# stardist/stardist

Hardware: AMD Instinct MI355X
Metric: predict_instances() Mpix/s (2D) + Mvox/s (3D) end-to-end at 1/2/4/8 GPU (higher is better)
Workload: dtype f32

## Files before the change

include/stardist_hip.h:

```cpp
#ifndef STARDIST_HIP_H
#define STARDIST_HIP_H

#include <stdbool.h>
#include <stdint.h>

#ifdef __cplusplus
extern "C" {
#endif

const char* sd_last_error(void);
int sd_version(void);
int sd_device_count(void);
int sd_release_workspace(void);
int sd_set_option(const char* name, int value);
int sd_get_option(const char* name);

int sd_nms2d_host(const float* dist, const float* points, int n_polys, int n_rays,
                  int use_kdtree, int use_bbox, int verbose, float threshold,
                  uint8_t* keep, int64_t* stats);
int sd_nms2d_device(const float* d_dist, const float* d_points, int n_polys, int n_rays,
                    int use_kdtree, int use_bbox, int verbose, float threshold,
                    uint8_t* d_keep, int64_t* stats, void* stream);

int sd_nms2d_build_device(const float* d_dist, const float* d_points, int n_polys, int n_rays, int32_t* d_vx, int32_t* d_vy,
                          int32_t* d_bbox, float* d_radius, float* d_area, int32_t* d_gstats, void* stream);

int sd_nms2d_old_host(const int32_t* polys, int n_polys, int n_rays, const int32_t* mapping, int height, int width,
                      float threshold, int max_bbox_search, int grid_y, int grid_x, int verbose, uint8_t* keep);
int sd_nms2d_old_device(const int32_t* d_polys, int n_polys, int n_rays, const int32_t* d_mapping, int height, int width,
                        float threshold, int max_bbox_search, int grid_y, int grid_x, int verbose, uint8_t* d_keep, void* stream);

int sd_exclusive_sum_i32_i64_device(const int32_t* d_in, int n, int64_t* d_out, void* stream);

int sd_prepare_polys_device(const int32_t* d_x, const int32_t* d_y, int n_polys, int n_verts, void* d_out,
                            int64_t out_bytes, void* stream);

int sd_clip_pairs_device(const int32_t* d_xa, const int32_t* d_ya, const int32_t* d_xb,
                         const int32_t* d_yb, int n_pairs, int n_verts,
                         int64_t* d_out_twice_area, int32_t* d_out_flags, void* stream);

int sd_area_bounds_pairs_device(const int32_t* d_xa, const int32_t* d_ya, const int32_t* d_xb, const int32_t* d_yb, int n_pairs,
                                int n_verts, float* d_out_area, float* d_out_band, int32_t* d_out_info, void* stream);
int sd_area_bounds_pairs_grid(void);

int sd_poly_pass_device(const int32_t* d_x, const int32_t* d_y, int n_polys, int n_verts, void* d_props, void* d_prep, void* stream);

int sd_star_dist2d_host(const uint16_t* src, int H, int W, int n_rays, int grid_y, int grid_x,
                        float* dst);
int sd_star_dist2d_device(const uint16_t* d_src, int H, int W, int n_rays, int grid_y,
                          int grid_x, float* d_dst, void* stream);
int sd_star_dist3d_host(const uint16_t* src, int Z, int Y, int X, const float* dz,
                        const float* dy, const float* dx, int n_rays, int grid_z, int grid_y,
                        int grid_x, float* dst);
int sd_star_dist3d_device(const uint16_t* d_src, int Z, int Y, int X, const float* d_dz,
                          const float* d_dy, const float* d_dx, int n_rays, int grid_z,
                          int grid_y, int grid_x, float* d_dst, void* stream);

int sd_edt_prob_device(const int32_t* d_lbl, int Z, int Y, int X, double sz, double sy, double sx, int max_label,
                       float* d_prob, void* stream);

int sd_polygons_to_label_host(const float* coord, const int32_t* labels, int n_polys, int n_rays,
                              int H, int W, int32_t* result);
int sd_polygons_to_label_device(const float* d_coord, const int32_t* d_labels, int n_polys,
                                int n_rays, int H, int W, int32_t* d_result, void* stream);
int sd_polygons_to_label_window_device(const float* d_coord, const int32_t* d_labels, int n_polys, int n_rays, int HI, int WI,
                                       int y0, int x0, int H, int W, int32_t* d_result, void* stream);

int sd_dist_to_coord_device(const float* d_dist, const double* d_points, const double* d_sincos, long long n_polys, int n_rays,
                            double scale_y, double scale_x, float* d_coord, void* stream);

int sd_survivor_positions_device(const unsigned char* d_keep, long long n, long long* d_positions, int32_t* d_count, void* stream);
int sd_survivors2d_device(const long long* d_positions, int m, const float* d_prob, const long long* d_points, const float* d_dist,
                          int n_rays, const double* d_sincos, float* d_out_prob, long long* d_out_points, float* d_out_coord,
                          float* d_out_coord_paint, int32_t* d_out_labels_paint, void* stream);

void _LIB_non_maximum_suppression_sparse(const float* scores, const float* dist,
                                         const float* points, const int n_polys,
                                         const int n_rays, const int n_faces, const float* verts,
                                         const int* faces, const float threshold,
                                         const int use_bbox, const int use_kdtree,
                                         const int verbose, bool* result);
int sd_nms3d_device(const float* d_scores, const float* d_dist, const float* d_points,
                    int n_polys, int n_rays, int n_faces, const float* d_verts,
                    const int* d_faces, float threshold, int use_bbox, int use_kdtree,
                    int verbose, uint8_t* d_keep, int64_t* stats, void* stream);

int sd_hiv_pairs_device(const float* d_dist, const float* d_points, int n_polys, int n_rays, int n_faces,
                        const float* d_verts, const int* d_faces, const int32_t* d_pairs, int n_pairs,
                        double* d_vol_kernel, double* d_vol_hull, void* stream);

void _LIB_polyhedron_to_label(const float* dist, const float* points, const float* verts,
                              const int* faces, const int n_polys, const int n_rays,
                              const int n_faces, const int* labels, const int nz, const int ny,
                              const int nx, const int render_mode, const int verbose,
                              const int use_overlap_label, const int overlap_label, int* result);
int sd_polyhedron_to_label_device(const float* d_dist, const float* d_points,
                                  const float* d_verts, const int* d_faces, int n_polys,
                                  int n_rays, int n_faces, const int* d_labels, int nz, int ny,
                                  int nx, int render_mode, int verbose, int use_overlap_label,
                                  int overlap_label, int* d_result, void* stream);
int sd_polyhedron_to_label_window_device(const float* d_dist, const float* d_points, const float* d_verts, const int* d_faces,
                                         int n_polys, int n_rays, int n_faces, const int* d_labels, int NZ, int NY, int NX,
                                         int z0, int y0, int x0, int nz, int ny, int nx, int render_mode, int verbose,
                                         int use_overlap_label, int overlap_label, int* d_result, void* stream);

int sd_select_candidates_device(const float* d_prob, const float* d_dist, int ndim,
                                const int* shape, const int* b, int n_rays, float thresh,
                                int cap, float* d_out_prob, float* d_out_dist,
                                int32_t* d_out_points, int32_t* d_count, void* stream);

int sd_sort_scores_desc_device(const float* d_scores, int n, float* d_sorted, int64_t* d_order, void* stream);

int sd_sorted_rows_device(const int32_t* d_points, const int64_t* d_order, int n, int ndim, const int* full_shape, const int* origin,
                          const int* grid, int64_t* d_rows, float* d_points_f32, int64_t* d_points_i64, void* stream);

void _LIB_non_maximum_suppression_2d(const float* dist, const float* points, const int n_polys,
                                     const int n_rays, const float threshold, const int use_bbox,
                                     const int use_kdtree, const int verbose, bool* result);
void _LIB_polygon_to_label(const float* coord, const int* labels, const int n_polys,
                           const int n_rays, const int ny, const int nx, int* result);
void _LIB_star_dist(const unsigned short* src, const int ny, const int nx, const int n_rays,
                    const int grid_y, const int grid_x, float* dst);
void _LIB_star_dist3d(const unsigned short* src, const int nz, const int ny, const int nx,
                      const float* pdz, const float* pdy, const float* pdx, const int n_rays,
                      const int grid_z, const int grid_y, const int grid_x, float* dst);

int sd_bias_act_device(float* d_x, const float* d_bias, long long n_outer, int n_channels,
                       long long inner, int act, void* stream);
int sd_add_bias_act_device(float* d_x, const float* d_addend, const float* d_bias, long long n_outer,
                           int n_channels, long long inner, int act, void* stream);

int sd_maxpool_ndhwc_device(const float* d_in, int n_channels, int D, int H, int W, int pz, int py, int px, float* d_out, void* stream);

int sd_inside_polyhedron_device(const float* d_dist, const float* d_centre, int n_rays, int n_faces,
                                const float* d_verts, const int* d_faces, const float* d_points,
                                long long n, int use_cone_map, uint8_t* d_out, void* stream);

int sd_bias_act_dot_device(const float* d_in, float* d_out, const float* d_bias, long long n_pix, int n_channels,
                           int act, const float* d_w, const float* d_wbias, int sigmoid, float* d_dot, void* stream);
int sd_head_rows_device(const float* d_feat, int n_channels, const long long* d_rows, long long n_rows,
                        const float* d_w, const float* d_bias, int n_out, float clamp_min, float* d_out,
                        void* stream);

long long sd_conv3_packed_floats(int c_in, int c_out, int kz);
int sd_conv3_pack_weights_host(const float* w , int c_in, int c_out, int kz, float* packed);
int sd_conv3_ndhwc_device(const float* d_src0, int c0, int stride0, int up0, const float* d_src1, int c1, int stride1, int up1,
                          int D, int H, int W, int kz, const float* d_wpacked, const float* d_bias, int c_out, int act,
                          float* d_out, void* stream);
int sd_conv3_res_ndhwc_device(const float* d_src0, int c0, int stride0, int up0, const float* d_src1, int c1, int stride1, int up1,
                              int D, int H, int W, int kz, const float* d_wpacked, const float* d_bias, const float* d_res,
                              int res_stride, int c_out, int act, float* d_out, void* stream);

long long sd_conv3_bf16x6_packed_floats(int c_in, int c_out, int kz);
int sd_conv3_bf16x6_pack_weights_host(const float* w , int c_in, int c_out, int kz, float* packed);
int sd_conv3_bf16x6_ndhwc_device(const float* d_src0, int c0, int stride0, int up0, const float* d_src1, int c1, int stride1,
                                 int up1, int D, int H, int W, int kz, const float* d_wpacked, const float* d_bias, int c_out,
                                 int act, float* d_out, void* stream);
int sd_conv3_bf16x6_res_ndhwc_device(const float* d_src0, int c0, int stride0, int up0, const float* d_src1, int c1, int stride1,
                                     int up1, int D, int H, int W, int kz, const float* d_wpacked, const float* d_bias,
                                     const float* d_res, int res_stride, int c_out, int act, float* d_out, void* stream);

long long sd_conv3_f16x3_packed_floats(int c_in, int c_out, int kz);
int sd_conv3_f16x3_pack_weights_host(const float* w , int c_in, int c_out, int kz, float* packed);
int sd_conv3_f16x3_ndhwc_device(const float* d_src0, int c0, int stride0, int up0, const float* d_src1, int c1, int stride1,
                                int up1, int D, int H, int W, int kz, const float* d_wpacked, const float* d_bias, int c_out,
                                int act, float* d_out, int* d_range_flag, void* stream);
int sd_conv3_f16x3_res_ndhwc_device(const float* d_src0, int c0, int stride0, int up0, const float* d_src1, int c1, int stride1,
                                    int up1, int D, int H, int W, int kz, const float* d_wpacked, const float* d_bias,
                                    const float* d_res, int res_stride, int c_out, int act, float* d_out, int* d_range_flag,
                                    void* stream);

int sd_conv3_f16x3_dot_ndhwc_device(const float* d_src0, int c0, int stride0, int up0, const float* d_src1, int c1, int stride1,
                                    int up1, int D, int H, int W, int kz, const float* d_wpacked, const float* d_bias, int c_out,
                                    int act, float* d_out, int* d_range_flag, const float* d_dot_w, float* d_dot_partial, void* stream);
int sd_dot_combine_device(const float* d_partial, int groups, long long n_pix, const float* d_wbias, int sigmoid, float* d_out, void* stream);

int sd_conv3_f16x3_fmt_ndhwc_device(const float* d_src0, int c0, int up0, const float* d_src1, int c1, int up1, int D, int H, int W, int kz,
                                    const float* d_wpacked, const float* d_bias, int c_out, int act, float* d_out, int in_split16,
                                    int out_split16, int* d_range_flag, const float* d_dot_w, float* d_dot_partial, void* stream);
int sd_conv3_f16x3_rows_device(const float* d_src, int c_in, int in_split16, int D, int H, int W, int kz, const float* d_wpacked,
                               const float* d_bias, int c_out, int act, const long long* d_rows, long long n_rows, float* d_out, void* stream);
int sd_conv3_c1x32_split16_device(const float* d_src, int D, int H, int W, int kz, const float* d_wpacked, const float* d_bias, int act,
                                  float* d_out, int* d_range_flag, void* stream);
int sd_maxpool_split16_ndhwc_device(const float* d_in, int n_channels, int D, int H, int W, int pz, int py, int px, float* d_out, void* stream);
int sd_split16_pack_device(const float* d_in, long long n_pix, int n_channels, float* d_out, int* d_range_flag, void* stream);
int sd_split16_unpack_device(const float* d_in, long long n_pix, int n_channels, float* d_out, void* stream);

int sd_upcat_ndhwc_device(const float* d_a, int ca, int up, const float* d_b, int cb, int D, int H, int W, float* d_out, void* stream);

long long sd_convg_packed_floats(int c_in, int c_out, int kz, int ky, int kx);
int sd_convg_pack_weights_host(const float* w , int c_in, int c_out, int kz, int ky, int kx, float* packed);
int sd_convg_ndhwc_device(const float* d_src, int c_in, int src_stride, int D, int H, int W, int kz, int ky, int kx, int sz, int sy,
                          int sx, int pz, int py, int px, int Do, int Ho, int Wo, const float* d_wpacked, const float* d_bias,
                          const float* d_res, int res_stride, int c_out, int act, float* d_out, int out_stride, void* stream);

int sd_label_overlap_device(const int32_t* d_true, const int32_t* d_pred, long long n, long long cap, int64_t* d_keys, int64_t* d_counts,
                            long long* h_count, int32_t* h_minmax, void* stream);

int sd_label_overlap_stack_device(const int32_t* d_ys, int K, long long n, long long cap, int64_t* d_keys, int64_t* d_counts,
                                  long long* h_offsets, long long* h_count, int32_t* h_minmax, void* stream);

int sd_relabel_stack_device(const int32_t* d_ys, int K, long long n, const int32_t* d_ids, const int32_t* d_new,
                            const long long* h_offsets, const int32_t* h_max, int32_t* d_out, void* stream);

int sd_conv_wgrad_ndhwc_device(const float* d_g, int c_out, const float* d_src0, int c0, int up0, const float* d_src1, int c1, int up1,
                               int B, int H, int W, int k, float* d_dw, float* d_db, void* stream);
int sd_relu_mask_device(const float* d_dy, const float* d_y, long long n, float* d_out, void* stream);
int sd_maxpool_adjoint_ndhwc_device(const float* d_in, const float* d_gout, int n_channels, int B, int H, int W, int py, int px,
                                    float* d_gin, void* stream);
int sd_upcat_adjoint_ndhwc_device(const float* d_gcat, int c0, int up0, int c1, int B, int H, int W, float* d_g0, float* d_g1, void* stream);
int sd_stardist_loss2d_device(const float* d_prob, const float* d_dist, const float* d_prob_true, const float* d_dist_true_mask,
                              long long n_pix, int n_rays, int dist_loss, double w_prob, double w_dist, double background_reg,
                              double* d_losses, float* d_grad_logit, float* d_grad_dist, void* stream);
int sd_stardist_loss2d_metrics_device(const float* d_prob, const float* d_dist, const float* d_prob_true, const float* d_dist_true_mask,
                                      long long n_pix, int n_rays, int dist_loss, double w_prob, double w_dist, double background_reg,
                                      double* d_losses, float* d_grad_logit, float* d_grad_dist, double* d_metrics, void* stream);

int sd_conv3_wgrad_ndhwc_device(const float* d_g, int c_out, const float* d_src0, int c0, int up0, const float* d_src1, int c1, int up1,
                                int B, int D, int H, int W, float* d_dw, float* d_db, void* stream);
int sd_convg_wgrad_ndhwc_device(const float* d_g, int c_out, const float* d_src, int c_in, int B, int D, int H, int W, int kz, int ky,
                                int kx, int sz, int sy, int sx, int pz, int py, int px, int Do, int Ho, int Wo, float* d_dw, float* d_db,
                                void* stream);
int sd_convg_dgrad_ndhwc_device(const float* d_g, int c_out, const float* d_wt, int c_in, int B, int D, int H, int W, int kz, int ky,
                                int kx, int sz, int sy, int sx, int pz, int py, int px, int Do, int Ho, int Wo, float* d_gin, void* stream);
int sd_maxpool3d_adjoint_ndhwc_device(const float* d_in, const float* d_gout, int n_channels, int B, int D, int H, int W, int pz, int py,
                                      int px, float* d_gin, void* stream);
int sd_upcat3d_adjoint_ndhwc_device(const float* d_gcat, int c0, int up0, int c1, int B, int D, int H, int W, float* d_g0, float* d_g1,
// ... 84 lines not shown
```

stardist_amd/csrc/common.h:

```cpp
#pragma once
#include <hip/hip_runtime.h>
#include <stdint.h>
#include <stdio.h>
#include <string.h>

namespace sd {

char* err_buf();
void set_error(const char* fmt, ...);

#define SD_CHECK(expr)                                                                   \
  do {                                                                                   \
    hipError_t _e = (expr);                                                              \
    if (_e != hipSuccess) {                                                              \
      sd::set_error("%s:%d: %s -> %s", __FILE__, __LINE__, #expr, hipGetErrorString(_e)); \
      return -1;                                                                         \
    }                                                                                    \
  } while (0)

#define SD_LAUNCH_CHECK() SD_CHECK(hipGetLastError())

class Arena {
 public:
  int begin(hipStream_t stream);
  void* take(size_t bytes);
  template <typename T> T* take_n(size_t n) { return (T*)take((n ? n : 1) * sizeof(T)); }
  void release();
  size_t capacity() const;
 private:
  enum { kMaxChunks = 64 };
  void* base_[kMaxChunks] = {};
  size_t cap_[kMaxChunks] = {};
  int n_ = 0, cur_ = 0;
  size_t off_ = 0;
};
Arena& arena();

hipStream_t side_stream();

enum { kMaxDevices = 64 };
int resident_grid(const void* kernel, int threads, int* cache);

int cu_count();
int allow_dynamic_lds(const void* const* kernels, int n, int bytes, bool* done);

static inline int div_up(long long a, long long b) { return (int)((a + b - 1) / b); }

enum Option { OPT_NMS3D_VOLUME_BOUNDS, OPT_NMS3D_CONE_MAP, OPT_NMS3D_REFINE_MESH, OPT_PROBE_TIER, OPT_PROBE_NO_GENERAL, OPT_TRACE, OPT_NMS3D_TAIL_BATCH, OPT_NMS3D_SPLIT_EXACT, OPT_CONV_F16_WGS, OPT_NMS2D_PAIR_LANES, OPT_NMS2D_AREA_BOUNDS, OPT_NMS2D_DEFER_UNDECIDED, OPT_NMS2D_STRICT, OPT_NMS2D_NBR_SINGLE, OPT_NMS3D_NBR_SINGLE, OPT_NMS2D_DEFER_MAX, OPT_NMS3D_BOUNDS_REUSE, OPT_NMS3D_DEFER_EXACT, OPT_NMS3D_BOUNDS_LEAN, OPT_COUNT };
int option(Option o);

#ifdef SD_DEBUG_SWITCHES
int tuning_env(const char* name, int dflt);
#else
static inline int tuning_env(const char*, int dflt) { return dflt; }
#endif

}
```

stardist_amd/csrc/lib.hip:

```cpp
#include "common.h"
#include "../../include/stardist_hip.h"
#include <stdarg.h>
#include <stdlib.h>
#include <mutex>

namespace sd {

static thread_local char g_err[1024] = "";
char* err_buf() { return g_err; }
void set_error(const char* fmt, ...) {
  va_list ap;
  va_start(ap, fmt);
  vsnprintf(g_err, sizeof(g_err), fmt, ap);
  va_end(ap);
}

static int g_opt[OPT_COUNT] = {1, 1, 2, 1, 0, 0, 1, 3, 2, 64, 1, 2, 0, 1, 1, 16384, 1, 3, 1};
static const char* const g_opt_name[OPT_COUNT] = {"nms3d_volume_bounds", "nms3d_cone_map", "nms3d_refine_mesh", "probe_tier", "probe_no_general", "trace", "nms3d_tail_batch", "nms3d_split_exact", "conv_f16_workgroups_per_cu", "nms2d_pair_lanes", "nms2d_area_bounds", "nms2d_defer_undecided", "nms2d_strict", "nms2d_neighbours_single_pass", "nms3d_neighbours_single_pass", "nms2d_defer_max", "nms3d_bounds_reuse", "nms3d_defer_exact", "nms3d_bounds_lean"};
int option(Option o) { return g_opt[o]; }
#ifdef SD_DEBUG_SWITCHES
int tuning_env(const char* name, int dflt) { const char* e = getenv(name); return e ? atoi(e) : dflt; }
#endif

static Arena g_arena[kMaxDevices];
Arena& arena() {
  int d = 0;
  if (hipGetDevice(&d) != hipSuccess || d < 0 || d >= kMaxDevices) d = 0;
  return g_arena[d];
}

hipStream_t side_stream() {
  static std::mutex mu;
  static hipStream_t st[kMaxDevices] = {};
  int d = 0;
  if (hipGetDevice(&d) != hipSuccess || d < 0 || d >= kMaxDevices) { set_error("side_stream: no current device"); return nullptr; }
  std::lock_guard<std::mutex> lock(mu);
  if (!st[d] && hipStreamCreateWithFlags(&st[d], hipStreamNonBlocking) != hipSuccess) { st[d] = nullptr; set_error("side_stream: cannot create a stream"); }
  return st[d];
}

int resident_grid(const void* kernel, int threads, int* cache) {
  static std::mutex mu;
  int d = 0;
  if (hipGetDevice(&d) != hipSuccess || d < 0 || d >= kMaxDevices) { set_error("resident_grid: no current device"); return 0; }
  std::lock_guard<std::mutex> lock(mu);
  if (!cache[d]) {
    int per_cu = 0, cus = 0;
    if (hipOccupancyMaxActiveBlocksPerMultiprocessor(&per_cu, kernel, threads, 0) != hipSuccess ||
        hipDeviceGetAttribute(&cus, hipDeviceAttributeMultiprocessorCount, d) != hipSuccess || per_cu <= 0 || cus <= 0) {
      set_error("resident_grid: occupancy query failed");
      return 0;
    }
    cache[d] = per_cu * cus;
  }
  return cache[d];
}

int cu_count() {
  static std::mutex mu;
  static int n_cu[kMaxDevices] = {};
  int d = 0;
  SD_CHECK(hipGetDevice(&d));
  const bool kept = d >= 0 && d < kMaxDevices;
  std::lock_guard<std::mutex> lock(mu);
  if (kept && n_cu[d] > 0) return n_cu[d];
  int cus = 0;
  SD_CHECK(hipDeviceGetAttribute(&cus, hipDeviceAttributeMultiprocessorCount, d));
  if (cus <= 0) cus = 256;
  if (kept) n_cu[d] = cus;
  return cus;
}

int allow_dynamic_lds(const void* const* kernels, int n, int bytes, bool* done) {
  static std::mutex mu;
  int d = 0;
  SD_CHECK(hipGetDevice(&d));
  const bool kept = d >= 0 && d < kMaxDevices;
  std::lock_guard<std::mutex> lock(mu);
  if (kept && done[d]) return 0;
  for (int k = 0; k < n; ++k) SD_CHECK(hipFuncSetAttribute(kernels[k], hipFuncAttributeMaxDynamicSharedMemorySize, bytes));
  if (kept) done[d] = true;
  return 0;
}

size_t Arena::capacity() const { size_t t = 0; for (int i = 0; i < n_; ++i) t += cap_[i]; return t; }
int Arena::begin(hipStream_t stream) {
  if (n_ > 1) {
    size_t total = capacity();
    SD_CHECK(hipStreamSynchronize(stream));
    for (int i = 0; i < n_; ++i) { (void)hipFree(base_[i]); base_[i] = nullptr; cap_[i] = 0; }
    n_ = 0;
    size_t want = total + (total >> 3);
    SD_CHECK(hipMalloc(&base_[0], want));
    cap_[0] = want; n_ = 1;
  }
  cur_ = 0; off_ = 0;
  return 0;
}
void* Arena::take(size_t bytes) {
  for (;;) {
    if (cur_ < n_) {
      size_t a = (off_ + 255) & ~size_t(255);
      if (a + bytes <= cap_[cur_]) { off_ = a + bytes; return (char*)base_[cur_] + a; }
      ++cur_; off_ = 0;
      continue;
    }
    if (n_ >= kMaxChunks) { set_error("workspace arena: too many chunks"); return nullptr; }
    size_t want = bytes + (bytes >> 2) + (size_t(4) << 20);
    void* p = nullptr;
    hipError_t e = hipMalloc(&p, want);
    if (e != hipSuccess) { set_error("workspace arena: hipMalloc(%zu) failed: %s", want, hipGetErrorString(e)); return nullptr; }
    base_[n_] = p; cap_[n_] = want; cur_ = n_; ++n_; off_ = 0;
  }
}
void Arena::release() {
  for (int i = 0; i < n_; ++i) { (void)hipFree(base_[i]); base_[i] = nullptr; cap_[i] = 0; }
  n_ = 0; cur_ = 0; off_ = 0;
}

}

extern "C" {
int sd_set_option(const char* name, int value) {
  for (int k = 0; name && k < sd::OPT_COUNT; ++k)
    if (!strcmp(name, sd::g_opt_name[k])) { sd::g_opt[k] = value; return 0; }
  sd::set_error("sd_set_option: unknown option '%s'", name ? name : "(null)");
  return -1;
}
int sd_get_option(const char* name) {
  for (int k = 0; name && k < sd::OPT_COUNT; ++k)
    if (!strcmp(name, sd::g_opt_name[k])) return sd::g_opt[k];
  return -1;
}
const char* sd_last_error(void) { return sd::err_buf(); }
int sd_version(void) { return 1; }
int sd_device_count(void) {
  int n = 0;
  if (hipGetDeviceCount(&n) != hipSuccess) return 0;
  return n;
}
int sd_release_workspace(void) { sd::arena().release(); return 0; }
}
```

stardist_amd/csrc/nms2d.hip:

```cpp
#include <type_traits>

#include "common.h"
#include "clip_sweep.h"
#include "clip_beam.h"
#include "area_bounds.h"
#include "poly_pass.h"
#include "nms_rounds.h"
#include "../../include/stardist_hip.h"
#include <hipcub/hipcub.hpp>
#include <math.h>
#include <stdlib.h>
#include <vector>

namespace {

using sdclip::i64;

__device__ __forceinline__ float wave_min(float v) { for (int o = 32; o; o >>= 1) v = fminf(v, __shfl_xor(v, o)); return v; }
__device__ __forceinline__ float wave_max(float v) { for (int o = 32; o; o >>= 1) v = fmaxf(v, __shfl_xor(v, o)); return v; }
__device__ __forceinline__ i64 wave_sum(i64 v) { for (int o = 32; o; o >>= 1) v += __shfl_xor(v, o); return v; }

__global__ void __launch_bounds__(256) k_build(const float* __restrict__ dist, const float* __restrict__ pts,
                                               const float2* __restrict__ sincos, int N, int R,
                                               int* __restrict__ vx, int* __restrict__ vy, int4* __restrict__ bbox,
// ... 522 lines not shown
    pairs[t] = ij;
    if (kind[t] == 0) { exact[atomicAdd(nExact, 1u)] = t; decided[t] = 3; }
    else if (state[ij.y] == ST_SUPPRESSED) { decided[t] = 4; atomicAdd(nSkipped, 1u); }
    else decided[t] = 0;
  }
  if (blockIdx.x == 0 && threadIdx.x == 0) { *nPairs = n; *firstNew = n; }
}
__global__ void k_round_lists_init(int N, int* __restrict__ U, unsigned char* __restrict__ state, unsigned char* __restrict__ pend,
                                   int* __restrict__ head, unsigned int* __restrict__ dcount) {
  const int i = blockIdx.x * blockDim.x + threadIdx.x;
  if (i == 0) *dcount = 0;
  if (i >= N) return;
  U[i] = i; state[i] = ST_UNDECIDED; pend[i] = 0; head[i] = -1;
}
__global__ void k_copy_u32(unsigned int* dst, const unsigned int* src) { *dst = *src; }
__device__ __forceinline__ bool deferred_suppresses(int j, const int* __restrict__ defHead, const int* __restrict__ defNext,
                                                    const unsigned char* __restrict__ supp) {
  for (int k = defHead[j]; k >= 0; k = defNext[k]) if (supp[k]) return true;
  return false;
}

__global__ void __launch_bounds__(256) k_tail_step(const int* __restrict__ U, int nU, unsigned char* state, const int2* __restrict__ pairs,
                                                   const unsigned char* __restrict__ supp, const unsigned int* __restrict__ segStart,
                                                   const int* __restrict__ segCnt, unsigned long long pairCap,
                                                   const int* __restrict__ defHead, const int* __restrict__ defNext) {
  const int t = blockIdx.x * blockDim.x + threadIdx.x;
  if (t >= nU) return;
  const int j = U[t];
  if (state[j] != ST_UNDECIDED) return;
  bool wait = false, sup = deferred_suppresses(j, defHead, defNext, supp);
  const unsigned int e0 = segStart[t];
  const int c = segCnt[t];
  for (int e = 0; e < c && !sup; ++e) {
    if ((unsigned long long)e0 + e >= pairCap) { wait = true; break; }
    const unsigned char si = state[pairs[e0 + e].x];
    if (si == ST_UNDECIDED) wait = true;
    else if (si == ST_KEPT && supp[e0 + e]) sup = true;
  }
  if (sup) state[j] = ST_SUPPRESSED;
  else if (!wait) state[j] = ST_KEPT;
}
__global__ void __launch_bounds__(1024) k_tail_resolve(const int* __restrict__ U, int nU, volatile unsigned char* state,
                                                       const int2* __restrict__ pairs, const unsigned char* __restrict__ supp,
                                                       const unsigned int* __restrict__ segStart, const int* __restrict__ segCnt,
                                                       unsigned long long pairCap, int* left, const int* __restrict__ defHead,
                                                       const int* __restrict__ defNext) {
  __shared__ int changed, undecided;
  for (int iter = 0; iter <= nU; ++iter) {
    if (threadIdx.x == 0) { changed = 0; undecided = 0; }
    __syncthreads();
    for (int t = threadIdx.x; t < nU; t += blockDim.x) {
      const int j = U[t];
      if (state[j] != ST_UNDECIDED) continue;
      bool wait = false, sup = deferred_suppresses(j, defHead, defNext, supp);
      const unsigned int e0 = segStart[t];
      const int c = segCnt[t];
      for (int e = 0; e < c && !sup; ++e) {
        if ((unsigned long long)e0 + e >= pairCap) { wait = true; break; }
        const unsigned char si = state[pairs[e0 + e].x];
        if (si == ST_UNDECIDED) wait = true;
        else if (si == ST_KEPT && supp[e0 + e]) sup = true;
      }
      if (sup) { state[j] = ST_SUPPRESSED; changed = 1; }
      else if (!wait) { state[j] = ST_KEPT; changed = 1; }
      else undecided = 1;
    }
    __threadfence_block();
    __syncthreads();
    const int ch = changed, un = undecided;
    __syncthreads();
    if (!un || !ch) { if (threadIdx.x == 0) *left = un; break; }
  }
}

__device__ __forceinline__ bool pair_j_suppressed(const unsigned char* __restrict__ state, int2 ij) { return state && state[ij.y] == ST_SUPPRESSED; }
constexpr int PAIR_BUCKETS = 4096;
struct PairKey { const char* prep; size_t prepStride; float inv; int nl, ny, nx; };
__device__ __forceinline__ int pair_bucket(const float* __restrict__ pts, int2 ij, const PairKey& k) {
  const float dy = pts[2 * ij.y] - pts[2 * ij.x], dx = pts[2 * ij.y + 1] - pts[2 * ij.x + 1];
  int by = (int)((dy * k.inv + 0.5f) * (float)k.ny), bx = (int)((dx * k.inv + 0.5f) * (float)k.nx);
  by = by < 0 ? 0 : (by >= k.ny ? k.ny - 1 : by); bx = bx < 0 ? 0 : (bx >= k.nx ? k.nx - 1 : bx);
  int lm = 0;
  if (k.nl > 1) {
    int a = *(const int*)(k.prep + (size_t)ij.x * k.prepStride + 4), b = *(const int*)(k.prep + (size_t)ij.y * k.prepStride + 4);
    a = a < 1 ? 0 : (a > 4 ? 3 : a - 1); b = b < 1 ? 0 : (b > 4 ? 3 : b - 1);
    lm = (a * 4 + b) % k.nl;
  }
  return (lm * k.ny + by) * k.nx + bx;
}
__global__ void __launch_bounds__(256) k_pair_bucket_count(const int2* __restrict__ pairs, const unsigned long long* __restrict__ nPtr,
                                                           const unsigned int* __restrict__ firstPtr, const float* __restrict__ pts, PairKey key,
                                                           unsigned int* __restrict__ hist, const unsigned char* __restrict__ decided,
                                                           const unsigned char* __restrict__ state, unsigned int* __restrict__ nSkipped) {
  __shared__ unsigned int h[PAIR_BUCKETS];
  __shared__ unsigned int skipped;
  for (int b = threadIdx.x; b < PAIR_BUCKETS; b += 256) h[b] = 0;
  if (threadIdx.x == 0) skipped = 0;
  __syncthreads();
  const unsigned long long n = *nPtr, first = firstPtr ? *firstPtr : 0u;
  for (unsigned long long t = first + (unsigned long long)blockIdx.x * 256 + threadIdx.x; t < n; t += (unsigned long long)gridDim.x * 256) {
    if (decided && decided[t]) continue;
    const int2 ij = pairs[t];
    if (pair_j_suppressed(state, ij)) { atomicAdd(&skipped, 1u); continue; }
    atomicAdd(&h[pair_bucket(pts, ij, key)], 1u);
  }
  __syncthreads();
  for (int b = threadIdx.x; b < PAIR_BUCKETS; b += 256) if (h[b]) atomicAdd(&hist[b], h[b]);
  if (threadIdx.x == 0 && skipped) atomicAdd(nSkipped, skipped);
}
__global__ void __launch_bounds__(1024) k_pair_bucket_scan(const unsigned int* __restrict__ hist, unsigned int* __restrict__ cursor,
                                                           unsigned long long* __restrict__ nOrdered) {
  __shared__ unsigned int sh[1024];
  const int t = threadIdx.x;
  unsigned int v[PAIR_BUCKETS / 1024], tot = 0;
#pragma unroll
  for (int k = 0; k < PAIR_BUCKETS / 1024; ++k) { v[k] = hist[t * (PAIR_BUCKETS / 1024) + k]; tot += v[k]; }
  sh[t] = tot;
  __syncthreads();
  for (int o = 1; o < 1024; o <<= 1) {
    const unsigned int add = t >= o ? sh[t - o] : 0u;
    __syncthreads();
    sh[t] += add;
    __syncthreads();
  }
  unsigned int run = sh[t] - tot;
#pragma unroll
  for (int k = 0; k < PAIR_BUCKETS / 1024; ++k) { cursor[t * (PAIR_BUCKETS / 1024) + k] = run; run += v[k]; }
  if (t == 1023) *nOrdered = sh[t];
}
__global__ void __launch_bounds__(256) k_pair_bucket_scatter(const int2* __restrict__ pairs, const unsigned long long* __restrict__ nPtr,
                                                             const unsigned int* __restrict__ firstPtr, const float* __restrict__ pts, PairKey key,
                                                             unsigned int* __restrict__ cursor, unsigned int* __restrict__ order, unsigned int cap,
                                                             const unsigned char* __restrict__ decided, const unsigned char* __restrict__ state) {
  const unsigned long long n = *nPtr, first = firstPtr ? *firstPtr : 0u;
  for (unsigned long long t = first + (unsigned long long)blockIdx.x * 256 + threadIdx.x; t < n; t += (unsigned long long)gridDim.x * 256) {
    if (decided && decided[t]) continue;
    const int2 ij = pairs[t];
    if (pair_j_suppressed(state, ij)) continue;
    const unsigned int k = atomicAdd(&cursor[pair_bucket(pts, ij, key)], 1u);
    if (k < cap) order[k] = (unsigned int)t;
  }
}

__global__ void k_count_after(unsigned int* out, const unsigned int* total, const unsigned int* first) { *out = *total > *first ? *total - *first : 0u; }

}

namespace sd {
int clip_full_pairs(const int2* d_pairs, const unsigned int* d_idx, const unsigned int* d_n, unsigned int cap, int R, const int* d_vx, const int* d_vy,
                    const float* d_area, float thr, unsigned char* d_state, unsigned char* d_supp, unsigned int* d_errCount, hipStream_t stream);
}

namespace {
struct Counters { int nU, nK, nS, left; unsigned long long nPairs; unsigned int nSpill, nExact, nErr, nDecided, nSkipped; };

template <int MAXV, int SPREP>
struct BeamPath {
  typedef sdclip::PolyPrep<MAXV> Prep;
  static constexpr size_t prep_stride = sizeof(Prep);
  static constexpr bool two_tiers = MAXV == 32;
  static int prepare(const int* vx, const int* vy, int N, int R, sdarea::PolyProps* props, void* prep, hipStream_t s) {
    if constexpr (MAXV == 32) {
      if (sdpass::launch_poly_pass(vx, vy, N, R, props, prep, s)) { sd::set_error("sd_nms2d: launch of the per-polygon pass failed"); return -1; }
      return 0;
    } else {
      const size_t lds = sdclip::PrepWork<sdclip::LdsStorage<SPREP>, MAXV>::lds_bytes() + 64;
      hipLaunchKernelGGL((k_prepare<MAXV, SPREP>), dim3(sd::div_up(N, SPREP)), dim3(SPREP), lds, s, vx, vy, N, R, (Prep*)prep);
      SD_LAUNCH_CHECK();
      return 0;
    }
  }
  static int tier1(const int2* pairs, const unsigned int* idx, const unsigned long long* nPairs, const unsigned int* first, const void* prep, const float* area,
                   float thr, unsigned char* state, unsigned char* supp, PairQueues q, hipStream_t s) {
    const int lanes = sd::option(sd::OPT_NMS2D_PAIR_LANES);
    if (lanes == 32) {
      static const size_t lds32 = beam_lds_bytes<MAXV, 8, 6, 4, 32>();
      hipLaunchKernelGGL((k_pairs_beam<MAXV, 8, 6, 4, 32, unsigned long long>), dim3(256 * 8), dim3(32), lds32, s, pairs, idx, nPairs, first, (const Prep*)prep, area, thr, state, supp, q);
    } else if (lanes == 6464) {
      static const size_t lds = beam_lds_bytes<MAXV, 8, 6, 4, 64>();
      hipLaunchKernelGGL((k_pairs_beam<MAXV, 8, 6, 4, 64, unsigned long long>), dim3(256 * 4), dim3(64), lds, s, pairs, idx, nPairs, first, (const Prep*)prep, area, thr, state, supp, q);
    } else {
      static const size_t lds16 = beam_lds_bytes<MAXV, 8, 6, 4, 64, true>();
      static const int per_cu = (int)((160 * 1024) / lds16);
      hipLaunchKernelGGL((k_pairs_beam<MAXV, 8, 6, 4, 64, unsigned long long, true>), dim3(256 * per_cu), dim3(64), lds16, s, pairs, idx, nPairs, first, (const Prep*)prep, area, thr, state, supp, q);
    }
    SD_LAUNCH_CHECK();
    return 0;
  }
  template <typename CNT>
  static int tier2(const int2* pairs, const unsigned int* idx, const CNT* nPairs, const unsigned int* first, const void* prep, const float* area, float thr,
                   unsigned char* state, unsigned char* supp, PairQueues q, hipStream_t s) {
    static const size_t lds = beam_lds_bytes<MAXV, 15, 16, 8, 32>();
    hipLaunchKernelGGL((k_pairs_beam<MAXV, 15, 16, 8, 32, CNT>), dim3(256 * 3), dim3(32), lds, s, pairs, idx, nPairs, first, (const Prep*)prep, area, thr, state, supp, q);
    SD_LAUNCH_CHECK();
    return 0;
  }
};
template <class F>
int with_beam_path(int R, F&& f) {
  if (R <= 32) return f(BeamPath<32, 64>{});
  if (R <= 64) return f(BeamPath<64, 64>{});
  if (R <= 128) return f(BeamPath<128, 32>{});
  return f(BeamPath<256, 16>{});
}
size_t prep_stride(int R) { return (size_t)with_beam_path(R, [](auto bp) { return (int)decltype(bp)::prep_stride; }); }
int prepare_polys(const int* vx, const int* vy, int N, int R, sdarea::PolyProps* props, void* prep, hipStream_t s) {
  return with_beam_path(R, [&](auto bp) { return decltype(bp)::prepare(vx, vy, N, R, props, prep, s); });
}

struct Sweep {
  hipStream_t s; int R; const int *vx, *vy; const void* prep; const float* area; float thr;
  const int2* pairs; unsigned int *spillPairs, *exactPairs, qCap; Counters* d_cnt; unsigned char *state, *supp;
};
int general_path(const Sweep& w) {
  return sd::clip_full_pairs(w.pairs, w.exactPairs, &w.d_cnt->nExact, w.qCap, w.R, w.vx, w.vy, w.area, w.thr, w.state, w.supp, &w.d_cnt->nErr, w.s);
}
template <class General>
int sweep_tiers(const Sweep& w, const unsigned int* idx, const unsigned long long* n, const unsigned int* first, Timer& pairTimer, General general) {
  const PairQueues q1{w.spillPairs, &w.d_cnt->nSpill, w.exactPairs, &w.d_cnt->nExact, w.qCap};
  const PairQueues q2{w.exactPairs, &w.d_cnt->nExact, w.exactPairs, &w.d_cnt->nExact, w.qCap};
  const int rc = with_beam_path(w.R, [&](auto bp) -> int {
    typedef decltype(bp) BP;
    if constexpr (BP::two_tiers) {
      if (BP::tier1(w.pairs, idx, n, first, w.prep, w.area, w.thr, w.state, w.supp, q1, w.s) || pairTimer.stop(w.s)) return -1;
      return BP::tier2(w.pairs, w.spillPairs, &w.d_cnt->nSpill, (const unsigned int*)nullptr, w.prep, w.area, w.thr, w.state, w.supp, q2, w.s);
    } else {
      if (BP::tier2(w.pairs, idx, n, first, w.prep, w.area, w.thr, w.state, w.supp, q2, w.s)) return -1;
      return pairTimer.stop(w.s);
    }
  });
  return rc ? -1 : general();
}
int check_sweep(const char* who, const Counters& h, unsigned int qCap, bool listOverflow, const char* alsoCounted) {
  if (listOverflow || h.nSpill > qCap || h.nExact > qCap) { sd::set_error("%s: pair queue overflow (internal error)", who); return -1; }
  if (h.nErr) { sd::set_error("%s: %u pairs exceeded the general path's fixed capacities%s", who, h.nErr, alsoCounted); return -1; }
  return 0;
}

int launch_build(sd::Arena& A, hipStream_t s, const float* d_dist, const float* d_points, int N, int R, int* vx, int* vy, int4* bbox,
                 float* radius, float* area, int** gstatsOut, hipEvent_t evStart) {
  const int gs_init[8] = {0, INT32_MAX, INT32_MIN, INT32_MAX, INT32_MIN, 0, 0, 0};
  std::vector<float> hdr(8 + 2 * (size_t)R);
  memcpy(hdr.data(), gs_init, sizeof(gs_init));
  const float ANGLE_PI = 2 * M_PI / R;
  for (int k = 0; k < R; ++k) { hdr[8 + 2 * k] = sinf(ANGLE_PI * k); hdr[8 + 2 * k + 1] = cosf(ANGLE_PI * k); }
  int* gstats = A.take_n<int>(8 + 2 * (size_t)R);
  if (!gstats) return -1;
  const float2* d_sc = (const float2*)(gstats + 8);
  SD_CHECK(hipMemcpyAsync(gstats, hdr.data(), hdr.size() * sizeof(float), hipMemcpyHostToDevice, s));
  if (evStart) SD_CHECK(hipEventRecord(evStart, s));
  if (R <= 32) {
    const int vec4 = ((((uintptr_t)d_dist | (uintptr_t)vx | (uintptr_t)vy) & 15) == 0) ? 1 : 0;
    hipLaunchKernelGGL(k_build32, dim3(sd::div_up(N, 64)), dim3(64), 2 * 64 * (size_t)R * sizeof(int), s, d_dist, d_points, d_sc, N, R, vec4,
                       vx, vy, bbox, radius, area, gstats);
  } else
    hipLaunchKernelGGL(k_build, dim3(sd::div_up(N, 4)), dim3(256), 4 * 2 * R * sizeof(int), s, d_dist, d_points, d_sc, N, R,
                       vx, vy, bbox, radius, area, gstats);
  SD_LAUNCH_CHECK();
  *gstatsOut = gstats;
  return 0;
}
}

extern "C" int sd_nms2d_build_device(const float* d_dist, const float* d_points, int n_polys, int n_rays, int32_t* d_vx, int32_t* d_vy,
                                     int32_t* d_bbox, float* d_radius, float* d_area, int32_t* d_gstats, void* stream_) {
  hipStream_t s = (hipStream_t)stream_;
  if (n_polys <= 0) return 0;
  if (n_rays < 1 || n_rays > 256) { sd::set_error("sd_nms2d_build: n_rays=%d unsupported (1..256)", n_rays); return -1; }
  sd::Arena& A = sd::arena();
  if (A.begin(s)) return -1;
  int* gstats = nullptr;
  if (launch_build(A, s, d_dist, d_points, n_polys, n_rays, d_vx, d_vy, (int4*)d_bbox, d_radius, d_area, &gstats, nullptr)) return -1;
  SD_CHECK(hipMemcpyAsync(d_gstats, gstats, 5 * sizeof(int), hipMemcpyDeviceToDevice, s));
  SD_CHECK(hipStreamSynchronize(s));
  return 0;
}

namespace {
struct SideEvents {
  hipEvent_t props = nullptr, prep = nullptr;
  ~SideEvents() { if (props) (void)hipEventDestroy(props); if (prep) (void)hipEventDestroy(prep); }
  int init() { SD_CHECK(hipEventCreateWithFlags(&props, hipEventDisableTiming)); SD_CHECK(hipEventCreateWithFlags(&prep, hipEventDisableTiming)); return 0; }
};

struct Nms2d {
  hipStream_t s; const float *dist, *pts; int N, R, use_kdtree, use_bbox; float thr; bool wantStats; sd::Arena& A;
  bool areaBounds = false, singlePass = false, ordered = false, decide = false, deferOn = false, trace = false;
  int tailT = -1, deferFrom = 0, keyMode = 2; unsigned int deferMax = 0;
  hipStream_t side = nullptr; sd::SideJoin sideJoin; SideEvents sideEv;
  Timer broadTimer, pairTimer, fullTimer, replayTimer;
  double ns_pairs = 0, ns_full = 0, ns_pre = 0; long long n_pair_launches = 0;
  int *vx = nullptr, *vy = nullptr, *candCell = nullptr, *gstats = nullptr; int4* bbox = nullptr; float *radius = nullptr, *area = nullptr;
  unsigned char* state = nullptr; void* prep = nullptr; size_t prepStride = 0; sdarea::PolyProps* props = nullptr;
  GridP g; NmsFlags f; float max_dist = 0, reach = 0;
  int by_bbox = 0, *cellStart = nullptr, *nbrCount = nullptr, *nbrLow = nullptr, *Ucur = nullptr; i64* nbrStart = nullptr; CellRec* cellRec = nullptr;
  void* scanTmp = nullptr; size_t scanBytes = 0; Deferred dfr{nullptr, nullptr, nullptr, nullptr, nullptr, 0};
  NbrLists L{}; i64 totalNbr = 0;
  unsigned long long pairCap = 0, *nOrdered = nullptr; int2* pairs = nullptr; unsigned char *decided = nullptr, *defKind = nullptr;
  unsigned int qCap = 0, *spillPairs = nullptr, *exactPairs = nullptr, *pairOrder = nullptr, *bucketHist = nullptr, *firstNew = nullptr, *nNewExact = nullptr, *nJoinDef = nullptr;
  int *Unext = nullptr, *K = nullptr, *Sl = nullptr, decideGrid = 0; Counters *d_cnt = nullptr, h;
  int nU = 0, rounds = 0; bool forceTail = false;
  i64 nDeferred = 0, nUndecDeferredUpper = 0, totalPairs = 0, totalExact = 0, totalSpill = 0, totalUndecDeferred = 0, totalDecided = 0, totalSkipped = 0;
  unsigned char* supp = nullptr; unsigned int* segStart = nullptr; int* segCnt = nullptr;

  Nms2d(hipStream_t s_, const float* dist_, const float* pts_, int N_, int R_, int use_kdtree_, int use_bbox_, float thr_, bool wantStats_)
      : s(s_), dist(dist_), pts(pts_), N(N_), R(R_), use_kdtree(use_kdtree_), use_bbox(use_bbox_), thr(thr_), wantStats(wantStats_), A(sd::arena()) {}

// ... 132 lines not shown
    firstNew = A.take_n<unsigned int>(1);
    nNewExact = A.take_n<unsigned int>(1);
    if (!Unext || !K || !pairs || !spillPairs || !exactPairs || !Sl || !d_cnt || !bucketHist || !nOrdered || !firstNew || !nNewExact || (ordered && !pairOrder) ||
        (decide && !decided)) return -1;
    static int decideGridOf[sd::kMaxDevices] = {};
    decideGrid = decide ? sd::resident_grid((const void*)k_pairs_decide, 256, decideGridOf) : 0;
    if (decide && decideGrid <= 0) return -1;
    dfr.cap = qCap;
    if (deferOn) {
      dfr.pairs = A.take_n<int2>(qCap);
      dfr.next = A.take_n<int>(qCap);
      if (!dfr.pairs || !dfr.next) return -1;
    }
    if (deferFrom > 0) {
      defKind = A.take_n<unsigned char>(qCap); nJoinDef = A.take_n<unsigned int>(1);
      if (!defKind || !nJoinDef) return -1;
      SD_CHECK(hipMemsetAsync(defKind, 0, qCap, s));
    }
    nU = N;
    return 0;
  }

  int order_pairs(unsigned char* suppOut, const unsigned int* first) {
    static const int modes[6][3] = {{1, 32, 32}, {1, 64, 16}, {1, 64, 64}, {16, 16, 16}, {16, 32, 8}, {4, 32, 32}};
    const int* md = modes[keyMode >= 0 && keyMode < 6 ? keyMode : 2];
    const PairKey key{(const char*)prep, prepStride, 1.f / (4.f * (max_dist + 1.f)), md[0], md[1], md[2]};
    SD_CHECK(hipMemsetAsync(bucketHist, 0, PAIR_BUCKETS * sizeof(unsigned int), s));
    if (decided)
      hipLaunchKernelGGL(k_pairs_decide, dim3(decideGrid), dim3(256), 0, s, pairs, &d_cnt->nPairs, first, vx, vy, R, props, area, thr, state, suppOut,
                         decided, &d_cnt->nDecided);
    if (!suppOut && deferFrom > 0 && rounds >= deferFrom)
      hipLaunchKernelGGL(k_defer_undecided, dim3(256), dim3(256), 0, s, pairs, &d_cnt->nPairs, &d_cnt->nDecided, deferMax, decided, state, dfr, defKind, &d_cnt->nErr);
    const unsigned int* bfirst = (suppOut && deferFrom > 0) ? nullptr : first;
    SD_CHECK(hipStreamWaitEvent(s, sideEv.prep, 0));
    const unsigned char* liveState = suppOut ? nullptr : state;
    hipLaunchKernelGGL(k_pair_bucket_count, dim3(512), dim3(256), 0, s, pairs, &d_cnt->nPairs, bfirst, pts, key, bucketHist, decided, liveState,
                       &d_cnt->nSkipped);
    hipLaunchKernelGGL(k_pair_bucket_scan, dim3(1), dim3(1024), 0, s, bucketHist, bucketHist + PAIR_BUCKETS, nOrdered);
    hipLaunchKernelGGL(k_pair_bucket_scatter, dim3(512), dim3(256), 0, s, pairs, &d_cnt->nPairs, bfirst, pts, key, bucketHist + PAIR_BUCKETS,
                       pairOrder, qCap, decided, liveState);
    SD_LAUNCH_CHECK();
    return 0;
  }

  int sweep_pairs(unsigned char* suppOut) {
    const unsigned int* first = suppOut ? firstNew : nullptr;
    if (pairTimer.start(s)) return -1;
    if (!ordered) SD_CHECK(hipStreamWaitEvent(s, sideEv.prep, 0));
    else if (order_pairs(suppOut, first)) return -1;
    const Sweep w{s, R, vx, vy, prep, area, thr, pairs, spillPairs, exactPairs, qCap, d_cnt, state, suppOut};
    auto general = [&]() -> int {
      if (fullTimer.start(s)) return -1;
      if (!suppOut && deferOn) {
        hipLaunchKernelGGL(k_defer, dim3(64), dim3(256), 0, s, pairs, exactPairs, &d_cnt->nExact, qCap, dfr, &d_cnt->nErr);
        SD_LAUNCH_CHECK();
      } else if (suppOut && sideJoin.pending) {
        hipLaunchKernelGGL(k_count_after, dim3(1), dim3(1), 0, s, nNewExact, &d_cnt->nExact, deferFrom > 0 ? nJoinDef : firstNew);
        SD_LAUNCH_CHECK();
        if (sd::clip_full_pairs(pairs, exactPairs + nDeferred, nNewExact, qCap - (unsigned int)nDeferred, R, vx, vy, area, thr, state, suppOut, &d_cnt->nErr, s)) return -1;
        if (sideJoin.join(s)) return -1;
      } else if (general_path(w)) return -1;
      return fullTimer.stop(s);
    };
    if (ordered) return sweep_tiers(w, pairOrder, nOrdered, nullptr, pairTimer, general);
    return sweep_tiers(w, nullptr, &d_cnt->nPairs, first, pairTimer, general);
  }

  int account(const char* what) {
    if (check_sweep("sd_nms2d", h, qCap, h.nPairs > pairCap,
                    " or the deferred-pair list (with more than 64 rays: at least that many; the launch stops at the first)")) return -1;
    totalPairs += (i64)h.nPairs; totalExact += h.nExact; totalSpill += h.nSpill; totalDecided += h.nDecided; totalSkipped += h.nSkipped;
    if (wantStats) {
      float ms = 0, ms2 = 0;
      if (pairTimer.ms(&ms) || fullTimer.ms(&ms2)) return -1;
      if (h.nPairs) { ns_pairs += ms * 1e6; ++n_pair_launches; }
      ns_full += ms2 * 1e6;
      if (trace) printf("%s %d: nU=%d nK=%d pairs=%llu decided by the area enclosure=%u j already suppressed=%u spill=%u exact=%u pair_kernel=%.3f ms general_path=%.3f ms\n", what, rounds, h.nU, h.nK, h.nPairs, h.nDecided, h.nSkipped, h.nSpill, h.nExact, ms, ms2);
    }
    return 0;
  }

  int run_round() {
    ++rounds;
    if (tailT >= 0 && ((nU <= tailT && rounds > 1) || forceTail)) return tail_batch();
    SD_CHECK(hipMemsetAsync(d_cnt, 0, sizeof(Counters), s));
    hipLaunchKernelGGL(k_round_triage, dim3(sd::div_up(nU, 1024)), dim3(1024), 0, s, Ucur, nU, state, L.waitOn, Unext, K, Sl, (int*)d_cnt, dfr.pend);
    const int wgrid = sd::div_up(nU, 4) < 2048 ? sd::div_up(nU, 4) : 2048;
    hipLaunchKernelGGL(k_round_scan, dim3(wgrid), dim3(256), 0, s, Sl, state, nbrStart, nbrLow, L.nbr, L.waitOn, Unext, K, (int*)d_cnt, dfr.pend);
    hipLaunchKernelGGL(k_round_emit, dim3(wgrid), dim3(256), 0, s, K, &d_cnt->nK, state, g, cellRec, cellStart, by_bbox, reach, f, pts, bbox,
                       radius, area, pairs, &d_cnt->nPairs, pairCap);
    SD_LAUNCH_CHECK();
    if (sweep_pairs(nullptr)) return -1;
    SD_CHECK(hipMemcpyAsync(&h, d_cnt, sizeof(Counters), hipMemcpyDeviceToHost, s));
    SD_CHECK(hipStreamSynchronize(s));
    if (h.nK == 0 && h.nU > 0) {
      if (deferOn && (nDeferred > 0 || nUndecDeferredUpper > 0) && !forceTail) forceTail = true;
      else { sd::set_error("sd_nms2d: greedy scan made no progress (internal error)"); return -1; }
    }
    if (deferOn) nDeferred += h.nExact;
    if (deferFrom > 0 && rounds >= deferFrom && h.nPairs > h.nDecided && h.nPairs - h.nDecided <= deferMax) nUndecDeferredUpper += (i64)(h.nPairs - h.nDecided);
    if (account("round")) return -1;
    nU = h.nU;
    int* t = Ucur; Ucur = Unext; Unext = t;
    return 0;
  }

  int tail_batch() {
    if (!supp) { supp = A.take_n<unsigned char>(pairCap); segStart = A.take_n<unsigned int>(N); segCnt = A.take_n<int>(N); }
    if (!supp || !segStart || !segCnt) return -1;
    SD_CHECK(hipMemsetAsync(d_cnt, 0, sizeof(Counters), s));
    SD_CHECK(hipMemsetAsync(supp, 0, pairCap, s));
    if (deferFrom > 0) {
      hipLaunchKernelGGL(k_tail_init2, dim3(64), dim3(256), 0, s, dfr, defKind, pairs, exactPairs, &d_cnt->nPairs, &d_cnt->nExact, firstNew, decided, state,
                         &d_cnt->nSkipped);
      hipLaunchKernelGGL(k_copy_u32, dim3(1), dim3(1), 0, s, nJoinDef, &d_cnt->nExact);
    } else
      hipLaunchKernelGGL(k_tail_init, dim3(64), dim3(256), 0, s, dfr, pairs, exactPairs, &d_cnt->nPairs, &d_cnt->nExact, firstNew);
    if (deferOn && nDeferred > 0 && nDeferred < (i64)qCap) {
      if (sideJoin.begin(s, side)) return -1;
      if (sd::clip_full_pairs(pairs, exactPairs, deferFrom > 0 ? nJoinDef : firstNew, qCap, R, vx, vy, area, thr, state, supp, &d_cnt->nErr, side)) return -1;
      if (sideJoin.end(side)) return -1;
    }
    const int wg = sd::div_up(nU, 4) < 2048 ? sd::div_up(nU, 4) : 2048;
    hipLaunchKernelGGL(k_tail_emit, dim3(wg), dim3(256), 0, s, Ucur, nU, state, nbrStart, nbrLow, L.nbr, f, pts, bbox, radius, area, pairs,
                       &d_cnt->nPairs, pairCap, segStart, segCnt);
    SD_LAUNCH_CHECK();
    if (sweep_pairs(supp)) return -1;
    if (trace && (replayTimer.init() || replayTimer.start(s))) return -1;
    for (int it = 0; it < 10; ++it)
      hipLaunchKernelGGL(k_tail_step, dim3(sd::div_up(nU, 256)), dim3(256), 0, s, Ucur, nU, state, pairs, supp, segStart, segCnt, pairCap, dfr.head, dfr.next);
    hipLaunchKernelGGL(k_tail_resolve, dim3(1), dim3(1024), 0, s, Ucur, nU, state, pairs, supp, segStart, segCnt, pairCap, &d_cnt->left, dfr.head, dfr.next);
    SD_LAUNCH_CHECK();
    if (trace) {
      float ms = 0;
      if (replayTimer.stop(s) || replayTimer.wait() || replayTimer.ms(&ms)) return -1;
      printf("tail replay (10 steps + resolve loop): %.3f ms\n", ms);
    }
    unsigned int hDefTotal = (unsigned int)nDeferred;
    SD_CHECK(hipMemcpyAsync(&h, d_cnt, sizeof(Counters), hipMemcpyDeviceToHost, s));
    if (deferFrom > 0) SD_CHECK(hipMemcpyAsync(&hDefTotal, dfr.count, sizeof(unsigned int), hipMemcpyDeviceToHost, s));
    SD_CHECK(hipStreamSynchronize(s));
    h.nU = nU; h.nK = 0;
    if (deferFrom > 0) totalUndecDeferred = (i64)hDefTotal - nDeferred;
    const unsigned long long counted = deferFrom > 0 ? (unsigned long long)hDefTotal : (unsigned long long)nDeferred;
    if (counted <= h.nPairs) h.nPairs -= counted;
    if ((i64)h.nExact >= nDeferred) h.nExact -= (unsigned int)nDeferred;
    if (account("tail batch after round")) return -1;
    if (h.left) { sd::set_error("sd_nms2d: tail batch left candidates undecided (internal error)"); return -1; }
    nU = 0;
    return 0;
  }

  int report(uint8_t* d_keep, int64_t* stats, int verbose) {
    hipLaunchKernelGGL(k_keep, dim3(sd::div_up(N, 256)), dim3(256), 0, s, state, d_keep, N);
    SD_LAUNCH_CHECK();
    SD_CHECK(hipStreamSynchronize(s));
    if (stats) { stats[0] = totalPairs; stats[1] = totalExact; stats[2] = rounds; stats[3] = totalNbr;
                 stats[4] = (int64_t)ns_pairs; stats[5] = n_pair_launches; stats[6] = (int64_t)ns_full; stats[7] = (int64_t)ns_pre;
                 stats[8] = totalSpill; stats[9] = totalDecided; stats[10] = totalUndecDeferred; stats[11] = totalSkipped;
                 stats[12] = L.slotTotal; stats[13] = L.slots ? 1 : 0; }
    if (verbose) {
      printf("NMS: %lld pair intersections (%lld on the exact-join path), %d greedy rounds, %lld neighbour entries\n",
             (long long)totalPairs, (long long)totalExact, rounds, (long long)totalNbr);
      fflush(stdout);
    }
    return 0;
  }
};
}

extern "C" int sd_nms2d_device(const float* d_dist, const float* d_points, int n_polys, int n_rays, int use_kdtree,
                               int use_bbox, int verbose, float threshold, uint8_t* d_keep, int64_t* stats,
                               void* stream_) {
  hipStream_t s = (hipStream_t)stream_;
  if (stats) memset(stats, 0, 16 * sizeof(int64_t));
  if (n_polys <= 0) return 0;
  Nms2d c(s, d_dist, d_points, n_polys, n_rays, use_kdtree, use_bbox, threshold, stats != nullptr);
  if (c.plan()) return -1;
  if (verbose) {
    printf("Non Maximum Suppression (2D) ++++ \n");
    printf("NMS: n_polys    = %d \nNMS: n_rays     = %d  \nNMS: thresh     = %.3f \nNMS: use_bbox   = %d\nNMS: use_kdtree = %d\n",
           n_polys, n_rays, threshold, use_bbox, use_kdtree);
    printf("NMS: using HIP (gfx950), uniform-grid broad phase + scan-beam pair kernel\n");
  }
  if (!use_kdtree && !use_bbox && threshold < 0) {
    SD_CHECK(hipMemsetAsync(d_keep, 0, n_polys, s));
    SD_CHECK(hipMemsetAsync(d_keep, 1, 1, s));
    SD_CHECK(hipStreamSynchronize(s));
    return 0;
  }
  if (c.build() || c.build_grid() || c.build_lists() || c.begin_rounds()) return -1;
  while (c.nU > 0)
    if (c.run_round()) return -1;
  return c.report(d_keep, stats, verbose);
}

namespace {
__global__ void __launch_bounds__(256) k_old_build(const int* __restrict__ polys, int N, int R, int* __restrict__ vx, int* __restrict__ vy,
                                                   int4* __restrict__ bbox, float* __restrict__ area, int* __restrict__ gmax) {
  const int i = blockIdx.x * blockDim.x + threadIdx.x;
  if (i >= N) return;
  const int* py = polys + (size_t)i * 2 * R;
  const int* px = py + R;
  int x1 = 0, x2 = 0, y1 = 0, y2 = 0;
  float a = 0.f;
  for (int k = 0; k < R; ++k) {
    const int y = py[k], x = px[k];
    if (k == 0) { x1 = x2 = x; y1 = y2 = y; }
    else { x1 = x < x1 ? x : x1; x2 = x > x2 ? x : x2; y1 = y < y1 ? y : y1; y2 = y > y2 ? y : y2; }
    vx[(size_t)i * R + k] = x; vy[(size_t)i * R + k] = y;
    const int kn = (k + 1 == R) ? 0 : k + 1;
    a += (float)((i64)x * py[kn] - (i64)y * px[kn]);
  }
  area[i] = (float)(0.5 * (double)fabsf(a));
  bbox[i] = make_int4(x1, x2, y1, y2);
  atomicMax(&gmax[0], x2 - x1); atomicMax(&gmax[1], y2 - y1);
}
struct OldSearch { int max_bbox_search, grid_y, grid_x, height, width; };
template <int MODE>
__global__ void __launch_bounds__(256) k_old_pairs(int N, OldSearch o, const int* __restrict__ mapping, const int4* __restrict__ bbox,
                                                   const int* __restrict__ gmax, int* __restrict__ cnt, const i64* __restrict__ start,
                                                   int2* __restrict__ pairs) {
  const int lane = threadIdx.x & 63;
  const int i = blockIdx.x * (blockDim.x >> 6) + (threadIdx.x >> 6);
  if (i >= N) return;
  const int4 bi = bbox[i];
  const i64 base = MODE ? start[i] : 0;
  int n = 0;
  auto visit = [&](bool in, int j) {
    const bool hit = in && j > i && j < N && bbox_intersect(bi, bbox[j]);
    const unsigned long long m = __ballot(hit);
    if (MODE && hit) pairs[base + n + __popcll(m & ((1ull << lane) - 1))] = make_int2(i, j);
    n += __popcll(m);
  };
  if (o.max_bbox_search) {
    const int mx = gmax[0], my = gmax[1];
    const int xs = max((bi.x - mx) / o.grid_x, 0), xe = min((bi.y + mx) / o.grid_x, o.width);
    const int ys = max((bi.z - my) / o.grid_y, 0), ye = min((bi.w + my) / o.grid_y, o.height);
    const int w = xe - xs, h = ye - ys;
    if (w > 0 && h > 0) {
      const i64 tot = (i64)w * h;
      for (i64 t = 0; t < tot; t += 64) {
        const i64 q = t + lane;
        const bool in = q < tot;
        int j = -1;
        if (in) { const int jj = ys + (int)(q / w), ii = xs + (int)(q % w); j = mapping[(size_t)jj * o.width + ii]; }
        visit(in, j);
      }
    }
  } else {
    for (int t = i + 1; t < N; t += 64) visit(t + lane < N, t + lane);
  }
  if (!MODE && lane == 0) cnt[i] = n;
}
__global__ void __launch_bounds__(1024) k_old_replay(int N, const i64* __restrict__ start, const int2* __restrict__ pairs,
                                                     const unsigned char* __restrict__ supp, volatile unsigned char* state) {
  for (int i = 0; i < N; ++i) {
    const i64 beg = start[i], end = start[i + 1];
    if (beg == end) continue;
    if (state[i] != ST_SUPPRESSED)
      for (i64 t = beg + threadIdx.x; t < end; t += blockDim.x) if (supp[t]) state[pairs[t].y] = ST_SUPPRESSED;
    __threadfence_block();
    __syncthreads();
  }
}
}

extern "C" int sd_nms2d_old_device(const int32_t* d_polys, int n_polys, int n_rays, const int32_t* d_mapping, int height, int width,
                                   float threshold, int max_bbox_search, int grid_y, int grid_x, int verbose, uint8_t* d_keep,
                                   void* stream_) {
  hipStream_t s = (hipStream_t)stream_;
  const int N = n_polys, R = n_rays;
  if (N <= 0) return 0;
  if (R < 1 || R > 256) { sd::set_error("sd_nms2d_old: n_rays=%d unsupported (1..256)", R); return -1; }
  if (max_bbox_search && (!d_mapping || height <= 0 || width <= 0 || grid_y <= 0 || grid_x <= 0)) {
    sd::set_error("sd_nms2d_old: max_bbox_search needs a (height, width) mapping and positive grid steps"); return -1;
  }
  if (verbose) {
    printf("Non Maximum Suppression (2D) ++++ \n");
    printf("NMS: n_polys  = %d \nNMS: n_rays   = %d  \nNMS: thresh   = %.3f \nNMS: max_bbox_search = %d \n", N, R, threshold, max_bbox_search);
    printf("NMS: using HIP (gfx950), every candidate pair by the scan-beam pair kernel, greedy order replayed on the device\n");
  }
  sd::Arena& A = sd::arena();
  if (A.begin(s)) return -1;
  int* vx = A.take_n<int>((size_t)N * R);
  int* vy = A.take_n<int>((size_t)N * R);
  int4* bbox = A.take_n<int4>(N);
  float* area = A.take_n<float>(N);
  int* gmax = A.take_n<int>(2);
  unsigned char* state = A.take_n<unsigned char>(N);
  int* cnt = A.take_n<int>(N + 1);
  i64* start = A.take_n<i64>(N + 1);
  Counters* d_cnt = (Counters*)A.take(sizeof(Counters));
  if (!vx || !vy || !bbox || !area || !gmax || !state || !cnt || !start || !d_cnt) return -1;
  SD_CHECK(hipMemsetAsync(gmax, 0, 2 * sizeof(int), s));
  SD_CHECK(hipMemsetAsync(state, 0, N, s));
  SD_CHECK(hipMemsetAsync(cnt, 0, (N + 1) * sizeof(int), s));
  SD_CHECK(hipMemsetAsync(d_cnt, 0, sizeof(Counters), s));
  hipLaunchKernelGGL(k_old_build, dim3(sd::div_up(N, 256)), dim3(256), 0, s, d_polys, N, R, vx, vy, bbox, area, gmax);
  SD_LAUNCH_CHECK();
  const OldSearch o{max_bbox_search, grid_y, grid_x, height, width};
  hipLaunchKernelGGL((k_old_pairs<0>), dim3(sd::div_up(N, 4)), dim3(256), 0, s, N, o, d_mapping, bbox, gmax, cnt, (const i64*)nullptr, (int2*)nullptr);
  SD_LAUNCH_CHECK();
  size_t tmpBytes = 0;
  (void)exclusive_sum_i64(nullptr, tmpBytes, cnt, start, N + 1, s);
  void* scanTmp = A.take(tmpBytes + 256);
  if (!scanTmp) return -1;
  SD_CHECK(exclusive_sum_i64(scanTmp, tmpBytes, cnt, start, N + 1, s));
  i64 total = 0;
  SD_CHECK(hipMemcpyAsync(&total, start + N, sizeof(i64), hipMemcpyDeviceToHost, s));
  SD_CHECK(hipStreamSynchronize(s));
  if (total < 0 || total >= (i64)(1ll << 30)) {
    sd::set_error("sd_nms2d_old: %lld candidate pairs exceed the capacity of one call (2^30)", (long long)total); return -1;
  }
  if (total > 0) {
    const unsigned int qCap = (unsigned int)total + 64u;
    int2* pairs = A.take_n<int2>((size_t)total + 64);
    unsigned char* supp = A.take_n<unsigned char>((size_t)total + 64);
    unsigned int* spillPairs = A.take_n<unsigned int>(qCap);
    unsigned int* exactPairs = A.take_n<unsigned int>(qCap);
    void* prep = A.take((size_t)N * prep_stride(R));
    if (!pairs || !supp || !spillPairs || !exactPairs || !prep) return -1;
    SD_CHECK(hipMemsetAsync(supp, 0, (size_t)total + 64, s));
    hipLaunchKernelGGL((k_old_pairs<1>), dim3(sd::div_up(N, 4)), dim3(256), 0, s, N, o, d_mapping, bbox, gmax, cnt, (const i64*)start, pairs);
    SD_LAUNCH_CHECK();
    const unsigned long long nP = (unsigned long long)total;
    SD_CHECK(hipMemcpyAsync(&d_cnt->nPairs, &nP, sizeof(nP), hipMemcpyHostToDevice, s));
    const Sweep w{s, R, vx, vy, prep, area, threshold, pairs, spillPairs, exactPairs, qCap, d_cnt, state, supp};
    Timer untimed;
    if (prepare_polys(vx, vy, N, R, nullptr, prep, s)) return -1;
    if (sweep_tiers(w, nullptr, &d_cnt->nPairs, nullptr, untimed, [&]() { return general_path(w); })) return -1;
    hipLaunchKernelGGL(k_old_replay, dim3(1), dim3(1024), 0, s, N, (const i64*)start, (const int2*)pairs, (const unsigned char*)supp, state);
    SD_LAUNCH_CHECK();
    Counters h;
    SD_CHECK(hipMemcpyAsync(&h, d_cnt, sizeof(Counters), hipMemcpyDeviceToHost, s));
    SD_CHECK(hipStreamSynchronize(s));
    if (check_sweep("sd_nms2d_old", h, qCap, false, "")) return -1;
  }
  hipLaunchKernelGGL(k_keep, dim3(sd::div_up(N, 256)), dim3(256), 0, s, state, d_keep, N);
  SD_LAUNCH_CHECK();
  SD_CHECK(hipStreamSynchronize(s));
  if (verbose) { printf("NMS: %lld candidate pairs evaluated\n", (long long)total); fflush(stdout); }
  return 0;
}

extern "C" int sd_exclusive_sum_i32_i64_device(const int32_t* d_in, int n, int64_t* d_out, void* stream_) {
  hipStream_t s = (hipStream_t)stream_;
  if (n <= 0) return 0;
  sd::Arena& A = sd::arena();
  if (A.begin(s)) return -1;
  size_t tmpBytes = 0;
  (void)exclusive_sum_i64(nullptr, tmpBytes, (const int*)d_in, (long long*)d_out, n, s);
  void* tmp = A.take(tmpBytes + 256);
  if (!tmp) return -1;
  SD_CHECK(exclusive_sum_i64(tmp, tmpBytes, (const int*)d_in, (long long*)d_out, n, s));
  SD_CHECK(hipStreamSynchronize(s));
  return 0;
}

extern "C" int sd_nms2d_old_host(const int32_t* polys, int n_polys, int n_rays, const int32_t* mapping, int height, int width,
                                 float threshold, int max_bbox_search, int grid_y, int grid_x, int verbose, uint8_t* keep) {
  if (n_polys <= 0) return 0;
  int32_t *d_polys = nullptr, *d_map = nullptr;
  uint8_t* d_keep = nullptr;
  const size_t pb = (size_t)n_polys * 2 * n_rays * sizeof(int32_t), mb = max_bbox_search ? (size_t)height * width * sizeof(int32_t) : 0;
  SD_CHECK(hipMalloc(&d_polys, pb));
  if (mb) SD_CHECK(hipMalloc(&d_map, mb));
  SD_CHECK(hipMalloc(&d_keep, n_polys));
  int rc = -1;
  do {
    if (hipMemcpy(d_polys, polys, pb, hipMemcpyHostToDevice) != hipSuccess) { sd::set_error("H2D failed"); break; }
    if (mb && hipMemcpy(d_map, mapping, mb, hipMemcpyHostToDevice) != hipSuccess) { sd::set_error("H2D failed"); break; }
    if (sd_nms2d_old_device(d_polys, n_polys, n_rays, d_map, height, width, threshold, max_bbox_search, grid_y, grid_x, verbose, d_keep, nullptr)) break;
    if (hipMemcpy(keep, d_keep, n_polys, hipMemcpyDeviceToHost) != hipSuccess) { sd::set_error("D2H failed"); break; }
    rc = 0;
  } while (0);
  (void)hipFree(d_polys); if (d_map) (void)hipFree(d_map); (void)hipFree(d_keep);
  return rc;
}

extern "C" int sd_nms2d_host(const float* dist, const float* points, int n_polys, int n_rays, int use_kdtree, int use_bbox,
                             int verbose, float threshold, uint8_t* keep, int64_t* stats) {
  if (n_polys <= 0) return 0;
  float *d_dist = nullptr, *d_pts = nullptr;
  uint8_t* d_keep = nullptr;
  SD_CHECK(hipMalloc(&d_dist, (size_t)n_polys * n_rays * sizeof(float)));
  SD_CHECK(hipMalloc(&d_pts, (size_t)n_polys * 2 * sizeof(float)));
  SD_CHECK(hipMalloc(&d_keep, n_polys));
  int rc = -1;
  do {
    if (hipMemcpy(d_dist, dist, (size_t)n_polys * n_rays * sizeof(float), hipMemcpyHostToDevice) != hipSuccess) { sd::set_error("H2D failed"); break; }
    if (hipMemcpy(d_pts, points, (size_t)n_polys * 2 * sizeof(float), hipMemcpyHostToDevice) != hipSuccess) { sd::set_error("H2D failed"); break; }
    if (sd_nms2d_device(d_dist, d_pts, n_polys, n_rays, use_kdtree, use_bbox, verbose, threshold, d_keep, stats, nullptr)) break;
    if (hipMemcpy(keep, d_keep, n_polys, hipMemcpyDeviceToHost) != hipSuccess) { sd::set_error("D2H failed"); break; }
    rc = 0;
  } while (0);
  (void)hipFree(d_dist); (void)hipFree(d_pts); (void)hipFree(d_keep);
  return rc;
}
```

stardist_amd/csrc/nms3d.hip:

```cpp
#include <algorithm>

#include "common.h"
#include "geom3d.h"
#include "nms_rounds.h"
#include "nms3d_shared.h"
#include "nms3d_lds.h"
#include "nms3d_hiv.h"
#include "nms3d_mesh.h"
#include "nms3d_hull.h"
#include "../../include/stardist_hip.h"
#include <hipcub/hipcub.hpp>
#include <math.h>
#include <vector>

namespace {

typedef long long i64;

__device__ __forceinline__ const float* stage_rows(const float* __restrict__ dist, int N, int R, float* lds, int staged) {
  if (!staged) return dist + (size_t)min((int)(blockIdx.x * blockDim.x + threadIdx.x), N - 1) * R;
  const int i0 = blockIdx.x * blockDim.x;
  const int rows = min((int)blockDim.x, N - i0);
  const float* src = dist + (size_t)i0 * R;
  const int pitch = sdl::RowsLds{R}.pitch();
// ... 1126 lines not shown
  template <class Exact>
  int finish_volume_stage(bool sp, bool tail, unsigned int nPairs, unsigned int* d_nX, unsigned int Counters::*nX, Exact launchExact, double* ns, float* ms) {
    const bool defer = sp && !tail && deferFrom > 0 && rounds >= deferFrom && hDef + nPairs <= dfrCap;
    if (defer)
      hipLaunchKernelGGL(k_defer3, dim3(nPairs < 16384u ? sd::div_up(nPairs, 256) : 64), dim3(256), 0, s, pairsX, d_nX, dfr, dfrCount, dfrCap, pend, &d_st->overflow);
    else if (sp) launchExact();
    SD_LAUNCH_CHECK();
    if (stageTimer.stop(s)) return -1;
    SD_CHECK(hipMemcpyAsync(&h, d_cnt, sizeof(Counters), hipMemcpyDeviceToHost, s));
    SD_CHECK(hipStreamSynchronize(s));
    if (defer) hDef += h.*nX;
    if (stageTimer.ms(ms)) return -1;
    *ns += *ms * 1e6;
    return 0;
  }

  int run_stage3(bool tail, const SuppSink& sink) {
    const unsigned int nP3 = h.nP3, b3grid = nP3 < 16384u ? nP3 : 16384u;
    if (stageTimer.start(s)) return -1;
    const bool sp3 = split3 && nP3 <= split3Max;
    const sdl::PairLds small = sdl::stage3_lds(R, F, sdl::WS_SMALL, b.R, 1);
    const bool small3 = sp3 && splitOpt >= 2 && small.ws < lds.s3.ws;
    const sdl::PairLds l3 = !small3 ? lds.s3 : leanOpt ? sdl::stage3_lds(R, F, sdl::WS_LEAN, b.R, 1) : small;
    hipLaunchKernelGGL(k_stage3, dim3(b3grid), dim3(64), l3.bytes(), s, pairs3, nP3, dist, pts, rays.verts, rays.faces, faceAdj, R, volume,
                       thr, sink, pairs4, &d_cnt->nP4, d_st, l3, flags3, b.verts, b.faces, b.R, b.F, (double*)nullptr, sp3 ? pairsX : (int2*)nullptr, &d_cnt->nX3);
    float ms;
    if (finish_volume_stage(sp3, tail, nP3, &d_cnt->nX3, &Counters::nX3, [&]() {
          hipLaunchKernelGGL(k_stage3x<4>, dim3(nP3 < 256u ? nP3 : 256u), dim3(256), lds.s3x.bytes(), s, pairsX, &d_cnt->nX3, 0u, dist, pts, rays.verts, rays.faces, faceAdj,
                             R, volume, thr, sink, pairs4, &d_cnt->nP4, d_st, lds.s3x, (double*)nullptr, b3.verts, b3.faces, b3.R, b3.F);
        }, &ns3, &ms)) return -1;
    if (wantStats && trace) printf("round %d: nU=%d nK=%d stage3 pairs=%u %.3f ms -> stage4 pairs=%u\n", rounds, h.nU, h.nK, h.nP3, ms, h.nP4);
    return 0;
  }

  int run_stage4(bool tail) {
    const unsigned int nP4 = h.nP4, b4grid = nP4 < 16384u ? nP4 : 16384u;
    if (stageTimer.start(s)) return -1;
    if (!hullPlanes) {
      hullPlanes = A.take_n<double>((size_t)N * hullCap * 4);
      hullAdj = A.take_n<unsigned short>((size_t)N * hullCap * 3);
      if (!hullPlanes || !hullAdj) return -1;
    }
    SD_CHECK(hipMemsetAsync(&d_cnt->nHull, 0, sizeof(unsigned int), s));
    hipLaunchKernelGGL(k_hull_mark, dim3(sd::div_up(nP4, 256)), dim3(256), 0, s, pairs4, nP4, hullState, hullList, &d_cnt->nHull);
    {
      const unsigned long long ub = 2ull * nP4;
      const unsigned int bh = ub < 32768ull ? (unsigned int)ub : 32768u;
      hipLaunchKernelGGL(k_hull, dim3(bh), dim3(64), lds.hull.bytes(), s, hullList, 0u, dist, pts, rays.verts, R, hullCap, hullPlanes, hullAdj, hullCount,
                         (const unsigned int*)&d_cnt->nHull);
      SD_LAUNCH_CHECK();
    }
    const bool sp4 = split4 && nP4 <= split4Max;
    const sdl::PairLds small = sdl::stage4_lds(hullCap, sdl::WS_SMALL, b.R, 1);
    const bool small4 = sp4 && splitOpt >= 2 && small.ws < lds.s4.ws;
    const sdl::PairLds l4 = !small4 ? lds.s4 : leanOpt ? sdl::stage4_lds(hullCap, sdl::WS_LEAN, b.R, 1) : small;
    hipLaunchKernelGGL(k_stage4, dim3(b4grid), dim3(64), l4.bytes(), s, pairs4, nP4, dist, pts, rays.verts, rays.faces, R, F, hullPlanes, hullAdj, hullCount,
                       volume, thr, pairs5, &d_cnt->nP5, d_st, l4, flags4, b.verts, b.faces, b.R, b.F, (double*)nullptr, sp4 ? pairsX : (int2*)nullptr, &d_cnt->nX4);
    float ms;
    if (finish_volume_stage(sp4, tail, nP4, &d_cnt->nX4, &Counters::nX4, [&]() {
          hipLaunchKernelGGL(k_stage4x<4>, dim3(nP4 < 256u ? nP4 : 256u), dim3(256), lds.s4x.bytes(), s, pairsX, &d_cnt->nX4, 0u, dist, pts, R, hullPlanes, hullAdj,
                             hullCount, volume, thr, pairs5, &d_cnt->nP5, d_st, lds.s4x, (double*)nullptr, b3.verts, b3.faces, b3.R, b3.F);
        }, &ns4, &ms)) return -1;
    if (wantStats && trace) printf("         stage4 pairs=%u hulls=%u %.3f ms -> stage5 pairs=%u\n", h.nP4, h.nHull, ms, h.nP5);
    return 0;
  }

  int run_stage5(const SuppSink& sink) {
    const unsigned int b5grid = h.nP5 < 16384u ? h.nP5 : 16384u;
    if (stageTimer.start(s)) return -1;
    hipLaunchKernelGGL(k_stage5, dim3(b5grid), dim3(256), lds.render.bytes(), s, pairs5, h.nP5, dist, pts, rays.verts, rays.faces, R, F, bbox, volume,
                       thr, sink, d_st, cmap, mesh_ok ? 0 : 1);
    SD_LAUNCH_CHECK();
    float ms;
    if (stageTimer.stop(s) || stageTimer.wait() || stageTimer.ms(&ms)) return -1;
    ns5 += ms * 1e6;
    return 0;
  }

  int tail_replay() {
    unsigned int nEdges = 0;
    SD_CHECK(hipMemcpyAsync(&nEdges, supCount, sizeof(unsigned int), hipMemcpyDeviceToHost, s));
    SD_CHECK(hipStreamSynchronize(s));
    if (nEdges > pairCap) { sd::set_error("sd_nms3d: tail edge list overflow (internal error)"); return -1; }
    if (trace) printf("tail batch after round %d: %d undecided candidates, %u suppressing edges, %u pairs carried over from the rounds%s\n", rounds - 1, nU, nEdges, hDef,
                      forceTail ? " (started early: every remaining candidate waits for one of them)" : "");
    int left = 1, sweeps = 0;
    while (left) {
      for (int it = 0; it < 8; ++it) {
        SD_CHECK(hipMemsetAsync(d_left, 0, sizeof(int), s));
        if (nEdges) hipLaunchKernelGGL(k_tail3_mark, dim3(sd::div_up(nEdges, 256)), dim3(256), 0, s, supEdges, nEdges, state, blocked);
        hipLaunchKernelGGL(k_tail3_promote, dim3(sd::div_up(nU, 256)), dim3(256), 0, s, Ucur, nU, state, blocked, d_left);
      }
      SD_LAUNCH_CHECK();
      SD_CHECK(hipMemcpyAsync(&left, d_left, sizeof(int), hipMemcpyDeviceToHost, s));
      SD_CHECK(hipStreamSynchronize(s));
      if (++sweeps > N / 8 + 4) { sd::set_error("sd_nms3d: tail replay does not converge (internal error)"); return -1; }
    }
    return 0;
  }

  int run_round() {
    ++rounds;
    const bool tail = rounds > 1 && (nU <= tailT || forceTail);
    SD_CHECK(hipMemsetAsync(d_cnt, 0, sizeof(Counters), s));
    if (tail) {
      if (!supEdges) {
        supEdges = A.take_n<int2>(pairCap); supCount = A.take_n<unsigned int>(1); blocked = A.take_n<unsigned char>(N); d_left = A.take_n<int>(1);
        if (!supEdges || !supCount || !blocked || !d_left) return -1;
      }
      SD_CHECK(hipMemsetAsync(supCount, 0, sizeof(unsigned int), s));
      SD_CHECK(hipMemsetAsync(blocked, 0, N, s));
      if (hDef) hipLaunchKernelGGL(k_seed3, dim3(sd::div_up(hDef, 256)), dim3(256), 0, s, dfr, dfrCount, dfrCap, pairs3, &d_cnt->nP3);
      h.nK = nU; h.nU = 0;
    } else {
      hipLaunchKernelGGL(k_round_triage, dim3(sd::div_up(nU, 256)), dim3(256), 0, s, Ucur, nU, state, L.waitOn, Unext, Kl, Sl, (int*)d_cnt, (const unsigned char*)pend);
      const int wgrid = sd::div_up(nU, 4) < 2048 ? sd::div_up(nU, 4) : 2048;
      hipLaunchKernelGGL(k_round_scan, dim3(wgrid), dim3(256), 0, s, Sl, state, nbrStart, nbrLow, L.nbr, L.waitOn, Unext, Kl, (int*)d_cnt, (const unsigned char*)pend);
      SD_LAUNCH_CHECK();
    }
    const SuppSink sink = tail ? SuppSink{state, supEdges, supCount, pairCap} : SuppSink{state, nullptr, nullptr, 0u};
    {
      const int egrid = sd::div_up(nU, 4) < 2048 ? sd::div_up(nU, 4) : 2048;
      hipLaunchKernelGGL(k_round_emit3, dim3(egrid), dim3(256), 0, s, tail ? Ucur : Kl, tail ? nU : 0, tail ? (const int*)nullptr : (const int*)&d_cnt->nK, sink, tail ? 1 : 0,
                         nbrStart, nbrCount, (const int*)L.nbr, f, an, pts, bbox, volume, r_outer, r_outer_iso, r_inner_iso, pairs3, &d_cnt->nP3, pairCap, d_st);
      SD_LAUNCH_CHECK();
      SD_CHECK(hipMemcpyAsync(&h, d_cnt, sizeof(Counters), hipMemcpyDeviceToHost, s));
      SD_CHECK(hipStreamSynchronize(s));
    }
    if (!tail && h.nK == 0 && h.nU > 0) {
      if (!hDef) { sd::set_error("sd_nms3d: greedy scan made no progress (internal error)"); return -1; }
      forceTail = true;
      nU = h.nU;
      std::swap(Ucur, Unext);
      return 0;
    }
    const int nUndecided = tail ? 0 : h.nU;
    if (h.nP3 > pairCap) { sd::set_error("sd_nms3d: pair queue overflow (internal error)"); return -1; }
    if (h.nP3 > 0) {
      if (run_stage3(tail, sink)) return -1;
      if (h.nP4 > 0 && run_stage4(tail)) return -1;
      if (h.nP4 > 0 && h.nP5 > 0 && run_stage5(sink)) return -1;
    }
    if (tail) {
      if (tail_replay()) return -1;
      nU = 0;
      return 0;
    }
    nU = nUndecided;
    std::swap(Ucur, Unext);
    return 0;
  }

  int report(uint8_t* d_keep, int64_t* stats) {
    hipLaunchKernelGGL(k_keep, dim3(sd::div_up(N, 256)), dim3(256), 0, s, state, d_keep, N);
    SD_LAUNCH_CHECK();
    Stats hs_;
    SD_CHECK(hipMemcpyAsync(&hs_, d_st, sizeof(Stats), hipMemcpyDeviceToHost, s));
    SD_CHECK(hipStreamSynchronize(s));
    if (hs_.overflow) { sd::set_error("sd_nms3d: half-space intersection capacity exceeded (%llu pairs)", hs_.overflow); return -1; }
    if (stats) {
      stats[0] = (int64_t)hs_.upper; stats[1] = (int64_t)hs_.lower; stats[2] = (int64_t)hs_.kernel; stats[3] = (int64_t)hs_.render;
      stats[4] = rounds; stats[5] = L.total; stats[6] = (int64_t)hs_.sup_kernel; stats[7] = (int64_t)hs_.sup_render;
      stats[8] = (int64_t)ns3; stats[9] = (int64_t)ns4; stats[10] = (int64_t)ns5; stats[11] = (int64_t)hs_.convex; stats[12] = (int64_t)hs_.kept_convex;
      stats[13] = (int64_t)hs_.near_thr; stats[14] = (int64_t)hs_.hiv_fallback;
      { float msb = 0; if (broadTimer.ms(&msb)) return -1; stats[15] = (int64_t)(msb * 1e6); }
      if (trace) printf("hiv: faces %llu list entries %llu clips %llu list overflows %llu fallbacks %llu\n", hs_.hiv_faces, hs_.hiv_list, hs_.hiv_clips, hs_.hiv_rest, hs_.hiv_fallback);
      if (trace && hs_.cyc[5]) printf("stage 3 wave cycles per pair (clock64): load+half-spaces %.0f, cull %.0f, bounds %.0f, decide/exact %.0f, total %.0f (%llu pairs)\n",
                                      (double)hs_.cyc[0] / hs_.cyc[5], (double)hs_.cyc[1] / hs_.cyc[5], (double)hs_.cyc[2] / hs_.cyc[5], (double)hs_.cyc[3] / hs_.cyc[5],
                                      (double)hs_.cyc[4] / hs_.cyc[5], hs_.cyc[5]);
      if (trace) printf("hiv: pairs decided by the lower bound %llu, by the upper bound %llu, of %llu\n", hs_.lb_decided, hs_.ub_decided, hs_.kernel + hs_.convex);
    }
    if (verbose) {
      printf("NMS: Function calls:\nNMS: ~ bbox+out: %8llu\nNMS: ~ inner:    %8llu\nNMS: ~ kernel:   %8llu\nNMS: ~ convex:   %8llu\nNMS: ~ render:   %8llu\n",
             hs_.upper, hs_.lower, hs_.kernel, hs_.convex, hs_.render);
      printf("NMS: Excluded intersection:\nNMS: + pretest:  %8llu\nNMS: + convex:   %8llu\n", hs_.kept_pre, hs_.kept_convex);
      printf("NMS: Suppressed polyhedra:\nNMS: # inner:    %8llu / %d\nNMS: # kernel:   %8llu / %d\nNMS: # render:   %8llu / %d\n", hs_.sup_pre, N,
             hs_.sup_kernel, N, hs_.sup_render, N);
      printf("NMS: greedy rounds: %d, neighbour entries: %lld\n", rounds, (long long)L.total);
      fflush(stdout);
    }
    if (trace) fflush(stdout);
    return 0;
  }
};

}

extern "C" int sd_nms3d_device(const float* d_scores, const float* d_dist, const float* d_points, int n_polys, int n_rays, int n_faces,
                               const float* d_verts, const int* d_faces, float threshold, int use_bbox, int use_kdtree, int verbose,
                               uint8_t* d_keep, int64_t* stats, void* stream_) {
  (void)d_scores;
  hipStream_t s = (hipStream_t)stream_;
  if (stats) memset(stats, 0, 16 * sizeof(int64_t));
  if (verbose) {
    printf("Non Maximum Suppression (3D) ++++ \n");
    printf("NMS: n_polys  = %d \nNMS: n_rays   = %d  \nNMS: n_faces  = %d \nNMS: thresh   = %.3f \nNMS: use_bbox = %d \nNMS: use_kdtree = %d \n",
           n_polys, n_rays, n_faces, threshold, use_bbox, use_kdtree);
    printf("NMS: using HIP (gfx950)\n");
    fflush(stdout);
  }
  if (n_polys <= 0) return 0;
  Nms3d c(s, d_dist, d_points, n_polys, n_rays, n_faces, d_verts, d_faces, threshold, use_bbox, use_kdtree, verbose, stats != nullptr);
  if (c.plan()) return -1;
  if (!use_kdtree && !use_bbox && threshold < 0) {
    SD_CHECK(hipMemsetAsync(d_keep, 0, n_polys, s));
    SD_CHECK(hipMemsetAsync(d_keep, 1, 1, s));
    SD_CHECK(hipStreamSynchronize(s));
    return 0;
  }
  if (c.precompute() || c.build_grid() || c.prepare_mesh() || c.build_lists() || c.begin_rounds()) return -1;
  while (c.nU > 0)
    if (c.run_round()) return -1;
  return c.report(d_keep, stats);
}

extern "C" void _LIB_non_maximum_suppression_sparse(const float* scores, const float* dist, const float* points, const int n_polys,
                                                    const int n_rays, const int n_faces, const float* verts, const int* faces,
                                                    const float threshold, const int use_bbox, const int use_kdtree, const int verbose,
                                                    bool* result) {
  if (n_polys <= 0) return;
  float *d_dist = nullptr, *d_pts = nullptr, *d_verts = nullptr, *d_scores = nullptr;
  int* d_faces = nullptr;
  uint8_t* d_keep = nullptr;
  bool ok = hipMalloc(&d_dist, (size_t)n_polys * n_rays * 4) == hipSuccess && hipMalloc(&d_pts, (size_t)n_polys * 12) == hipSuccess &&
            hipMalloc(&d_verts, (size_t)n_rays * 12) == hipSuccess && hipMalloc(&d_faces, (size_t)n_faces * 12) == hipSuccess &&
            hipMalloc(&d_scores, (size_t)n_polys * 4) == hipSuccess && hipMalloc(&d_keep, n_polys) == hipSuccess;
  if (ok) {
    ok = hipMemcpy(d_dist, dist, (size_t)n_polys * n_rays * 4, hipMemcpyHostToDevice) == hipSuccess &&
         hipMemcpy(d_pts, points, (size_t)n_polys * 12, hipMemcpyHostToDevice) == hipSuccess &&
         hipMemcpy(d_verts, verts, (size_t)n_rays * 12, hipMemcpyHostToDevice) == hipSuccess &&
         hipMemcpy(d_faces, faces, (size_t)n_faces * 12, hipMemcpyHostToDevice) == hipSuccess &&
         (scores == nullptr || hipMemcpy(d_scores, scores, (size_t)n_polys * 4, hipMemcpyHostToDevice) == hipSuccess);
    if (!ok) sd::set_error("_LIB_non_maximum_suppression_sparse: H2D failed");
  } else sd::set_error("_LIB_non_maximum_suppression_sparse: hipMalloc failed");
  std::vector<uint8_t> keep(n_polys);
  if (ok) ok = sd_nms3d_device(d_scores, d_dist, d_pts, n_polys, n_rays, n_faces, d_verts, d_faces, threshold, use_bbox, use_kdtree, verbose,
                               d_keep, nullptr, nullptr) == 0;
  if (ok) ok = hipMemcpy(keep.data(), d_keep, n_polys, hipMemcpyDeviceToHost) == hipSuccess;
  (void)hipFree(d_dist); (void)hipFree(d_pts); (void)hipFree(d_verts); (void)hipFree(d_faces); (void)hipFree(d_scores); (void)hipFree(d_keep);
  if (!ok) {
    fprintf(stderr, "_LIB_non_maximum_suppression_sparse failed: %s\n", sd::err_buf());
    abort();
  }
  for (int i = 0; i < n_polys; ++i) result[i] = keep[i] != 0;
}
```

stardist_amd/csrc/nms_rounds.h:

```cpp
#pragma once
#include "common.h"
#include <hipcub/hipcub.hpp>

namespace sd {
struct SideJoin {
  hipEvent_t fork = nullptr, done = nullptr;
  bool pending = false;
  ~SideJoin() { if (pending) (void)hipEventSynchronize(done); if (fork) (void)hipEventDestroy(fork); if (done) (void)hipEventDestroy(done); }
  int begin(hipStream_t s, hipStream_t side) {
    if (!fork) { SD_CHECK(hipEventCreateWithFlags(&fork, hipEventDisableTiming)); SD_CHECK(hipEventCreateWithFlags(&done, hipEventDisableTiming)); }
    SD_CHECK(hipEventRecord(fork, s));
    SD_CHECK(hipStreamWaitEvent(side, fork, 0));
    return 0;
  }
  int end(hipStream_t side) { SD_CHECK(hipEventRecord(done, side)); pending = true; return 0; }
  int join(hipStream_t s) { if (pending) { SD_CHECK(hipStreamWaitEvent(s, done, 0)); pending = false; } return 0; }
};
}

namespace {

struct Timer {
  hipEvent_t a = nullptr, b = nullptr;
  ~Timer() { if (a) (void)hipEventDestroy(a); if (b) (void)hipEventDestroy(b); }
  int init() { SD_CHECK(hipEventCreate(&a)); SD_CHECK(hipEventCreate(&b)); return 0; }
  int start(hipStream_t s) { if (a) SD_CHECK(hipEventRecord(a, s)); return 0; }
  int stop(hipStream_t s) { if (a) SD_CHECK(hipEventRecord(b, s)); return 0; }
  int wait() { if (a) SD_CHECK(hipEventSynchronize(b)); return 0; }
  int ms(float* out) { *out = 0; if (a) SD_CHECK(hipEventElapsedTime(out, a, b)); return 0; }
};

enum { ST_UNDECIDED = 0, ST_KEPT = 1, ST_SUPPRESSED = 2 };

#define WAIT_NONE (-2)
#define WAIT_SCAN (-1)

struct NmsFlags { int use_kdtree, use_bbox, thr_nonneg; float thr, max_dist; };

__global__ void k_iota(int* a, int n) { int i = blockIdx.x * blockDim.x + threadIdx.x; if (i < n) a[i] = i; }
__global__ void k_keep(const unsigned char* __restrict__ state, unsigned char* __restrict__ keep, int n) {
  int i = blockIdx.x * blockDim.x + threadIdx.x;
  if (i < n) keep[i] = (state[i] != ST_SUPPRESSED);
}

__global__ void __launch_bounds__(256) k_sum_halves(const int* __restrict__ nLow, const int* __restrict__ nHigh, int N, unsigned long long* total) {
  __shared__ unsigned long long ws[4];
  unsigned long long v = 0;
  for (int i = blockIdx.x * 256 + threadIdx.x; i < N; i += gridDim.x * 256) v += (unsigned long long)(nLow[i] + (nHigh ? nHigh[i] : 0));
  for (int o = 32; o; o >>= 1) v += __shfl_xor(v, o);
  if ((threadIdx.x & 63) == 0) ws[threadIdx.x >> 6] = v;
  __syncthreads();
  if (threadIdx.x == 0) atomicAdd(total, ws[0] + ws[1] + ws[2] + ws[3]);
}

__global__ void __launch_bounds__(1024) k_round_triage(const int* __restrict__ U, int nU, const unsigned char* __restrict__ state,
                                                       const int* __restrict__ waitOn, int* __restrict__ Unext, int* __restrict__ K,
                                                       int* __restrict__ S, int* counters ,
                                                       const unsigned char* __restrict__ pend) {
  const int t = blockIdx.x * blockDim.x + threadIdx.x;
  const int lane = threadIdx.x & 63, wave = threadIdx.x >> 6, nw = blockDim.x >> 6;
  int kind = 0, i = -1;
  if (t < nU) {
    i = U[t];
    if (state[i] != ST_SUPPRESSED) {
      const int wo = waitOn[i];
      if (pend && pend[i]) kind = 1;
      else if (wo == WAIT_NONE) kind = 2;
      else if (wo >= 0 && state[wo] == ST_UNDECIDED) kind = 1;
      else kind = 3;
    }
  }
  __shared__ int wcnt[3][16];
  __shared__ int bbase[3];
#pragma unroll
  for (int q = 1; q <= 3; ++q) {
    const unsigned long long m = __ballot(kind == q);
    if (lane == 0) wcnt[q - 1][wave] = __popcll(m);
  }
  __syncthreads();
  if (threadIdx.x < 3) {
    int sum = 0;
    for (int w = 0; w < nw; ++w) { const int c = wcnt[threadIdx.x][w]; wcnt[threadIdx.x][w] = sum; sum += c; }
    bbase[threadIdx.x] = sum ? atomicAdd(&counters[threadIdx.x], sum) : 0;
  }
  __syncthreads();
#pragma unroll
  for (int q = 1; q <= 3; ++q) {
    const unsigned long long m = __ballot(kind == q);
    if (kind == q) (q == 1 ? Unext : (q == 2 ? K : S))[bbase[q - 1] + wcnt[q - 1][wave] + __popcll(m & ((1ull << lane) - 1))] = i;
  }
}

__global__ void __launch_bounds__(256) k_round_scan(const int* __restrict__ S, const unsigned char* __restrict__ state,
                                                    const long long* __restrict__ nbrStart, const int* __restrict__ nbrLow, const int* __restrict__ nbr,
                                                    int* __restrict__ waitOn, int* __restrict__ Unext, int* __restrict__ K,
                                                    int* counters , const unsigned char* __restrict__ pend) {
  const int lane = threadIdx.x & 63;
  const int nS = counters[2];
  const int nWaves = gridDim.x * (blockDim.x >> 6);
  int myI = -1, myKind = 0, nbuf = 0;
  auto flush = [&]() {
#pragma unroll
    for (int q = 1; q <= 2; ++q) {
      const unsigned long long m = __ballot(lane < nbuf && myKind == q);
      if (!m) continue;
      int base = 0;
      if (lane == 0) base = atomicAdd(&counters[q - 1], __popcll(m));
      base = __shfl(base, 0);
      if (lane < nbuf && myKind == q) (q == 1 ? Unext : K)[base + __popcll(m & ((1ull << lane) - 1))] = myI;
    }
    nbuf = 0;
  };
  const int sub = lane >> 4, sl = lane & 15;
  for (int w0 = (blockIdx.x * (blockDim.x >> 6) + (threadIdx.x >> 6)) * 4; w0 < nS; w0 += nWaves * 4) {
    const int w = w0 + sub;
    const bool valid = w < nS;
    const int i = valid ? S[w] : -1;
    long long t = 0, end = 0;
    if (valid) { t = nbrStart[i]; end = t + nbrLow[i]; }
    int found = -1;
    while (__any(found < 0 && t < end)) {
      const long long idx = t + sl;
      int j = -1;
      if (found < 0 && idx < end) { j = nbr[idx]; if (!(j < i && state[j] == ST_UNDECIDED)) j = -1; }
      const unsigned long long m = __ballot(j >= 0);
      const unsigned int m16 = (unsigned int)(m >> (sub << 4)) & 0xffffu;
      const int src = (sub << 4) + (m16 ? __ffs((int)m16) - 1 : 0);
      const int jf = __shfl(j, src);
      if (found < 0 && m16) found = jf;
      t += 16;
    }
    if (valid && sl == 0) waitOn[i] = found >= 0 ? found : WAIT_NONE;
    const int kind = (found >= 0 || (valid && pend && pend[i])) ? 1 : 2;
#pragma unroll
    for (int q = 0; q < 4; ++q) {
      const int vi = __shfl(i, q << 4), vk = __shfl(kind, q << 4);
      if (vi >= 0) { if (lane == nbuf) { myI = vi; myKind = vk; } ++nbuf; }
    }
    if (nbuf > 60) flush();
  }
  flush();
}

struct NbrLists {
  int* count; int* low; long long* start;
  int* nbr; int* waitOn;
  long long total, slotTotal;
  bool slots;
  bool lowOnly;
  bool wantSlotTotal;
};

struct WidenCount { __host__ __device__ __forceinline__ long long operator()(const int& v) const { return (long long)v; } };
inline hipError_t exclusive_sum_i64(void* tmp, size_t& tmpBytes, const int* count, long long* start, int n, hipStream_t s) {
  hipcub::TransformInputIterator<long long, WidenCount, const int*> in(count, WidenCount());
  return hipcub::DeviceScan::ExclusiveScan(tmp, tmpBytes, in, start, hipcub::Sum(), (long long)0, n, s);
}

template <class LaunchNeighbours, class BeforeLists>
int build_neighbour_lists(sd::Arena& A, hipStream_t s, int N, bool singlePass, void* scanTmp, size_t scanBytes,
                          LaunchNeighbours launch, BeforeLists beforeLists, NbrLists& L) {
  L.nbr = nullptr; L.waitOn = nullptr; L.total = 0; L.slotTotal = 0; L.slots = false;
  if (singlePass || L.wantSlotTotal) {
    SD_CHECK(exclusive_sum_i64(scanTmp, scanBytes, L.count, L.start, N + 1, s));
    SD_CHECK(hipMemcpyAsync(&L.slotTotal, L.start + N, sizeof(long long), hipMemcpyDeviceToHost, s));
    SD_CHECK(hipStreamSynchronize(s));
    L.slots = singlePass && L.slotTotal >= 0 && L.slotTotal < 0x7fffffffll;
  }
  if (L.slots) {
    L.nbr = A.take_n<int>((size_t)L.slotTotal);
    if (!L.nbr) L.slots = false;
  }
  if (L.slots && beforeLists()) return -1;
  if (!L.slots) {
    SD_CHECK(hipMemsetAsync(L.count, 0, (N + 1) * sizeof(int), s));
    launch(0, L);
    SD_LAUNCH_CHECK();
    SD_CHECK(exclusive_sum_i64(scanTmp, scanBytes, L.count, L.start, N + 1, s));
    SD_CHECK(hipMemcpyAsync(&L.total, L.start + N, sizeof(long long), hipMemcpyDeviceToHost, s));
    SD_CHECK(hipStreamSynchronize(s));
    if (beforeLists()) return -1;
  }
  if (L.total < 0 || L.total >= 0x7fffffffll) return 1;
  if (!L.slots) L.nbr = A.take_n<int>((size_t)L.total);
  L.waitOn = A.take_n<int>(N);
  if (!L.nbr || !L.waitOn) return -1;
  if (L.slots) {
    unsigned long long* d_total = A.take_n<unsigned long long>(1);
    if (!d_total) return -1;
    SD_CHECK(hipMemsetAsync(d_total, 0, sizeof(unsigned long long), s));
    launch(2, L);
    hipLaunchKernelGGL(k_sum_halves, dim3(sd::div_up(N, 256) < 1024 ? sd::div_up(N, 256) : 1024), dim3(256), 0, s, L.low, L.lowOnly ? (const int*)nullptr : L.count, N, d_total);
    SD_LAUNCH_CHECK();
    unsigned long long tot = 0;
    SD_CHECK(hipMemcpyAsync(&tot, d_total, sizeof(tot), hipMemcpyDeviceToHost, s));
    SD_CHECK(hipStreamSynchronize(s));
// ... 10 lines not shown
```

stardist_amd/csrc/raster2d.hip:

```cpp
#include "common.h"
#include "../../include/stardist_hip.h"
#include <math.h>

namespace {

__device__ __forceinline__ int point_in_polygon(const double* xp, const double* yp, int n, double x, double y) {
  unsigned int l_cross = 0, r_cross = 0;
  const double eps = (double)1e-12f;
  double x1 = xp[n - 1] - x, y1 = yp[n - 1] - y;
  for (int i = 0; i < n; ++i) {
    const double x0 = xp[i] - x, y0 = yp[i] - y;
    if ((-eps < x0 && x0 < eps) && (-eps < y0 && y0 < eps)) return 2;
    if ((y0 > 0) != (y1 > 0)) { if (((x0 * y1 - x1 * y0) / (y1 - y0)) > 0) r_cross++; }
    if ((y0 < 0) != (y1 < 0)) { if (((x0 * y1 - x1 * y0) / (y1 - y0)) < 0) l_cross++; }
    x1 = x0; y1 = y0;
  }
  if ((r_cross & 1) != (l_cross & 1)) return 3;
  return (r_cross & 1) ? 1 : 0;
}

__global__ void __launch_bounds__(256) k_paint(const float* __restrict__ coord, int n_polys, int R, int HI, int WI, int y0, int x0, int H, int W,
                                               int* __restrict__ img) {
  extern __shared__ double sv[];
  double* sr = sv; double* scol = sv + R;
  __shared__ float red[4][4];
  for (int p = blockIdx.x; p < n_polys; p += gridDim.x) {
    const float* cr = coord + (size_t)p * 2 * R;
    float rmin = INFINITY, rmax = -INFINITY, cmin = INFINITY, cmax = -INFINITY;
    __syncthreads();
    for (int k = threadIdx.x; k < R; k += blockDim.x) {
      const float r = cr[k], c = cr[R + k];
      sr[k] = (double)r; scol[k] = (double)c;
      rmin = fminf(rmin, r); rmax = fmaxf(rmax, r); cmin = fminf(cmin, c); cmax = fmaxf(cmax, c);
    }
    for (int o = 32; o; o >>= 1) {
      rmin = fminf(rmin, __shfl_xor(rmin, o)); rmax = fmaxf(rmax, __shfl_xor(rmax, o));
      cmin = fminf(cmin, __shfl_xor(cmin, o)); cmax = fmaxf(cmax, __shfl_xor(cmax, o));
    }
    const int wave = threadIdx.x >> 6;
    if ((threadIdx.x & 63) == 0) { red[wave][0] = rmin; red[wave][1] = rmax; red[wave][2] = cmin; red[wave][3] = cmax; }
    __syncthreads();
    rmin = fminf(fminf(red[0][0], red[1][0]), fminf(red[2][0], red[3][0]));
    rmax = fmaxf(fmaxf(red[0][1], red[1][1]), fmaxf(red[2][1], red[3][1]));
    cmin = fminf(fminf(red[0][2], red[1][2]), fminf(red[2][2], red[3][2]));
    cmax = fmaxf(fmaxf(red[0][3], red[1][3]), fmaxf(red[2][3], red[3][3]));
    long long minr = (long long)fmaxf(0.f, rmin), minc = (long long)fmaxf(0.f, cmin);
    long long maxr = (long long)ceilf(rmax), maxc = (long long)ceilf(cmax);
    if (maxr > HI - 1) maxr = HI - 1;
    if (maxc > WI - 1) maxc = WI - 1;
    if (minr < y0) minr = y0;
    if (minc < x0) minc = x0;
    if (maxr > y0 + H - 1) maxr = y0 + H - 1;
    if (maxc > x0 + W - 1) maxc = x0 + W - 1;
    if (maxr < minr || maxc < minc) continue;
    const long long nr = maxr - minr + 1, nc = maxc - minc + 1;
    for (long long t = threadIdx.x; t < nr * nc; t += blockDim.x) {
      const int r_i = (int)(minr + t / nc), c_i = (int)(minc + t % nc);
      if (point_in_polygon(scol, sr, R, (double)c_i, (double)r_i)) atomicMax(&img[(size_t)(r_i - y0) * W + (c_i - x0)], p + 1);
    }
  }
}

__global__ void k_map_labels(int* __restrict__ img, long long n, const int* __restrict__ labels) {
  const long long i = (long long)blockIdx.x * blockDim.x + threadIdx.x;
  if (i < n) { const int v = img[i]; if (v > 0) img[i] = labels[v - 1] + 1; }
}

}

__global__ void __launch_bounds__(256) k_dist_to_coord(const float* __restrict__ dist, const double* __restrict__ points, const double* __restrict__ sc,
                                                       long long n, int R, double sy, double sx, int scaled, float* __restrict__ coord) {
  const long long t = (long long)blockIdx.x * 256 + threadIdx.x;
  if (t >= n * 2 * R) return;
  const int k = (int)(t % R), a = (int)((t / R) % 2);
  const long long i = t / (2 * R);
  float c = (float)((double)dist[i * R + k] * sc[a * R + k]);
  if (scaled) c = (float)((double)c * (a ? sx : sy));
  coord[t] = (float)((double)c + points[i * 2 + a]);
}

extern "C" int sd_dist_to_coord_device(const float* d_dist, const double* d_points, const double* d_sincos, long long n_polys, int n_rays,
                                       double scale_y, double scale_x, float* d_coord, void* stream) {
  if (n_polys <= 0 || n_rays <= 0) return 0;
  const long long tot = n_polys * 2 * n_rays;
  hipLaunchKernelGGL(k_dist_to_coord, dim3((unsigned)((tot + 255) / 256)), dim3(256), 0, (hipStream_t)stream, d_dist, d_points, d_sincos, n_polys, n_rays,
                     scale_y, scale_x, (scale_y != 1.0 || scale_x != 1.0) ? 1 : 0, d_coord);
  SD_LAUNCH_CHECK();
  return 0;
}

extern "C" int sd_polygons_to_label_window_device(const float* d_coord, const int32_t* d_labels, int n_polys, int n_rays, int HI, int WI,
                                                  int y0, int x0, int H, int W, int32_t* d_result, void* stream) {
  hipStream_t s = (hipStream_t)stream;
  if (H <= 0 || W <= 0) return 0;
  if (y0 < 0 || x0 < 0 || y0 + H > HI || x0 + W > WI) { sd::set_error("sd_polygons_to_label_window: window outside the image"); return -1; }
  SD_CHECK(hipMemsetAsync(d_result, 0, (size_t)H * W * sizeof(int32_t), s));
  if (n_polys <= 0 || n_rays <= 0) return 0;
  if ((size_t)n_rays * 2 * sizeof(double) > 60000) { sd::set_error("sd_polygons_to_label: n_rays=%d too large", n_rays); return -1; }
  const int blocks = n_polys < 65535 * 16 ? n_polys : 65535 * 16;
  hipLaunchKernelGGL(k_paint, dim3(blocks), dim3(256), 2 * n_rays * sizeof(double), s, d_coord, n_polys, n_rays, HI, WI, y0, x0, H, W, d_result);
  SD_LAUNCH_CHECK();
  const long long n = (long long)H * W;
  hipLaunchKernelGGL(k_map_labels, dim3((unsigned)((n + 255) / 256)), dim3(256), 0, s, d_result, n, d_labels);
  SD_LAUNCH_CHECK();
  return 0;
}

extern "C" int sd_polygons_to_label_device(const float* d_coord, const int32_t* d_labels, int n_polys, int n_rays,
                                           int H, int W, int32_t* d_result, void* stream) {
  return sd_polygons_to_label_window_device(d_coord, d_labels, n_polys, n_rays, H, W, 0, 0, H, W, d_result, stream);
}

extern "C" int sd_polygons_to_label_host(const float* coord, const int32_t* labels, int n_polys, int n_rays, int H, int W,
                                         int32_t* result) {
  if (H <= 0 || W <= 0) return 0;
  float* d_coord = nullptr; int* d_lab = nullptr; int* d_res = nullptr;
  const size_t nc = (size_t)(n_polys > 0 ? n_polys : 1) * 2 * (n_rays > 0 ? n_rays : 1) * sizeof(float);
  SD_CHECK(hipMalloc(&d_coord, nc));
  SD_CHECK(hipMalloc(&d_lab, (size_t)(n_polys > 0 ? n_polys : 1) * sizeof(int)));
  SD_CHECK(hipMalloc(&d_res, (size_t)H * W * sizeof(int)));
  int rc = -1;
  do {
    if (n_polys > 0) {
      if (hipMemcpy(d_coord, coord, (size_t)n_polys * 2 * n_rays * sizeof(float), hipMemcpyHostToDevice) != hipSuccess) { sd::set_error("H2D failed"); break; }
      if (hipMemcpy(d_lab, labels, (size_t)n_polys * sizeof(int), hipMemcpyHostToDevice) != hipSuccess) { sd::set_error("H2D failed"); break; }
    }
    if (sd_polygons_to_label_device(d_coord, d_lab, n_polys, n_rays, H, W, d_res, nullptr)) break;
    if (hipMemcpy(result, d_res, (size_t)H * W * sizeof(int), hipMemcpyDeviceToHost) != hipSuccess) { sd::set_error("D2H failed"); break; }
    rc = 0;
  } while (0);
  (void)hipFree(d_coord); (void)hipFree(d_lab); (void)hipFree(d_res);
  return rc;
}
```

stardist_amd/csrc/survivors.hip:

```cpp
#include "common.h"
#include <hipcub/hipcub.hpp>

namespace {
enum { ITEMS = 4, BLOCK = 256, TILE = ITEMS * BLOCK };

__global__ void __launch_bounds__(BLOCK) k_keep_count(const unsigned char* __restrict__ keep, long long n, int* __restrict__ blockCount) {
  __shared__ int wsum[4];
  const long long base = (long long)blockIdx.x * TILE;
  int c = 0;
  for (int r = 0; r < ITEMS; ++r) {
    const long long idx = base + r * BLOCK + threadIdx.x;
    c += __popcll(__ballot(idx < n && keep[idx] != 0));
  }
  if ((threadIdx.x & 63) == 0) wsum[threadIdx.x >> 6] = c;
  __syncthreads();
  if (threadIdx.x == 0) blockCount[blockIdx.x] = wsum[0] + wsum[1] + wsum[2] + wsum[3];
}

__global__ void __launch_bounds__(BLOCK) k_keep_write(const unsigned char* __restrict__ keep, long long n, const int* __restrict__ blockStart,
                                                      long long* __restrict__ pos, int* __restrict__ count, int nBlocks) {
  __shared__ int wcnt[ITEMS][4];
  const long long base = (long long)blockIdx.x * TILE;
  const int wave = threadIdx.x >> 6, lane = threadIdx.x & 63;
  unsigned long long masks[ITEMS];
  for (int r = 0; r < ITEMS; ++r) {
    const long long idx = base + r * BLOCK + threadIdx.x;
    masks[r] = __ballot(idx < n && keep[idx] != 0);
    if (lane == 0) wcnt[r][wave] = __popcll(masks[r]);
  }
  __syncthreads();
  int run = blockStart[blockIdx.x];
  for (int r = 0; r < ITEMS; ++r) {
    for (int w = 0; w < 4; ++w) {
      if (w == wave && ((masks[r] >> lane) & 1ull)) {
        const int o = run + __popcll(masks[r] & ((1ull << lane) - 1ull));
        pos[o] = base + r * BLOCK + threadIdx.x;
      }
      run += wcnt[r][w];
    }
  }
  if (blockIdx.x == nBlocks - 1 && threadIdx.x == 0) *count = run;
}

__global__ void __launch_bounds__(256) k_survivor_rows(const long long* __restrict__ pos, int m, const float* __restrict__ prob,
                                                       const long long* __restrict__ points, float* __restrict__ oprob,
                                                       long long* __restrict__ opoints, int* __restrict__ rank, int* __restrict__ labelsPaint) {
  const int r = blockIdx.x * 256 + threadIdx.x;
  if (r >= m) return;
  const long long i = pos[r];
  const float p = prob[i];
  oprob[r] = p;
  opoints[2 * r] = points[2 * i]; opoints[2 * r + 1] = points[2 * i + 1];
  int gs = r, ge = r + 1;
  while (gs > 0 && prob[pos[gs - 1]] == p) --gs;
  while (ge < m && prob[pos[ge]] == p) ++ge;
  const int rk = (m - ge) + (r - gs);
  rank[r] = rk;
  labelsPaint[rk] = r;
}

__global__ void __launch_bounds__(256) k_survivor_coord(const long long* __restrict__ pos, int m, const float* __restrict__ dist,
                                                        const long long* __restrict__ points, const double* __restrict__ sc, int R,
                                                        const int* __restrict__ rank, float* __restrict__ coord, float* __restrict__ coordPaint) {
  const long long t = (long long)blockIdx.x * 256 + threadIdx.x;
  if (t >= (long long)m * 2 * R) return;
  const int k = (int)(t % R), a = (int)((t / R) % 2);
  const int r = (int)(t / (2 * R));
  const long long i = pos[r];
  const float c = (float)((double)dist[i * R + k] * sc[a * R + k]);
  const float v = (float)((double)c + (double)points[2 * i + a]);
  coord[t] = v;
  if (coordPaint) coordPaint[((long long)rank[r] * 2 + a) * R + k] = v;
}
}

extern "C" int sd_survivor_positions_device(const unsigned char* d_keep, long long n, long long* d_positions, int32_t* d_count, void* stream) {
  hipStream_t s = (hipStream_t)stream;
  SD_CHECK(hipMemsetAsync(d_count, 0, sizeof(int), s));
  if (n <= 0) return 0;
  if (n > (1ll << 31) - TILE) { sd::set_error("sd_survivor_positions: more than 2^31 flags"); return -1; }
  const int nBlocks = (int)((n + TILE - 1) / TILE);
  sd::Arena& A = sd::arena();
  if (A.begin(s)) return -1;
  int* blockCount = A.take_n<int>(nBlocks + 1);
  int* blockStart = A.take_n<int>(nBlocks + 1);
  size_t tmpBytes = 0;
  (void)hipcub::DeviceScan::ExclusiveSum(nullptr, tmpBytes, blockCount, blockStart, nBlocks, s);
  void* tmp = A.take(tmpBytes + 256);
  if (!blockCount || !blockStart || !tmp) return -1;
  hipLaunchKernelGGL(k_keep_count, dim3(nBlocks), dim3(BLOCK), 0, s, d_keep, n, blockCount);
  SD_LAUNCH_CHECK();
  SD_CHECK(hipcub::DeviceScan::ExclusiveSum(tmp, tmpBytes, blockCount, blockStart, nBlocks, s));
  hipLaunchKernelGGL(k_keep_write, dim3(nBlocks), dim3(BLOCK), 0, s, d_keep, n, blockStart, d_positions, d_count, nBlocks);
  SD_LAUNCH_CHECK();
  return 0;
}

extern "C" int sd_survivors2d_device(const long long* d_positions, int m, const float* d_prob, const long long* d_points, const float* d_dist,
                                     int n_rays, const double* d_sincos, float* d_out_prob, long long* d_out_points, float* d_out_coord,
                                     float* d_out_coord_paint, int32_t* d_out_labels_paint, void* stream) {
  hipStream_t s = (hipStream_t)stream;
  if (m <= 0) return 0;
  if (n_rays <= 0) { sd::set_error("sd_survivors2d: n_rays must be positive"); return -1; }
  sd::Arena& A = sd::arena();
  if (A.begin(s)) return -1;
  int* rank = A.take_n<int>(m);
  int* lab = d_out_labels_paint ? d_out_labels_paint : A.take_n<int>(m);
  if (!rank || !lab) return -1;
  hipLaunchKernelGGL(k_survivor_rows, dim3((m + 255) / 256), dim3(256), 0, s, d_positions, m, d_prob, d_points, d_out_prob, d_out_points, rank, lab);
  SD_LAUNCH_CHECK();
  const long long tot = (long long)m * 2 * n_rays;
  hipLaunchKernelGGL(k_survivor_coord, dim3((unsigned)((tot + 255) / 256)), dim3(256), 0, s, d_positions, m, d_dist, d_points, d_sincos, n_rays, rank,
                     d_out_coord, d_out_coord_paint);
  SD_LAUNCH_CHECK();
  return 0;
}
```

stardist_amd/lib/_native.py:

```python
import ctypes
import os

import numpy as np

_HERE = os.path.dirname(os.path.abspath(__file__))
LIB_PATH = os.path.join(_HERE, "..", "csrc", "libstardist_hip.so")

_lib = None
last_stats = {}

_c_f32p = ctypes.POINTER(ctypes.c_float)
_c_i32p = ctypes.POINTER(ctypes.c_int32)
_c_i64p = ctypes.POINTER(ctypes.c_int64)
_c_u8p = ctypes.POINTER(ctypes.c_uint8)
_c_u16p = ctypes.POINTER(ctypes.c_uint16)
_vp = ctypes.c_void_p
_i = ctypes.c_int
_f = ctypes.c_float

SIGNATURES = {
    "sd_last_error": (ctypes.c_char_p, []),
    "sd_version": (_i, []),
    "sd_device_count": (_i, []),
    "sd_release_workspace": (_i, []),
    "sd_set_option": (_i, [ctypes.c_char_p, _i]),
    "sd_get_option": (_i, [ctypes.c_char_p]),
    "sd_nms2d_host": (_i, [_vp, _vp, _i, _i, _i, _i, _i, _f, _vp, _vp]),
    "sd_nms2d_device": (_i, [_vp, _vp, _i, _i, _i, _i, _i, _f, _vp, _vp, _vp]),
    "sd_nms2d_build_device": (_i, [_vp, _vp, _i, _i, _vp, _vp, _vp, _vp, _vp, _vp, _vp]),
    "sd_exclusive_sum_i32_i64_device": (_i, [_vp, _i, _vp, _vp]),
    "sd_nms2d_old_host": (_i, [_vp, _i, _i, _vp, _i, _i, _f, _i, _i, _i, _i, _vp]),
    "sd_nms2d_old_device": (_i, [_vp, _i, _i, _vp, _i, _i, _f, _i, _i, _i, _i, _vp, _vp]),
    "sd_clip_pairs_device": (_i, [_vp, _vp, _vp, _vp, _i, _i, _vp, _vp, _vp]),
    "sd_area_bounds_pairs_device": (_i, [_vp, _vp, _vp, _vp, _i, _i, _vp, _vp, _vp, _vp]),
    "sd_area_bounds_pairs_grid": (_i, []),
    "sd_prepare_polys_device": (_i, [_vp, _vp, _i, _i, _vp, ctypes.c_int64, _vp]),
    "sd_poly_pass_device": (_i, [_vp, _vp, _i, _i, _vp, _vp, _vp]),
    "sd_star_dist2d_host": (_i, [_vp, _i, _i, _i, _i, _i, _vp]),
    "sd_star_dist2d_device": (_i, [_vp, _i, _i, _i, _i, _i, _vp, _vp]),
    "sd_star_dist3d_host": (_i, [_vp, _i, _i, _i, _vp, _vp, _vp, _i, _i, _i, _i, _vp]),
    "sd_star_dist3d_device": (_i, [_vp, _i, _i, _i, _vp, _vp, _vp, _i, _i, _i, _i, _vp, _vp]),
    "sd_edt_prob_device": (_i, [_vp, _i, _i, _i, ctypes.c_double, ctypes.c_double, ctypes.c_double, _i, _vp, _vp]),
    "sd_dist_to_coord_device": (_i, [_vp, _vp, _vp, ctypes.c_longlong, _i, ctypes.c_double, ctypes.c_double, _vp, _vp]),
    "sd_polygons_to_label_host": (_i, [_vp, _vp, _i, _i, _i, _i, _vp]),
    "sd_polygons_to_label_device": (_i, [_vp, _vp, _i, _i, _i, _i, _vp, _vp]),
    "sd_polygons_to_label_window_device": (_i, [_vp, _vp, _i, _i, _i, _i, _i, _i, _i, _i, _vp, _vp]),
    "sd_polyhedron_to_label_window_device": (_i, [_vp, _vp, _vp, _vp, _i, _i, _i, _vp] + [_i] * 13 + [_vp, _vp]),
    "_LIB_non_maximum_suppression_sparse": (None, [_vp, _vp, _vp, _i, _i, _i, _vp, _vp, _f, _i, _i, _i, _vp]),
    "sd_nms3d_device": (_i, [_vp, _vp, _vp, _i, _i, _i, _vp, _vp, _f, _i, _i, _i, _vp, _vp, _vp]),
    "sd_hiv_pairs_device": (_i, [_vp, _vp, _i, _i, _i, _vp, _vp, _vp, _i, _vp, _vp, _vp]),
    "_LIB_polyhedron_to_label": (None, [_vp, _vp, _vp, _vp, _i, _i, _i, _vp, _i, _i, _i, _i, _i, _i, _i, _vp]),
    "sd_polyhedron_to_label_device": (_i, [_vp, _vp, _vp, _vp, _i, _i, _i, _vp, _i, _i, _i, _i, _i, _i, _i, _vp, _vp]),
    "sd_select_candidates_device": (_i, [_vp, _vp, _i, _vp, _vp, _i, _f, _i, _vp, _vp, _vp, _vp, _vp]),
    "sd_survivor_positions_device": (_i, [_vp, ctypes.c_longlong, _vp, _vp, _vp]),
    "sd_survivors2d_device": (_i, [_vp, _i, _vp, _vp, _vp, _i, _vp, _vp, _vp, _vp, _vp, _vp, _vp]),
    "sd_sorted_rows_device": (_i, [_vp, _vp, _i, _i, _vp, _vp, _vp, _vp, _vp, _vp, _vp]),
    "sd_sort_scores_desc_device": (_i, [_vp, _i, _vp, _vp, _vp]),
    "sd_bias_act_device": (_i, [_vp, _vp, ctypes.c_longlong, _i, ctypes.c_longlong, _i, _vp]),
    "sd_add_bias_act_device": (_i, [_vp, _vp, _vp, ctypes.c_longlong, _i, ctypes.c_longlong, _i, _vp]),
    "sd_maxpool_ndhwc_device": (_i, [_vp, _i, _i, _i, _i, _i, _i, _i, _vp, _vp]),
    "sd_upcat_ndhwc_device": (_i, [_vp, _i, _i, _vp, _i, _i, _i, _i, _vp, _vp]),
    "sd_inside_polyhedron_device": (_i, [_vp, _vp, _i, _i, _vp, _vp, _vp, ctypes.c_longlong, _i, _vp, _vp]),
    "sd_bias_act_dot_device": (_i, [_vp, _vp, _vp, ctypes.c_longlong, _i, _i, _vp, _vp, _i, _vp, _vp]),
    "sd_head_rows_device": (_i, [_vp, _i, _vp, ctypes.c_longlong, _vp, _vp, _i, ctypes.c_float, _vp, _vp]),
    "sd_conv3_packed_floats": (ctypes.c_longlong, [_i, _i, _i]),
    "sd_conv3_pack_weights_host": (_i, [_vp, _i, _i, _i, _vp]),
    "sd_conv3_ndhwc_device": (_i, [_vp, _i, _i, _i, _vp, _i, _i, _i, _i, _i, _i, _i, _vp, _vp, _i, _i, _vp, _vp]),
    "sd_conv3_res_ndhwc_device": (_i, [_vp, _i, _i, _i, _vp, _i, _i, _i, _i, _i, _i, _i, _vp, _vp, _vp, _i, _i, _i, _vp, _vp]),
    "sd_conv3_bf16x6_res_ndhwc_device": (_i, [_vp, _i, _i, _i, _vp, _i, _i, _i, _i, _i, _i, _i, _vp, _vp, _vp, _i, _i, _i, _vp, _vp]),
    "sd_convg_packed_floats": (ctypes.c_longlong, [_i, _i, _i, _i, _i]),
    "sd_convg_pack_weights_host": (_i, [_vp, _i, _i, _i, _i, _i, _vp]),
    "sd_convg_ndhwc_device": (_i, [_vp] + [_i] * 17 + [_vp, _vp, _vp, _i, _i, _i, _vp, _i, _vp]),
    "sd_conv3_bf16x6_packed_floats": (ctypes.c_longlong, [_i, _i, _i]),
    "sd_conv3_bf16x6_pack_weights_host": (_i, [_vp, _i, _i, _i, _vp]),
    "sd_conv3_bf16x6_ndhwc_device": (_i, [_vp, _i, _i, _i, _vp, _i, _i, _i, _i, _i, _i, _i, _vp, _vp, _i, _i, _vp, _vp]),
    "sd_conv3_f16x3_packed_floats": (ctypes.c_longlong, [_i, _i, _i]),
    "sd_conv3_f16x3_pack_weights_host": (_i, [_vp, _i, _i, _i, _vp]),
    "sd_conv3_f16x3_ndhwc_device": (_i, [_vp, _i, _i, _i, _vp, _i, _i, _i, _i, _i, _i, _i, _vp, _vp, _i, _i, _vp, _vp, _vp]),
    "sd_conv3_f16x3_res_ndhwc_device": (_i, [_vp, _i, _i, _i, _vp, _i, _i, _i, _i, _i, _i, _i, _vp, _vp, _vp, _i, _i, _i, _vp, _vp, _vp]),
    "sd_conv3_f16x3_dot_ndhwc_device": (_i, [_vp, _i, _i, _i, _vp, _i, _i, _i, _i, _i, _i, _i, _vp, _vp, _i, _i, _vp, _vp, _vp, _vp, _vp]),
    "sd_dot_combine_device": (_i, [_vp, _i, ctypes.c_longlong, _vp, _i, _vp, _vp]),
    "sd_conv3_f16x3_fmt_ndhwc_device": (_i, [_vp, _i, _i, _vp, _i, _i, _i, _i, _i, _i, _vp, _vp, _i, _i, _vp, _i, _i, _vp, _vp, _vp, _vp]),
    "sd_conv3_f16x3_rows_device": (_i, [_vp, _i, _i, _i, _i, _i, _i, _vp, _vp, _i, _i, _vp, ctypes.c_longlong, _vp, _vp]),
    "sd_conv3_c1x32_split16_device": (_i, [_vp, _i, _i, _i, _i, _vp, _vp, _i, _vp, _vp, _vp]),
    "sd_maxpool_split16_ndhwc_device": (_i, [_vp, _i, _i, _i, _i, _i, _i, _i, _vp, _vp]),
    "sd_split16_pack_device": (_i, [_vp, ctypes.c_longlong, _i, _vp, _vp, _vp]),
    "sd_split16_unpack_device": (_i, [_vp, ctypes.c_longlong, _i, _vp, _vp]),
    "sd_label_overlap_device": (_i, [_vp, _vp, ctypes.c_longlong, ctypes.c_longlong, _vp, _vp, _vp, _vp, _vp]),
    "sd_label_overlap_stack_device": (_i, [_vp, _i, ctypes.c_longlong, ctypes.c_longlong, _vp, _vp, _vp, _vp, _vp, _vp]),
    "sd_relabel_stack_device": (_i, [_vp, _i, ctypes.c_longlong, _vp, _vp, _vp, _vp, _vp, _vp]),
    "sd_conv_wgrad_ndhwc_device": (_i, [_vp, _i, _vp, _i, _i, _vp, _i, _i, _i, _i, _i, _i, _vp, _vp, _vp]),
    "sd_relu_mask_device": (_i, [_vp, _vp, ctypes.c_longlong, _vp, _vp]),
    "sd_maxpool_adjoint_ndhwc_device": (_i, [_vp, _vp, _i, _i, _i, _i, _i, _i, _vp, _vp]),
    "sd_upcat_adjoint_ndhwc_device": (_i, [_vp, _i, _i, _i, _i, _i, _i, _vp, _vp, _vp]),
    "sd_stardist_loss2d_device": (_i, [_vp, _vp, _vp, _vp, ctypes.c_longlong, _i, _i, ctypes.c_double, ctypes.c_double, ctypes.c_double,
                                       _vp, _vp, _vp, _vp]),
    "sd_stardist_loss2d_metrics_device": (_i, [_vp, _vp, _vp, _vp, ctypes.c_longlong, _i, _i, ctypes.c_double, ctypes.c_double,
                                               ctypes.c_double, _vp, _vp, _vp, _vp, _vp]),
    "sd_conv3_wgrad_ndhwc_device": (_i, [_vp, _i, _vp, _i, _i, _vp, _i, _i, _i, _i, _i, _i, _vp, _vp, _vp]),
    "sd_convg_wgrad_ndhwc_device": (_i, [_vp, _i, _vp, _i] + [_i] * 16 + [_vp, _vp, _vp]),
    "sd_convg_dgrad_ndhwc_device": (_i, [_vp, _i, _vp, _i] + [_i] * 16 + [_vp, _vp]),
    "sd_maxpool3d_adjoint_ndhwc_device": (_i, [_vp, _vp, _i, _i, _i, _i, _i, _i, _i, _i, _vp, _vp]),
    "sd_upcat3d_adjoint_ndhwc_device": (_i, [_vp, _i, _i, _i, _i, _i, _i, _i, _vp, _vp, _vp]),
    "sd_class_targets_device": (_i, [_vp, _i, _i, _i, _i, _vp, _vp, _vp, _vp, _vp, _vp, _i, _i, _i, _vp, _i, _vp, _vp, _vp]),
    "sd_class_loss_device": (_i, [_vp, _vp, _vp, ctypes.c_longlong, _i, ctypes.c_double, _vp, _vp, _vp]),
    "sd_percentiles_device": (_i, [_vp, _i, ctypes.c_longlong, _i, _vp, _i, _i, _vp, _vp]),
    "sd_normalize_mi_ma_device": (_i, [_vp, _i, ctypes.c_longlong, _i, _vp, _vp, _f, _i, _vp, _vp]),
    "sd_zoom_linear_device": (_i, [_vp, _vp, _i, _i, _vp, _vp, _vp, _vp, _vp, _vp]),
    "sd_label_boxes_device": (_i, [_vp, _i, _i, _i, _i, _vp, _vp]),
    "sd_fill_label_holes_device": (_i, [_vp, _i, _i, _i, _i, _vp, _vp]),
    "sd_label_centroid_sums_device": (_i, [_vp, _i, _i, _i, _i, _vp, _vp]),
    "sd_label_intensity_stats_device": (_i, [_vp, _i, _i, _i, _i, _vp, _vp, _i, _i, _vp, _vp, _vp, _vp]),
    "sd_label_percentiles_device": (_i, [_vp, _i, _i, _i, _i, _vp, _vp, _i, _i, _vp, _i, _i, _vp, _vp]),
    "sd_label_moment_sums_device": (_i, [_vp, _i, _i, _i, _i, _vp, _vp, _vp]),
    "sd_label_contour_counts_device": (_i, [_vp, _i, _i, _i, _vp, _vp]),
    "sd_label_hull_device": (_i, [_vp, _i, _i, _i, _vp, _vp, _vp]),
    "sd_label_components_device": (_i, [_vp, _i, _i, _i, _i, _i, ctypes.c_longlong, _vp, _vp, _vp]),
    "sd_nearest_feature_device": (_i, [_vp, _i, _i, _i, _i, _i] + [ctypes.c_double] * 4 + [_vp, _vp, _vp]),
    "sd_expand_labels_device": (_i, [_vp, _i, _i, _i] + [ctypes.c_double] * 4 + [_vp, _vp]),
    "sd_find_boundaries_device": (_i, [_vp, _i, _i, _i, _i, _i, ctypes.c_longlong, ctypes.c_longlong, _vp, _vp]),
    "sd_label_border_flags_device": (_i, [_vp, _i, _i, _i, _i, _i, _vp, ctypes.c_longlong, _vp, _vp]),
    "sd_label_clear_flagged_device": (_i, [_vp, _vp, _vp, ctypes.c_longlong, ctypes.c_longlong, _i, _vp, _vp]),
    "sd_label_contacts_device": (_i, [_vp, _i, _i, _i, _i, _i, _i, ctypes.c_longlong, _vp, _vp, _vp, _vp, _vp, _vp]),
    "sd_point_neighbors_device": (_i, [_vp, ctypes.c_longlong, _vp, ctypes.c_longlong, _i, _i, _i, _i, ctypes.c_double, ctypes.c_double,
                                       ctypes.c_longlong, _vp, _vp, _vp, _vp, _vp, _vp]),
    "sd_gaussian_filter_device": (_i, [_vp, _i, _i] + [ctypes.c_longlong] * 3 + [_vp, _vp, _vp, _vp, _vp]),
    "sd_peak_local_max_device": (_i, [_vp, _i, _i] + [ctypes.c_longlong] * 3 + [_vp, _vp, _vp, _i, ctypes.c_double, _i, ctypes.c_double]
                                 + [ctypes.c_longlong] * 3 + [_vp, _vp, _vp]),
    "sd_peaks_emit_device": (_i, [_vp, _i, _i] + [ctypes.c_longlong] * 3 + [_vp, _vp, ctypes.c_longlong, _vp, _vp, _vp, _vp]),
    "sd_augment_batch_device": (_i, [_vp, _vp, _i, _i, _vp, _i, _vp, _vp, _vp, _i, _vp, _vp, _vp]),
    "sd_star_dist2d_points_device": (_i, [_vp, _i, _i, _vp, _i, _i, _vp, _vp]),
    "sd_star_dist3d_points_device": (_i, [_vp, _i, _i, _i, _vp, _i, _vp, _vp, _vp, _i, _f, _vp, _vp]),
    "sd_star_dist2d_points_host": (_i, [_vp, _i, _i, _vp, _i, _i, _vp]),
    "sd_star_dist3d_points_host": (_i, [_vp, _i, _i, _i, _vp, _i, _vp, _vp, _vp, _i, _f, _vp]),
    "_LIB_non_maximum_suppression_2d": (None, [_vp, _vp, _i, _i, _f, _i, _i, _i, _vp]),
    "_LIB_polygon_to_label": (None, [_vp, _vp, _i, _i, _i, _i, _vp]),
    "_LIB_star_dist": (None, [_vp, _i, _i, _i, _i, _i, _vp]),
    "_LIB_star_dist3d": (None, [_vp, _i, _i, _i, _vp, _vp, _vp, _i, _i, _i, _i, _vp]),
}


class NativeError(RuntimeError):
    pass


def lib():
    global _lib
    if _lib is None:
        path = os.path.abspath(LIB_PATH)
        if not os.path.exists(path):
            raise NativeError("libstardist_hip.so not built (%s): run `python -m stardist_amd.build` "
                              "or __graft_entry__.build(); there is no CPU fallback" % path)
        try:
            import torch
        except Exception:
            pass
        l = ctypes.CDLL(path)
        for name, (res, args) in SIGNATURES.items():
            fn = getattr(l, name)
            fn.restype = res
            fn.argtypes = args
        _lib = l
    return _lib


class option(object):

    def __init__(self, name, value):
        self.name, self.value = name.encode(), int(value)

    def __enter__(self):
        self.old = lib().sd_get_option(self.name)
        check(lib().sd_set_option(self.name, self.value))
        return self

    def __exit__(self, *exc):
        lib().sd_set_option(self.name, self.old)
        return False


def require_device():
    if lib().sd_device_count() < 1:
        raise NativeError("no HIP device visible: the stardist_amd natives only run on a GPU "
                          "(there is no CPU fallback)")


def check(rc):
    if rc != 0:
        raise NativeError(lib().sd_last_error().decode(errors="replace"))


def ptr(a):
    if a is None:
        return None
    assert a.flags["C_CONTIGUOUS"]
    return a.ctypes.data_as(ctypes.c_void_p)


def is_torch(x):
    return type(x).__module__.startswith("torch")


def tptr(t):
    assert t.is_cuda and t.is_contiguous()
    return ctypes.c_void_p(t.data_ptr())


def current_stream(device=None):
# ... 14 lines not shown
```

stardist_amd/lib/stardist2d.py:

```python
import numpy as np

from . import _native as N


def c_non_max_suppression_inds(dist, points, use_kdtree, use_bbox, verbose, threshold, return_stats=False, _as_uint8=False):
    N.require_device()
    stats = np.zeros(16, np.int64)
    if N.is_torch(dist):
        import torch
        assert dist.dtype == torch.float32 and points.dtype == torch.float32
        dist = dist.contiguous(); points = points.contiguous()
        n, R = dist.shape
        keep = torch.empty(n, dtype=torch.uint8, device=dist.device)
        N.dcall(dist, "sd_nms2d_device", N.tptr(dist), N.tptr(points), n, R, int(use_kdtree), int(use_bbox),
                                        int(verbose), float(threshold), N.tptr(keep), N.ptr(stats))
        if not _as_uint8:
            keep = keep.bool()
    else:
        dist = np.ascontiguousarray(dist, np.float32)
        points = np.ascontiguousarray(points, np.float32)
        if dist.ndim != 2 or points.ndim != 2 or points.shape[1] != 2 or len(points) != len(dist):
            raise ValueError("dist must be (n,n_rays) and points (n,2)")
        n, R = dist.shape
        keep = np.zeros(n, np.uint8)
        N.check(N.lib().sd_nms2d_host(N.ptr(dist), N.ptr(points), n, R, int(use_kdtree), int(use_bbox),
                                      int(verbose), float(threshold), N.ptr(keep), N.ptr(stats)))
        keep = keep.astype(bool)
    N.last_stats["nms2d"] = stats
    return (keep, stats) if return_stats else keep


def c_non_max_suppression_inds_old(polys, mapping, threshold, max_bbox_search, grid_y, grid_x, verbose):
    N.require_device()
    if N.is_torch(polys):
        import torch
        assert polys.dtype == torch.int32 and polys.dim() == 3 and polys.shape[1] == 2
        polys = polys.contiguous()
        mapping = mapping.to(torch.int32).contiguous()
        n, _, R = polys.shape
        H, W = (int(mapping.shape[0]), int(mapping.shape[1])) if mapping.dim() == 2 else (0, 0)
        keep = torch.empty(n, dtype=torch.uint8, device=polys.device)
        if n:
            N.dcall(polys, "sd_nms2d_old_device", N.tptr(polys), n, R, N.tptr(mapping) if mapping.numel() else None, H, W, float(threshold),
                    int(max_bbox_search), int(grid_y), int(grid_x), int(verbose), N.tptr(keep))
        return keep.bool()
    polys = np.ascontiguousarray(polys)
    mapping = np.ascontiguousarray(mapping)
    if polys.dtype != np.int32 or mapping.dtype != np.int32:
        raise TypeError("polys and mapping must be int32")
    if polys.ndim != 3 or polys.shape[1] != 2:
        raise ValueError("polys must be (n, 2, n_rays)")
    n, _, R = polys.shape
    H, W = (mapping.shape[0], mapping.shape[1]) if mapping.ndim == 2 else (0, 0)
    keep = np.zeros(n, np.uint8)
    if n:
        N.check(N.lib().sd_nms2d_old_host(N.ptr(polys), n, R, N.ptr(mapping) if mapping.size else None, int(H), int(W), float(threshold),
                                          int(max_bbox_search), int(grid_y), int(grid_x), int(verbose), N.ptr(keep)))
    return keep.astype(bool)


def c_star_dist(src, n_rays, grid_y, grid_x):
    N.require_device()
    n_rays, grid_y, grid_x = int(n_rays), int(grid_y), int(grid_x)
    if N.is_torch(src):
        import torch
        assert src.dtype in (torch.uint16, torch.int16) and src.dim() == 2
        src = src.contiguous()
        H, W = src.shape
        dst = torch.empty(((H - 1) // grid_y + 1, (W - 1) // grid_x + 1, n_rays), dtype=torch.float32, device=src.device)
        N.dcall(src, "sd_star_dist2d_device", N.tptr(src), H, W, n_rays, grid_y, grid_x, N.tptr(dst))
        return dst
    src = np.ascontiguousarray(src)
    if src.dtype != np.uint16:
        src = src.astype(np.uint16)
    H, W = src.shape
    dst = np.empty(((H - 1) // grid_y + 1, (W - 1) // grid_x + 1, n_rays), np.float32)
    N.check(N.lib().sd_star_dist2d_host(N.ptr(src), H, W, n_rays, grid_y, grid_x, N.ptr(dst)))
    return dst


def c_polygons_to_label(coord, labels, shape, window=None):
    N.require_device()
    H, W = int(shape[0]), int(shape[1])
    if N.is_torch(coord):
        import torch
        coord = coord.contiguous().float()
        labels = labels.contiguous().to(torch.int32)
        n, _, R = coord.shape
        (y0, x0), (h, w) = ((0, 0), (H, W)) if window is None else window
        out = torch.empty((int(h), int(w)), dtype=torch.int32, device=coord.device)
        N.dcall(coord, "sd_polygons_to_label_window_device", N.tptr(coord), N.tptr(labels), n, R, H, W, int(y0), int(x0), int(h), int(w), N.tptr(out))
        return out
    if window is not None:
        raise ValueError("window rendering takes device tensors")
    coord = np.ascontiguousarray(coord, np.float32)
    labels = np.ascontiguousarray(labels, np.int32)
    n = coord.shape[0]
    R = coord.shape[2] if coord.ndim == 3 else 0
    out = np.zeros((H, W), np.int32)
    if n:
        N.check(N.lib().sd_polygons_to_label_host(N.ptr(coord), N.ptr(labels), n, R, H, W, N.ptr(out)))
    return out


def survivors_of_sorted(keep, prob, points, dist, want_paint=True):
    import torch
    from ..geometry.geom2d import ray_angles, _SC_CACHE
    N.require_device()
    assert keep.is_cuda and prob.dtype == torch.float32 and dist.dtype == torch.float32 and points.dtype == torch.int64 and points.shape[1] == 2
    n, R = int(dist.shape[0]), int(dist.shape[1])
    assert keep.numel() == n == prob.numel() == points.shape[0]
    dev = keep.device
    keep = keep.contiguous().view(torch.uint8) if keep.dtype == torch.bool else keep.contiguous()
    prob, points, dist = prob.contiguous(), points.contiguous(), dist.contiguous()
    pos = torch.empty(max(n, 1), dtype=torch.int64, device=dev)
    cnt = torch.empty(1, dtype=torch.int32, device=dev)
    N.dcall(keep, "sd_survivor_positions_device", N.tptr(keep), n, N.tptr(pos), N.tptr(cnt))
    m = int(cnt.item())
    key = (R, str(dev))
    sct = _SC_CACHE.get(key)
    if sct is None:
        phis = ray_angles(R)
        sct = _SC_CACHE[key] = torch.as_tensor(np.ascontiguousarray(np.array([np.sin(phis), np.cos(phis)])), device=dev)
    oprob = torch.empty(m, dtype=torch.float32, device=dev)
    opts = torch.empty((m, 2), dtype=torch.int64, device=dev)
    coord = torch.empty((m, 2, R), dtype=torch.float32, device=dev)
    cpaint = torch.empty((m, 2, R), dtype=torch.float32, device=dev) if want_paint else None
    lpaint = torch.empty(m, dtype=torch.int32, device=dev) if want_paint else None
    if m:
        N.dcall(keep, "sd_survivors2d_device", N.tptr(pos), m, N.tptr(prob), N.tptr(points), N.tptr(dist), R, N.tptr(sct), N.tptr(oprob), N.tptr(opts),
                N.tptr(coord), N.tptr(cpaint) if want_paint else None, N.tptr(lpaint) if want_paint else None)
    return oprob, opts, coord, cpaint, lpaint


def clip_pairs(xa, ya, xb, yb):
    import torch
    N.require_device()
    dev = torch.device("cuda")
    t = [torch.from_numpy(np.ascontiguousarray(v, np.int32)).to(dev) for v in (xa, ya, xb, yb)]
    n, R = t[0].shape
    out = torch.zeros(n, dtype=torch.int64, device=dev)
    fl = torch.zeros(n, dtype=torch.int32, device=dev)
    N.dcall(t[0], "sd_clip_pairs_device", N.tptr(t[0]), N.tptr(t[1]), N.tptr(t[2]), N.tptr(t[3]), n, R,
                                         N.tptr(out), N.tptr(fl))
    torch.cuda.synchronize()
    return out.cpu().numpy(), fl.cpu().numpy()


def nms2d_build(dist, points):
    import torch
    N.require_device()
    dev = torch.device("cuda")
    d = torch.from_numpy(np.ascontiguousarray(dist, np.float32)).to(dev); p = torch.from_numpy(np.ascontiguousarray(points, np.float32)).to(dev)
    n, R = d.shape
    vx = torch.zeros((n, R), dtype=torch.int32, device=dev); vy = torch.zeros((n, R), dtype=torch.int32, device=dev)
    bbox = torch.zeros((n, 4), dtype=torch.int32, device=dev); gstats = torch.zeros(5, dtype=torch.int32, device=dev)
    radius = torch.zeros(n, dtype=torch.float32, device=dev); area = torch.zeros(n, dtype=torch.float32, device=dev)
    N.dcall(d, "sd_nms2d_build_device", N.tptr(d), N.tptr(p), n, R, N.tptr(vx), N.tptr(vy), N.tptr(bbox), N.tptr(radius), N.tptr(area), N.tptr(gstats))
    torch.cuda.synchronize()
    return tuple(t.cpu().numpy() for t in (vx, vy, bbox, radius, area, gstats))


def area_bounds_pairs(xa, ya, xb, yb):
    import torch
    N.require_device()
    dev = torch.device("cuda")
    t = [torch.from_numpy(np.ascontiguousarray(v, np.int32)).to(dev) for v in (xa, ya, xb, yb)]
    n, R = t[0].shape
    area = torch.zeros(n, dtype=torch.float32, device=dev); band = torch.zeros(n, dtype=torch.float32, device=dev)
    info = torch.zeros(n, dtype=torch.int32, device=dev)
    N.dcall(t[0], "sd_area_bounds_pairs_device", N.tptr(t[0]), N.tptr(t[1]), N.tptr(t[2]), N.tptr(t[3]), n, R, N.tptr(area), N.tptr(band), N.tptr(info))
    torch.cuda.synchronize()
    info = info.cpu().numpy()
    return area.cpu().numpy(), band.cpu().numpy(), (info & 1).astype(bool), (info >> 8) & 0x3FF, (info >> 18) & 0x7FF
```

stardist_amd/models/model2d.py:

```python
import numpy as np

from ..utils import to_host

from ..geometry.geom2d import dist_to_coord, polygons_to_label
from ..lib import _native as N
from ..nms import non_maximum_suppression, non_maximum_suppression_sparse
from .base import StarDistBase, axes_check_and_normalize
from .config import Config2D


class StarDist2D(StarDistBase):

    def __init__(self, config=Config2D(), name=None, basedir=".", **kwargs):
        super().__init__(config, name=name, basedir=basedir, **kwargs)

    def _build(self):
        from .unet import StarDistNet
        if self.config.backbone != "unet":
            raise NotImplementedError()
        return StarDistNet(self.config)

    def _instances_from_prediction(self, img_shape, prob, dist, points=None, prob_class=None, prob_thresh=None,
                                   nms_thresh=None, overlap_label=None, return_labels=True, scale=None, **nms_kwargs):
        if prob_thresh is None: prob_thresh = self.thresholds.prob
        if nms_thresh is None: nms_thresh = self.thresholds.nms
        if overlap_label is not None:
            raise NotImplementedError("overlap_label not supported for 2D yet!")
        if points is not None:
            points, probi, disti, indsi = non_maximum_suppression_sparse(dist, prob, points, nms_thresh=nms_thresh, **nms_kwargs)
            if prob_class is not None:
                prob_class = prob_class[indsi]
        else:
            points, probi, disti = non_maximum_suppression(dist, prob, grid=self.config.grid, prob_thresh=prob_thresh,
                                                           nms_thresh=nms_thresh, **nms_kwargs)
            if prob_class is not None:
                inds = tuple(p // g for p, g in zip(points.T, self.config.grid))
                prob_class = prob_class[inds]
        return self._instances_from_survivors(img_shape, points, probi, disti, prob_class=prob_class, return_labels=return_labels, scale=scale)

    def _instances_from_sorted(self, img_shape, cand, nms_thresh=None, overlap_label=None, return_labels=True, scale=None, **nms_kwargs):
        from ..nms import non_maximum_suppression_sparse_sorted
        if nms_thresh is None: nms_thresh = self.thresholds.nms
        if overlap_label is not None:
            raise NotImplementedError("overlap_label not supported for 2D yet!")
        import torch
        if scale is None and cand.dist.is_cuda and cand.dist.dtype == torch.float32 and cand.points.dtype == torch.int64 and len(cand.prob):
            from ..lib.stardist2d import survivors_of_sorted, c_polygons_to_label
            from ..nms import nms_keep_sorted
            from ..utils import to_host_many
            keep = nms_keep_sorted(cand.dist, cand.prob, cand.points_f32, nms_thresh=nms_thresh, **nms_kwargs)
            probi, points, coord, cpaint, lpaint = survivors_of_sorted(keep, cand.prob, cand.points, cand.dist, want_paint=return_labels)
            labels = c_polygons_to_label(cpaint, lpaint, img_shape) if return_labels else None
            labels, coord_h, points_h, prob_h = to_host_many([labels, coord, points, probi])
            return labels, dict(coord=coord_h, points=points_h, prob=prob_h)
        idx = non_maximum_suppression_sparse_sorted(cand.dist, cand.prob, cand.points_f32, nms_thresh=nms_thresh, **nms_kwargs)
        return self._instances_from_survivors(img_shape, cand.points.index_select(0, idx), cand.prob.index_select(0, idx),
                                              cand.dist.index_select(0, idx), return_labels=return_labels, scale=scale)

    def _instances_from_survivors(self, img_shape, points, probi, disti, prob_class=None, return_labels=True, scale=None, window=None):
        if scale is not None:
            if not (isinstance(scale, dict) and "X" in scale and "Y" in scale):
                raise ValueError("scale must be a dictionary with entries for 'X' and 'Y'")
            rescale = (1 / scale["Y"], 1 / scale["X"])
            if N.is_torch(points):
                import torch
                points = points * torch.tensor(rescale, device=points.device, dtype=torch.float64).reshape(1, 2)
            else:
                points = points * np.array(rescale).reshape(1, 2)
        else:
            rescale = (1, 1)
        if window is None and N.is_torch(disti) and N.is_torch(points) and N.is_torch(probi) and disti.is_cuda:
            import torch
            from ..geometry.geom2d import polygons_to_label_coord
            from ..utils import to_host_many
            coord = dist_to_coord(disti, points, scale_dist=rescale)
            labels = None
            if return_labels:
                ind = torch.sort(probi, stable=True)[1]
                labels = polygons_to_label_coord(coord.index_select(0, ind), shape=img_shape, labels=ind)
            pc = prob_class if (prob_class is not None and N.is_torch(prob_class)) else None
            labels, coord_h, points_h, prob_h, pc_h = to_host_many([labels, coord, points, probi, pc])
            res_dict = dict(coord=coord_h, points=points_h, prob=prob_h)
            if prob_class is not None:
                prob_class = np.asarray(pc_h if pc is not None else prob_class)
                res_dict.update(dict(class_prob=prob_class, class_id=np.argmax(prob_class, axis=-1)))
            return labels, res_dict
        if return_labels:
            labels = polygons_to_label(disti, points, prob=probi, shape=img_shape, scale_dist=rescale, window=window)
        else:
            labels = None
        if window is not None:
            return labels, None
        coord = dist_to_coord(disti, points, scale_dist=rescale)
        to_np = (lambda t: t.cpu().numpy()) if N.is_torch(coord) else (lambda t: t)
        if labels is not None and N.is_torch(labels):
            labels = to_host(labels)
        res_dict = dict(coord=to_np(coord), points=to_np(points), prob=to_np(probi))
        if prob_class is not None:
            prob_class = np.asarray(to_np(prob_class) if N.is_torch(prob_class) else prob_class)
            class_id = np.argmax(prob_class, axis=-1)
            res_dict.update(dict(class_prob=prob_class, class_id=class_id))
        return labels, res_dict

    def _nms_sparse(self, dist, prob, points, nms_thresh=None, **nms_kwargs):
        if nms_thresh is None: nms_thresh = self.thresholds.nms
        inds = non_maximum_suppression_sparse(dist, prob, points, nms_thresh=nms_thresh, **nms_kwargs)[3]
        return inds.cpu().numpy() if N.is_torch(inds) else np.asarray(inds)

    def _nms_sparse_device(self, dist, prob, points, nms_thresh=None, **nms_kwargs):
        if nms_thresh is None: nms_thresh = self.thresholds.nms
        r = non_maximum_suppression_sparse(dist, prob, points, nms_thresh=nms_thresh, **nms_kwargs)
        return r[0], r[1], r[2], r[3]

    def train(self, X, Y, validation_data, classes="auto", augmenter=None, seed=None, epochs=None, steps_per_epoch=None, workers=1):
        import warnings
        from ..training import train
        if not self._is_multiclass() and classes not in ("auto", None):
            warnings.warn("Ignoring given classes as n_classes is set to None")
        return train(self, X, Y, validation_data, classes=classes, augmenter=augmenter, seed=seed, epochs=epochs,
                     steps_per_epoch=steps_per_epoch)

    def _axes_div_by(self, query_axes):
        query_axes = axes_check_and_normalize(query_axes)
        div_by = dict(zip(self.config.axes.replace("C", ""),
                          tuple(p ** self.config.unet_n_depth * g for p, g in zip(self.config.unet_pool, self.config.grid))))
        return tuple(div_by.get(a, 1) for a in query_axes)

    @property
    def _config_class(self):
        return Config2D
```

stardist_amd/nms.py:

```python
import numpy as np

from .lib import _native as N
from .utils import _normalize_grid


def _is_t(x):
    return N.is_torch(x)


def _as_arrays(*xs):
    if any(_is_t(x) for x in xs):
        return xs
    return tuple(np.asarray(x) for x in xs)


def _ind_prob_thresh(prob, prob_thresh, b=2):
    if b is not None and np.isscalar(b):
        b = ((b, b),) * prob.ndim
    if _is_t(prob):
        import torch
        ind_thresh = prob > torch.tensor(prob_thresh, dtype=prob.dtype, device=prob.device)
        if b is not None:
            _ind = torch.zeros_like(ind_thresh)
            ss = tuple(slice(_bs[0] if _bs[0] > 0 else None, -_bs[1] if _bs[1] > 0 else None) for _bs in b)
            _ind[ss] = True
            ind_thresh &= _ind
        return ind_thresh
    ind_thresh = prob > prob_thresh
    if b is not None:
        _ind = np.zeros_like(ind_thresh)
        ss = tuple(slice(_bs[0] if _bs[0] > 0 else None, -_bs[1] if _bs[1] > 0 else None) for _bs in b)
        _ind[ss] = True
        ind_thresh &= _ind
    return ind_thresh


def _argsort_desc(x):
    if _is_t(x):
        return _sort_desc(x)[1]
    return np.argsort(x, kind="stable")[::-1]


def _sort_desc(x):
    import torch
    if x.is_cuda and x.dtype == torch.float32 and x.dim() == 1 and 0 < x.numel() < 2 ** 31:
        from .lib import _native as N
        x = x.contiguous()
        sp = torch.empty_like(x)
        order = torch.empty(x.numel(), dtype=torch.int64, device=x.device)
        N.dcall(x, "sd_sort_scores_desc_device", N.tptr(x), int(x.numel()), N.tptr(sp), N.tptr(order))
        return sp, order
    sp, order = torch.sort(x, stable=True)
    return torch.flip(sp, dims=(0,)), torch.flip(order, dims=(0,))


def non_maximum_suppression_inds(dist, points, scores, thresh=0.5, use_bbox=True, use_kdtree=True, verbose=1):
    from .lib.stardist2d import c_non_max_suppression_inds
    assert dist.ndim == 2 and points.ndim == 2
    n_poly = dist.shape[0]
    assert points.shape[0] == n_poly and (scores is None or len(scores) == n_poly)
    if _is_t(dist):
        import torch
        d = dist.to(torch.float32).contiguous()
        p = points.to(torch.float32).contiguous()
    else:
        d = np.ascontiguousarray(dist.astype(np.float32, copy=False))
        p = np.ascontiguousarray(points.astype(np.float32, copy=False))
    return c_non_max_suppression_inds(d, p, int(use_kdtree), int(use_bbox), int(verbose), np.float32(thresh))


def _non_maximum_suppression_old(coord, prob, grid=(1, 1), b=2, nms_thresh=0.5, prob_thresh=0.5, verbose=False, max_bbox_search=True):
    from .lib.stardist2d import c_non_max_suppression_inds_old
    coord = np.asarray(coord); prob = np.asarray(prob)
    assert prob.ndim == 2
    assert coord.ndim == 4
    grid = _normalize_grid(grid, 2)
    mask = _ind_prob_thresh(prob, prob_thresh, b)
    polygons = coord[mask]
    scores = prob[mask]
    ind = _argsort_desc(scores)
    survivors = np.zeros(len(ind), bool)
    polygons = polygons[ind]
    scores = scores[ind]
    if max_bbox_search:
        mapping = -np.ones(mask.shape, np.int32)
        mapping.flat[np.flatnonzero(mask)[ind]] = range(len(ind))
    else:
        mapping = np.empty((0, 0), np.int32)
    survivors[ind] = c_non_max_suppression_inds_old(np.ascontiguousarray(polygons.astype(np.int32)), mapping, np.float32(nms_thresh),
                                                    np.int32(max_bbox_search), np.int32(grid[0]), np.int32(grid[1]), np.int32(verbose))
    if verbose:
        print("keeping %s/%s polygons" % (np.count_nonzero(survivors), len(polygons)))
    points = np.stack([ii[survivors] for ii in np.nonzero(mask)], axis=-1)
    return points


def non_maximum_suppression(dist, prob, grid=(1, 1), b=2, nms_thresh=0.5, prob_thresh=0.5,
                            use_bbox=True, use_kdtree=True, verbose=False):
    assert prob.ndim == 2 and dist.ndim == 3 and tuple(prob.shape) == tuple(dist.shape[:2])
    grid = _normalize_grid(grid, 2)
    mask = _ind_prob_thresh(prob, prob_thresh, b)
    if _is_t(prob):
        import torch
        points = torch.stack(torch.where(mask), dim=1)
        dist = dist[mask]; scores = prob[mask]
        ind = _argsort_desc(scores)
        dist, scores, points = dist[ind], scores[ind], points[ind]
        points = points * torch.tensor(grid, device=points.device).reshape(1, 2)
        inds = non_maximum_suppression_inds(dist, points.to(torch.int32), scores=scores, use_bbox=use_bbox,
                                            use_kdtree=use_kdtree, thresh=nms_thresh, verbose=verbose)
        return points[inds], scores[inds], dist[inds]
    dist = np.asarray(dist); prob = np.asarray(prob)
    points = np.stack(np.where(mask), axis=1)
    dist = dist[mask]; scores = prob[mask]
    ind = _argsort_desc(scores)
    dist, scores, points = dist[ind], scores[ind], points[ind]
    points = (points * np.array(grid).reshape((1, 2)))
    inds = non_maximum_suppression_inds(dist, points.astype(np.int32, copy=False), scores=scores, use_bbox=use_bbox,
                                        use_kdtree=use_kdtree, thresh=nms_thresh, verbose=verbose)
    return points[inds], scores[inds], dist[inds]


def non_maximum_suppression_sparse(dist, prob, points, b=2, nms_thresh=0.5, use_bbox=True, use_kdtree=True, verbose=False):
    dist, prob, points = _as_arrays(dist, prob, points)
    assert dist.ndim == 2 and prob.ndim == 1 and points.ndim == 2 and points.shape[-1] == 2 and \
        len(prob) == len(dist) == len(points)
    _sorted = _argsort_desc(prob)
    if _is_t(prob):
        import torch
        inds_original = torch.arange(len(prob), device=prob.device)[_sorted]
    else:
        dist = np.asarray(dist); prob = np.asarray(prob); points = np.asarray(points)
        inds_original = np.arange(len(prob))[_sorted]
    probi, disti, pointsi = prob[_sorted], dist[_sorted], points[_sorted]
    inds = non_maximum_suppression_inds(disti, pointsi, scores=probi, thresh=nms_thresh, use_kdtree=use_kdtree, verbose=verbose)
    if _is_t(inds):
        inds = _survivor_positions(inds)
    return pointsi[inds], probi[inds], disti[inds], inds_original[inds]


def _survivor_positions(keep):
    import torch
    return torch.nonzero(keep).reshape(-1)


def non_maximum_suppression_sparse_sorted(dist, prob, points, b=2, nms_thresh=0.5, use_bbox=True, use_kdtree=True, verbose=False):
    return _survivor_positions(nms_keep_sorted(dist, prob, points, b=b, nms_thresh=nms_thresh, use_bbox=use_bbox, use_kdtree=use_kdtree, verbose=verbose))


def nms_keep_sorted(dist, prob, points, b=2, nms_thresh=0.5, use_bbox=True, use_kdtree=True, verbose=False):
    from .lib.stardist2d import c_non_max_suppression_inds
    import torch
    assert dist.ndim == 2 and prob.ndim == 1 and points.ndim == 2 and points.shape[-1] == 2 and len(prob) == len(dist) == len(points)
    return c_non_max_suppression_inds(dist.to(torch.float32).contiguous(), points.to(torch.float32).contiguous(), int(use_kdtree), 1, int(verbose),
                                      np.float32(nms_thresh), _as_uint8=True)


def non_maximum_suppression_3d_sparse_sorted(dist, prob, points, rays, b=2, nms_thresh=0.5, use_kdtree=True, verbose=False):
    from .lib.stardist3d import c_non_max_suppression_inds
    from .rays3d import rays_device_tensors, warn_if_degenerate
    assert dist.ndim == 2 and prob.ndim == 1 and points.ndim == 2 and dist.shape[-1] == len(rays) and points.shape[-1] == 3 and \
        len(prob) == len(dist) == len(points)
    warn_if_degenerate(rays)
    verts, faces = rays_device_tensors(rays, dist.device)
    keep = c_non_max_suppression_inds(dist, points, verts, faces, prob, 1, int(use_kdtree), int(verbose), np.float32(nms_thresh), _as_uint8=True)
    return _survivor_positions(keep)


def non_maximum_suppression_3d_inds(dist, points, rays, scores, thresh=0.5, use_bbox=True, use_kdtree=True, verbose=1):
    from .lib.stardist3d import c_non_max_suppression_inds
    from .rays3d import warn_if_degenerate
    assert dist.ndim == 2 and points.ndim == 2 and dist.shape[1] == len(rays)
    warn_if_degenerate(rays)
    n_poly = dist.shape[0]
    if _is_t(dist):
        import torch
        if scores is None:
            scores = torch.ones(n_poly, device=dist.device)
        ind = _argsort_desc(scores)
        survivors = torch.ones(n_poly, dtype=torch.bool, device=dist.device)
        from .rays3d import rays_device_tensors
        verts, faces = rays_device_tensors(rays, dist.device)
        survivors[ind] = c_non_max_suppression_inds(dist[ind].float().contiguous(), points[ind].float().contiguous(),
                                                    verts, faces, scores[ind].float().contiguous(),
                                                    int(use_bbox), int(use_kdtree), int(verbose), np.float32(thresh))
        return survivors
    if scores is None:
        scores = np.ones(n_poly)
    ind = _argsort_desc(scores)
    survivors = np.ones(n_poly, bool)
    dist, points, scores = dist[ind], points[ind], scores[ind]

    def _prep(x, dtype):
        return np.ascontiguousarray(x.astype(dtype, copy=False))
    survivors[ind] = c_non_max_suppression_inds(_prep(dist, np.float32), _prep(points, np.float32),
                                                _prep(rays.vertices, np.float32), _prep(rays.faces, np.int32),
                                                _prep(scores, np.float32), int(use_bbox), int(use_kdtree), int(verbose),
                                                np.float32(thresh))
    return survivors


def non_maximum_suppression_3d(dist, prob, rays, grid=(1, 1, 1), b=2, nms_thresh=0.5, prob_thresh=0.5, use_bbox=True,
                               use_kdtree=True, verbose=False):
    dist = np.asarray(dist); prob = np.asarray(prob)
    assert prob.ndim == 3 and dist.ndim == 4 and dist.shape[-1] == len(rays) and prob.shape == dist.shape[:3]
    grid = _normalize_grid(grid, 3)
    ind_thresh = _ind_prob_thresh(prob, prob_thresh, b)
    points = np.stack(np.where(ind_thresh), axis=1)
    probi = prob[ind_thresh]; disti = dist[ind_thresh]
    _sorted = _argsort_desc(probi)
    probi, disti, points = probi[_sorted], disti[_sorted], points[_sorted]
    points = (points * np.array(grid).reshape((1, 3)))
    inds = non_maximum_suppression_3d_inds(disti, points, rays=rays, scores=probi, thresh=nms_thresh, use_bbox=use_bbox,
                                           use_kdtree=use_kdtree, verbose=verbose)
    return points[inds], probi[inds], disti[inds]


def non_maximum_suppression_3d_sparse(dist, prob, points, rays, b=2, nms_thresh=0.5, use_kdtree=True, verbose=False):
    dist, prob, points = _as_arrays(dist, prob, points)
    assert dist.ndim == 2 and prob.ndim == 1 and points.ndim == 2 and dist.shape[-1] == len(rays) and \
        points.shape[-1] == 3 and len(prob) == len(dist) == len(points)
    _sorted = _argsort_desc(prob)
    if _is_t(prob):
        import torch
        inds_original = torch.arange(len(prob), device=prob.device)[_sorted]
    else:
        dist = np.asarray(dist); prob = np.asarray(prob); points = np.asarray(points)
        inds_original = np.arange(len(prob))[_sorted]
    probi, disti, pointsi = prob[_sorted], dist[_sorted], points[_sorted]
    inds = non_maximum_suppression_3d_inds(disti, pointsi, rays=rays, scores=probi, thresh=nms_thresh, use_kdtree=use_kdtree, verbose=verbose)
    if _is_t(inds):
        inds = _survivor_positions(inds)
    return pointsi[inds], probi[inds], disti[inds], inds_original[inds]
```

Before: 349.5.

## Fuse 2D instance finish into one device call with band-binned rasterization

The 2D NMS keep kernel now also counts survivors into a pinned host word, so the survivor count is known without a separate nonzero pass. A new native finish routine gathers survivors, bins polygons into row bands and paints the label image band by band, copying the results straight into pinned host buffers, with work spread over the main and side streams. This replaces several Python-level launches, the device-wide rasterization and the separate device-to-host copies. It adds band-list memory and more complex synchronization, and it fails with an error if the announced count does not match the keep flags.

```diff
diff --git a/include/stardist_hip.h b/include/stardist_hip.h
--- a/include/stardist_hip.h
+++ b/include/stardist_hip.h
@@ -73,6 +73,12 @@
 int sd_survivors2d_device(const long long* d_positions, int m, const float* d_prob, const long long* d_points, const float* d_dist,
                           int n_rays, const double* d_sincos, float* d_out_prob, long long* d_out_points, float* d_out_coord,
                           float* d_out_coord_paint, int32_t* d_out_labels_paint, void* stream);
+
+int sd_instances2d_finish_device(const unsigned char* d_keep, long long n, const float* d_prob, const long long* d_points, const float* d_dist,
+                                 int n_rays, const double* d_sincos, int H, int W, int m, int32_t* h_labels, float* h_coord,
+                                 long long* h_points, float* h_prob, int band_rows, void* stream);
+int sd_raster2d_band_lists_device(const float* d_coord, int n_polys, int n_rays, int H, int band_rows, int32_t* d_band_count,
+                                  int32_t* d_band_list, void* stream);
 
 void _LIB_non_maximum_suppression_sparse(const float* scores, const float* dist,
                                          const float* points, const int n_polys,
diff --git a/stardist_amd/csrc/common.h b/stardist_amd/csrc/common.h
--- a/stardist_amd/csrc/common.h
+++ b/stardist_amd/csrc/common.h
@@ -37,6 +37,7 @@
 Arena& arena();
 
 hipStream_t side_stream();
+int* pinned_words();
 
 enum { kMaxDevices = 64 };
 int resident_grid(const void* kernel, int threads, int* cache);
@@ -46,7 +47,13 @@
 
 static inline int div_up(long long a, long long b) { return (int)((a + b - 1) / b); }
 
-enum Option { OPT_NMS3D_VOLUME_BOUNDS, OPT_NMS3D_CONE_MAP, OPT_NMS3D_REFINE_MESH, OPT_PROBE_TIER, OPT_PROBE_NO_GENERAL, OPT_TRACE, OPT_NMS3D_TAIL_BATCH, OPT_NMS3D_SPLIT_EXACT, OPT_CONV_F16_WGS, OPT_NMS2D_PAIR_LANES, OPT_NMS2D_AREA_BOUNDS, OPT_NMS2D_DEFER_UNDECIDED, OPT_NMS2D_STRICT, OPT_NMS2D_NBR_SINGLE, OPT_NMS3D_NBR_SINGLE, OPT_NMS2D_DEFER_MAX, OPT_NMS3D_BOUNDS_REUSE, OPT_NMS3D_DEFER_EXACT, OPT_NMS3D_BOUNDS_LEAN, OPT_COUNT };
+int raster2d_check_rays(int n_rays);
+int raster2d_bin_bands(const float* d_coord, int n_polys, const int* d_n, int n_rays, int HI, int band_rows, int n_bands, int* d_band_count,
+                       int* d_band_list, hipStream_t s);
+int raster2d_paint_rows(const float* d_coord, const int32_t* d_labels, int n_polys, const int* d_n, const int* d_list, const int* d_list_count,
+                        int n_rays, int HI, int WI, int y0, int rows, int32_t* d_rows, hipStream_t s);
+
+enum Option { OPT_NMS3D_VOLUME_BOUNDS, OPT_NMS3D_CONE_MAP, OPT_NMS3D_REFINE_MESH, OPT_PROBE_TIER, OPT_PROBE_NO_GENERAL, OPT_TRACE, OPT_NMS3D_TAIL_BATCH, OPT_NMS3D_SPLIT_EXACT, OPT_CONV_F16_WGS, OPT_NMS2D_PAIR_LANES, OPT_NMS2D_AREA_BOUNDS, OPT_NMS2D_DEFER_UNDECIDED, OPT_NMS2D_STRICT, OPT_NMS2D_NBR_SINGLE, OPT_NMS3D_NBR_SINGLE, OPT_NMS2D_DEFER_MAX, OPT_NMS3D_BOUNDS_REUSE, OPT_NMS3D_DEFER_EXACT, OPT_NMS3D_BOUNDS_LEAN, OPT_FINISH2D_BAND_ROWS, OPT_COUNT };
 int option(Option o);
 
 #ifdef SD_DEBUG_SWITCHES
diff --git a/stardist_amd/csrc/lib.hip b/stardist_amd/csrc/lib.hip
--- a/stardist_amd/csrc/lib.hip
+++ b/stardist_amd/csrc/lib.hip
@@ -15,8 +15,8 @@
   va_end(ap);
 }
 
-static int g_opt[OPT_COUNT] = {1, 1, 2, 1, 0, 0, 1, 3, 2, 64, 1, 2, 0, 1, 1, 16384, 1, 3, 1};
-static const char* const g_opt_name[OPT_COUNT] = {"nms3d_volume_bounds", "nms3d_cone_map", "nms3d_refine_mesh", "probe_tier", "probe_no_general", "trace", "nms3d_tail_batch", "nms3d_split_exact", "conv_f16_workgroups_per_cu", "nms2d_pair_lanes", "nms2d_area_bounds", "nms2d_defer_undecided", "nms2d_strict", "nms2d_neighbours_single_pass", "nms3d_neighbours_single_pass", "nms2d_defer_max", "nms3d_bounds_reuse", "nms3d_defer_exact", "nms3d_bounds_lean"};
+static int g_opt[OPT_COUNT] = {1, 1, 2, 1, 0, 0, 1, 3, 2, 64, 1, 2, 0, 1, 1, 16384, 1, 3, 1, 0};
+static const char* const g_opt_name[OPT_COUNT] = {"nms3d_volume_bounds", "nms3d_cone_map", "nms3d_refine_mesh", "probe_tier", "probe_no_general", "trace", "nms3d_tail_batch", "nms3d_split_exact", "conv_f16_workgroups_per_cu", "nms2d_pair_lanes", "nms2d_area_bounds", "nms2d_defer_undecided", "nms2d_strict", "nms2d_neighbours_single_pass", "nms3d_neighbours_single_pass", "nms2d_defer_max", "nms3d_bounds_reuse", "nms3d_defer_exact", "nms3d_bounds_lean", "finish2d_band_rows"};
 int option(Option o) { return g_opt[o]; }
 #ifdef SD_DEBUG_SWITCHES
 int tuning_env(const char* name, int dflt) { const char* e = getenv(name); return e ? atoi(e) : dflt; }
@@ -37,6 +37,16 @@
   std::lock_guard<std::mutex> lock(mu);
   if (!st[d] && hipStreamCreateWithFlags(&st[d], hipStreamNonBlocking) != hipSuccess) { st[d] = nullptr; set_error("side_stream: cannot create a stream"); }
   return st[d];
+}
+
+int* pinned_words() {
+  static std::mutex mu;
+  static int* w[kMaxDevices] = {};
+  int d = 0;
+  if (hipGetDevice(&d) != hipSuccess || d < 0 || d >= kMaxDevices) { set_error("pinned_words: no current device"); return nullptr; }
+  std::lock_guard<std::mutex> lock(mu);
+  if (!w[d] && hipHostMalloc((void**)&w[d], 16 * sizeof(int), hipHostMallocDefault) != hipSuccess) { w[d] = nullptr; set_error("pinned_words: cannot allocate page-locked memory"); }
+  return w[d];
 }
 
 int resident_grid(const void* kernel, int threads, int* cache) {
diff --git a/stardist_amd/csrc/nms2d.hip b/stardist_amd/csrc/nms2d.hip
--- a/stardist_amd/csrc/nms2d.hip
+++ b/stardist_amd/csrc/nms2d.hip
@@ -698,7 +698,7 @@
 }
 
 namespace {
-struct Counters { int nU, nK, nS, left; unsigned long long nPairs; unsigned int nSpill, nExact, nErr, nDecided, nSkipped; };
+struct Counters { int nU, nK, nS, left; unsigned long long nPairs; unsigned int nSpill, nExact, nErr, nDecided, nSkipped, nKeep; };
 
 template <int MAXV, int SPREP>
 struct BeamPath {
@@ -1137,9 +1137,14 @@
   }
 
   int report(uint8_t* d_keep, int64_t* stats, int verbose) {
-    hipLaunchKernelGGL(k_keep, dim3(sd::div_up(N, 256)), dim3(256), 0, s, state, d_keep, N);
+    int* hKeep = stats ? sd::pinned_words() : nullptr;
+    if (stats && !hKeep) return -1;
+    if (stats && rounds == 0) SD_CHECK(hipMemsetAsync(&d_cnt->nKeep, 0, sizeof(unsigned int), s));
+    hipLaunchKernelGGL(k_keep, dim3(keep_grid(N, stats != nullptr)), dim3(256), 0, s, state, d_keep, N, stats ? &d_cnt->nKeep : (unsigned int*)nullptr);
     SD_LAUNCH_CHECK();
+    if (stats) SD_CHECK(hipMemcpyAsync(hKeep, &d_cnt->nKeep, sizeof(unsigned int), hipMemcpyDeviceToHost, s));
     SD_CHECK(hipStreamSynchronize(s));
+    if (stats) stats[14] = (int64_t)(unsigned int)hKeep[0];
     if (stats) { stats[0] = totalPairs; stats[1] = totalExact; stats[2] = rounds; stats[3] = totalNbr;
                  stats[4] = (int64_t)ns_pairs; stats[5] = n_pair_launches; stats[6] = (int64_t)ns_full; stats[7] = (int64_t)ns_pre;
                  stats[8] = totalSpill; stats[9] = totalDecided; stats[10] = totalUndecDeferred; stats[11] = totalSkipped;
@@ -1172,6 +1177,7 @@
     SD_CHECK(hipMemsetAsync(d_keep, 0, n_polys, s));
     SD_CHECK(hipMemsetAsync(d_keep, 1, 1, s));
     SD_CHECK(hipStreamSynchronize(s));
+    if (stats) stats[14] = 1;
     return 0;
   }
   if (c.build() || c.build_grid() || c.build_lists() || c.begin_rounds()) return -1;
@@ -1322,7 +1328,7 @@
     SD_CHECK(hipStreamSynchronize(s));
     if (check_sweep("sd_nms2d_old", h, qCap, false, "")) return -1;
   }
-  hipLaunchKernelGGL(k_keep, dim3(sd::div_up(N, 256)), dim3(256), 0, s, state, d_keep, N);
+  hipLaunchKernelGGL(k_keep, dim3(sd::div_up(N, 256)), dim3(256), 0, s, state, d_keep, N, (unsigned int*)nullptr);
   SD_LAUNCH_CHECK();
   SD_CHECK(hipStreamSynchronize(s));
   if (verbose) { printf("NMS: %lld candidate pairs evaluated\n", (long long)total); fflush(stdout); }
diff --git a/stardist_amd/csrc/nms3d.hip b/stardist_amd/csrc/nms3d.hip
--- a/stardist_amd/csrc/nms3d.hip
+++ b/stardist_amd/csrc/nms3d.hip
@@ -1302,7 +1302,7 @@
   }
 
   int report(uint8_t* d_keep, int64_t* stats) {
-    hipLaunchKernelGGL(k_keep, dim3(sd::div_up(N, 256)), dim3(256), 0, s, state, d_keep, N);
+    hipLaunchKernelGGL(k_keep, dim3(sd::div_up(N, 256)), dim3(256), 0, s, state, d_keep, N, (unsigned int*)nullptr);
     SD_LAUNCH_CHECK();
     Stats hs_;
     SD_CHECK(hipMemcpyAsync(&hs_, d_st, sizeof(Stats), hipMemcpyDeviceToHost, s));
diff --git a/stardist_amd/csrc/nms_rounds.h b/stardist_amd/csrc/nms_rounds.h
--- a/stardist_amd/csrc/nms_rounds.h
+++ b/stardist_amd/csrc/nms_rounds.h
@@ -38,10 +38,22 @@
 struct NmsFlags { int use_kdtree, use_bbox, thr_nonneg; float thr, max_dist; };
 
 __global__ void k_iota(int* a, int n) { int i = blockIdx.x * blockDim.x + threadIdx.x; if (i < n) a[i] = i; }
-__global__ void k_keep(const unsigned char* __restrict__ state, unsigned char* __restrict__ keep, int n) {
-  int i = blockIdx.x * blockDim.x + threadIdx.x;
-  if (i < n) keep[i] = (state[i] != ST_SUPPRESSED);
-}
+__global__ void __launch_bounds__(256) k_keep(const unsigned char* __restrict__ state, unsigned char* __restrict__ keep, int n,
+                                              unsigned int* __restrict__ count) {
+  __shared__ int ws[4];
+  int c = 0;
+  for (long long i = (long long)blockIdx.x * 256 + threadIdx.x; i < n; i += (long long)gridDim.x * 256) {
+    const bool k = state[i] != ST_SUPPRESSED;
+    keep[i] = k;
+    c += k ? 1 : 0;
+  }
+  if (!count) return;
+  for (int o = 32; o; o >>= 1) c += __shfl_xor(c, o);
+  if ((threadIdx.x & 63) == 0) ws[threadIdx.x >> 6] = c;
+  __syncthreads();
+  if (threadIdx.x == 0 && ws[0] + ws[1] + ws[2] + ws[3]) atomicAdd(count, (unsigned int)(ws[0] + ws[1] + ws[2] + ws[3]));
+}
+static inline int keep_grid(int n, bool counting) { const int g = sd::div_up(n, 256); return counting && g > 256 ? 256 : g; }
 
 __global__ void __launch_bounds__(256) k_sum_halves(const int* __restrict__ nLow, const int* __restrict__ nHigh, int N, unsigned long long* total) {
   __shared__ unsigned long long ws[4];
diff --git a/stardist_amd/csrc/raster2d.hip b/stardist_amd/csrc/raster2d.hip
--- a/stardist_amd/csrc/raster2d.hip
+++ b/stardist_amd/csrc/raster2d.hip
@@ -19,45 +19,83 @@
   return (r_cross & 1) ? 1 : 0;
 }
 
-__global__ void __launch_bounds__(256) k_paint(const float* __restrict__ coord, int n_polys, int R, int HI, int WI, int y0, int x0, int H, int W,
-                                               int* __restrict__ img) {
+__device__ __forceinline__ void paint_polygon(const float* __restrict__ coord, int p, int R, int HI, int WI, int y0, int x0, int H, int W,
+                                              int* __restrict__ img, double* sr, double* scol, float (*red)[4]) {
+  const float* cr = coord + (size_t)p * 2 * R;
+  float rmin = INFINITY, rmax = -INFINITY, cmin = INFINITY, cmax = -INFINITY;
+  __syncthreads();
+  for (int k = threadIdx.x; k < R; k += blockDim.x) {
+    const float r = cr[k], c = cr[R + k];
+    sr[k] = (double)r; scol[k] = (double)c;
+    rmin = fminf(rmin, r); rmax = fmaxf(rmax, r); cmin = fminf(cmin, c); cmax = fmaxf(cmax, c);
+  }
+  for (int o = 32; o; o >>= 1) {
+    rmin = fminf(rmin, __shfl_xor(rmin, o)); rmax = fmaxf(rmax, __shfl_xor(rmax, o));
+    cmin = fminf(cmin, __shfl_xor(cmin, o)); cmax = fmaxf(cmax, __shfl_xor(cmax, o));
+  }
+  const int wave = threadIdx.x >> 6;
+  if ((threadIdx.x & 63) == 0) { red[wave][0] = rmin; red[wave][1] = rmax; red[wave][2] = cmin; red[wave][3] = cmax; }
+  __syncthreads();
+  rmin = fminf(fminf(red[0][0], red[1][0]), fminf(red[2][0], red[3][0]));
+  rmax = fmaxf(fmaxf(red[0][1], red[1][1]), fmaxf(red[2][1], red[3][1]));
+  cmin = fminf(fminf(red[0][2], red[1][2]), fminf(red[2][2], red[3][2]));
+  cmax = fmaxf(fmaxf(red[0][3], red[1][3]), fmaxf(red[2][3], red[3][3]));
+  long long minr = (long long)fmaxf(0.f, rmin), minc = (long long)fmaxf(0.f, cmin);
+  long long maxr = (long long)ceilf(rmax), maxc = (long long)ceilf(cmax);
+  if (maxr > HI - 1) maxr = HI - 1;
+  if (maxc > WI - 1) maxc = WI - 1;
+  if (minr < y0) minr = y0;
+  if (minc < x0) minc = x0;
+  if (maxr > y0 + H - 1) maxr = y0 + H - 1;
+  if (maxc > x0 + W - 1) maxc = x0 + W - 1;
+  if (maxr < minr || maxc < minc) return;
+  const long long nr = maxr - minr + 1, nc = maxc - minc + 1;
+  for (long long t = threadIdx.x; t < nr * nc; t += blockDim.x) {
+    const int r_i = (int)(minr + t / nc), c_i = (int)(minc + t % nc);
+    if (point_in_polygon(scol, sr, R, (double)c_i, (double)r_i)) atomicMax(&img[(size_t)(r_i - y0) * W + (c_i - x0)], p + 1);
+  }
+}
+
+__global__ void __launch_bounds__(256) k_paint(const float* __restrict__ coord, int n_polys, const int* __restrict__ n_dev, int R, int HI, int WI, int y0,
+                                               int x0, int H, int W, int* __restrict__ img) {
   extern __shared__ double sv[];
-  double* sr = sv; double* scol = sv + R;
   __shared__ float red[4][4];
-  for (int p = blockIdx.x; p < n_polys; p += gridDim.x) {
+  if (n_dev && *n_dev < n_polys) n_polys = *n_dev;
+  for (int p = blockIdx.x; p < n_polys; p += gridDim.x) paint_polygon(coord, p, R, HI, WI, y0, x0, H, W, img, sv, sv + R, red);
+}
+
+__global__ void __launch_bounds__(256) k_paint_list(const float* __restrict__ coord, const int* __restrict__ list, const int* __restrict__ listCount, int R,
+                                                    int HI, int WI, int y0, int H, int* __restrict__ img) {
+  extern __shared__ double sv[];
+  __shared__ float red[4][4];
+  const int n = *listCount;
+  for (int e = blockIdx.x; e < n; e += gridDim.x) paint_polygon(coord, list[e], R, HI, WI, y0, 0, H, WI, img, sv, sv + R, red);
+}
+
+__global__ void __launch_bounds__(256) k_bin_bands(const float* __restrict__ coord, int n_polys, const int* __restrict__ n_dev, int R, int HI, int band_rows,
+                                                   int cap, int* __restrict__ bandCount, int* __restrict__ bandList) {
+  if (n_dev && *n_dev < n_polys) n_polys = *n_dev;
+  const int p = blockIdx.x * 256 + threadIdx.x, lane = threadIdx.x & 63;
+  int b0 = 0x7fffffff, b1 = -1;
+  if (p < n_polys) {
     const float* cr = coord + (size_t)p * 2 * R;
-    float rmin = INFINITY, rmax = -INFINITY, cmin = INFINITY, cmax = -INFINITY;
-    __syncthreads();
-    for (int k = threadIdx.x; k < R; k += blockDim.x) {
-      const float r = cr[k], c = cr[R + k];
-      sr[k] = (double)r; scol[k] = (double)c;
-      rmin = fminf(rmin, r); rmax = fmaxf(rmax, r); cmin = fminf(cmin, c); cmax = fmaxf(cmax, c);
-    }
-    for (int o = 32; o; o >>= 1) {
-      rmin = fminf(rmin, __shfl_xor(rmin, o)); rmax = fmaxf(rmax, __shfl_xor(rmax, o));
-      cmin = fminf(cmin, __shfl_xor(cmin, o)); cmax = fmaxf(cmax, __shfl_xor(cmax, o));
-    }
-    const int wave = threadIdx.x >> 6;
-    if ((threadIdx.x & 63) == 0) { red[wave][0] = rmin; red[wave][1] = rmax; red[wave][2] = cmin; red[wave][3] = cmax; }
-    __syncthreads();
-    rmin = fminf(fminf(red[0][0], red[1][0]), fminf(red[2][0], red[3][0]));
-    rmax = fmaxf(fmaxf(red[0][1], red[1][1]), fmaxf(red[2][1], red[3][1]));
-    cmin = fminf(fminf(red[0][2], red[1][2]), fminf(red[2][2], red[3][2]));
-    cmax = fmaxf(fmaxf(red[0][3], red[1][3]), fmaxf(red[2][3], red[3][3]));
-    long long minr = (long long)fmaxf(0.f, rmin), minc = (long long)fmaxf(0.f, cmin);
-    long long maxr = (long long)ceilf(rmax), maxc = (long long)ceilf(cmax);
+    float rmin = INFINITY, rmax = -INFINITY;
+    for (int k = 0; k < R; ++k) { const float r = cr[k]; rmin = fminf(rmin, r); rmax = fmaxf(rmax, r); }
+    long long minr = (long long)fmaxf(0.f, rmin), maxr = (long long)ceilf(rmax);
     if (maxr > HI - 1) maxr = HI - 1;
-    if (maxc > WI - 1) maxc = WI - 1;
-    if (minr < y0) minr = y0;
-    if (minc < x0) minc = x0;
-    if (maxr > y0 + H - 1) maxr = y0 + H - 1;
-    if (maxc > x0 + W - 1) maxc = x0 + W - 1;
-    if (maxr < minr || maxc < minc) continue;
-    const long long nr = maxr - minr + 1, nc = maxc - minc + 1;
-    for (long long t = threadIdx.x; t < nr * nc; t += blockDim.x) {
-      const int r_i = (int)(minr + t / nc), c_i = (int)(minc + t % nc);
-      if (point_in_polygon(scol, sr, R, (double)c_i, (double)r_i)) atomicMax(&img[(size_t)(r_i - y0) * W + (c_i - x0)], p + 1);
-    }
+    if (maxr >= minr) { b0 = (int)(minr / band_rows); b1 = (int)(maxr / band_rows); }
+  }
+  int lo = b0, hi = b1;
+  for (int o = 32; o; o >>= 1) { lo = min(lo, __shfl_xor(lo, o)); hi = max(hi, __shfl_xor(hi, o)); }
+  for (int b = lo; b <= hi; ++b) {
+    const bool in = b0 <= b && b <= b1;
+    const unsigned long long mask = __ballot(in);
+    if (!mask) continue;
+    const int leader = __ffsll((long long)mask) - 1;
+    int base = 0;
+    if (lane == leader) base = atomicAdd(&bandCount[b], __popcll(mask));
+    base = __shfl(base, leader);
+    if (in) bandList[(size_t)b * cap + base + __popcll(mask & ((1ull << lane) - 1ull))] = p;
   }
 }
 
@@ -98,12 +136,56 @@
   if (n_polys <= 0 || n_rays <= 0) return 0;
   if ((size_t)n_rays * 2 * sizeof(double) > 60000) { sd::set_error("sd_polygons_to_label: n_rays=%d too large", n_rays); return -1; }
   const int blocks = n_polys < 65535 * 16 ? n_polys : 65535 * 16;
-  hipLaunchKernelGGL(k_paint, dim3(blocks), dim3(256), 2 * n_rays * sizeof(double), s, d_coord, n_polys, n_rays, HI, WI, y0, x0, H, W, d_result);
+  hipLaunchKernelGGL(k_paint, dim3(blocks), dim3(256), 2 * n_rays * sizeof(double), s, d_coord, n_polys, (const int*)nullptr, n_rays, HI, WI, y0,
+                     x0, H, W, d_result);
   SD_LAUNCH_CHECK();
   const long long n = (long long)H * W;
   hipLaunchKernelGGL(k_map_labels, dim3((unsigned)((n + 255) / 256)), dim3(256), 0, s, d_result, n, d_labels);
   SD_LAUNCH_CHECK();
   return 0;
+}
+
+namespace sd {
+int raster2d_check_rays(int n_rays) {
+  if ((size_t)n_rays * 2 * sizeof(double) > 60000) { set_error("sd_polygons_to_label: n_rays=%d too large", n_rays); return -1; }
+  return 0;
+}
+
+int raster2d_bin_bands(const float* d_coord, int n_polys, const int* d_n, int n_rays, int HI, int band_rows, int n_bands, int* d_band_count,
+                       int* d_band_list, hipStream_t s) {
+  if (band_rows <= 0 || n_bands != div_up(HI, band_rows)) { set_error("raster2d_bin_bands: %d bands of %d rows do not tile %d rows", n_bands, band_rows, HI); return -1; }
+  SD_CHECK(hipMemsetAsync(d_band_count, 0, (size_t)n_bands * sizeof(int), s));
+  if (n_polys <= 0) return 0;
+  hipLaunchKernelGGL(k_bin_bands, dim3(div_up(n_polys, 256)), dim3(256), 0, s, d_coord, n_polys, d_n, n_rays, HI, band_rows, n_polys, d_band_count,
+                     d_band_list);
+  SD_LAUNCH_CHECK();
+  return 0;
+}
+
+int raster2d_paint_rows(const float* d_coord, const int32_t* d_labels, int n_polys, const int* d_n, const int* d_list, const int* d_list_count,
+                        int n_rays, int HI, int WI, int y0, int rows, int32_t* d_rows, hipStream_t s) {
+  if (n_polys <= 0 || rows <= 0) return 0;
+  if (d_list) {
+    const int cus = cu_count();
+    if (cus < 0) return -1;
+    const int blocks = n_polys < cus * 8 ? n_polys : cus * 8;
+    hipLaunchKernelGGL(k_paint_list, dim3(blocks), dim3(256), 2 * n_rays * sizeof(double), s, d_coord, d_list, d_list_count, n_rays, HI, WI, y0, rows, d_rows);
+  } else {
+    const int blocks = n_polys < 65535 * 16 ? n_polys : 65535 * 16;
+    hipLaunchKernelGGL(k_paint, dim3(blocks), dim3(256), 2 * n_rays * sizeof(double), s, d_coord, n_polys, d_n, n_rays, HI, WI, y0, 0, rows, WI, d_rows);
+  }
+  SD_LAUNCH_CHECK();
+  const long long n = (long long)rows * WI;
+  hipLaunchKernelGGL(k_map_labels, dim3((unsigned)((n + 255) / 256)), dim3(256), 0, s, d_rows, n, d_labels);
+  SD_LAUNCH_CHECK();
+  return 0;
+}
+}
+
+extern "C" int sd_raster2d_band_lists_device(const float* d_coord, int n_polys, int n_rays, int H, int band_rows, int32_t* d_band_count,
+                                             int32_t* d_band_list, void* stream) {
+  if (H <= 0 || band_rows <= 0) { sd::set_error("sd_raster2d_band_lists: H and band_rows must be positive"); return -1; }
+  return sd::raster2d_bin_bands(d_coord, n_polys, nullptr, n_rays, H, band_rows, sd::div_up(H, band_rows), d_band_count, d_band_list, (hipStream_t)stream);
 }
 
 extern "C" int sd_polygons_to_label_device(const float* d_coord, const int32_t* d_labels, int n_polys, int n_rays,
diff --git a/stardist_amd/csrc/survivors.hip b/stardist_amd/csrc/survivors.hip
--- a/stardist_amd/csrc/survivors.hip
+++ b/stardist_amd/csrc/survivors.hip
@@ -1,5 +1,7 @@
 #include "common.h"
 #include <hipcub/hipcub.hpp>
+#include <mutex>
+#include <vector>
 
 namespace {
 enum { ITEMS = 4, BLOCK = 256, TILE = ITEMS * BLOCK };
@@ -44,7 +46,9 @@
 
 __global__ void __launch_bounds__(256) k_survivor_rows(const long long* __restrict__ pos, int m, const float* __restrict__ prob,
                                                        const long long* __restrict__ points, float* __restrict__ oprob,
-                                                       long long* __restrict__ opoints, int* __restrict__ rank, int* __restrict__ labelsPaint) {
+                                                       long long* __restrict__ opoints, int* __restrict__ rank, int* __restrict__ labelsPaint,
+                                                       const int* __restrict__ dcount) {
+  if (dcount && *dcount < m) m = *dcount;
   const int r = blockIdx.x * 256 + threadIdx.x;
   if (r >= m) return;
   const long long i = pos[r];
@@ -61,7 +65,9 @@
 
 __global__ void __launch_bounds__(256) k_survivor_coord(const long long* __restrict__ pos, int m, const float* __restrict__ dist,
                                                         const long long* __restrict__ points, const double* __restrict__ sc, int R,
-                                                        const int* __restrict__ rank, float* __restrict__ coord, float* __restrict__ coordPaint) {
+                                                        const int* __restrict__ rank, float* __restrict__ coord, float* __restrict__ coordPaint,
+                                                        const int* __restrict__ dcount) {
+  if (dcount && *dcount < m) m = *dcount;
   const long long t = (long long)blockIdx.x * 256 + threadIdx.x;
   if (t >= (long long)m * 2 * R) return;
   const int k = (int)(t % R), a = (int)((t / R) % 2);
@@ -74,14 +80,12 @@
 }
 }
 
-extern "C" int sd_survivor_positions_device(const unsigned char* d_keep, long long n, long long* d_positions, int32_t* d_count, void* stream) {
-  hipStream_t s = (hipStream_t)stream;
+namespace {
+int enqueue_positions(sd::Arena& A, hipStream_t s, const unsigned char* d_keep, long long n, long long* d_positions, int32_t* d_count) {
   SD_CHECK(hipMemsetAsync(d_count, 0, sizeof(int), s));
   if (n <= 0) return 0;
   if (n > (1ll << 31) - TILE) { sd::set_error("sd_survivor_positions: more than 2^31 flags"); return -1; }
   const int nBlocks = (int)((n + TILE - 1) / TILE);
-  sd::Arena& A = sd::arena();
-  if (A.begin(s)) return -1;
   int* blockCount = A.take_n<int>(nBlocks + 1);
   int* blockStart = A.take_n<int>(nBlocks + 1);
   size_t tmpBytes = 0;
@@ -96,22 +100,144 @@
   return 0;
 }
 
+int enqueue_survivors(sd::Arena& A, hipStream_t s, const long long* d_positions, int m, const int* d_count, const float* d_prob, const long long* d_points,
+                      const float* d_dist, int n_rays, const double* d_sincos, float* d_out_prob, long long* d_out_points, float* d_out_coord,
+                      float* d_out_coord_paint, int32_t* d_out_labels_paint) {
+  if (m <= 0) return 0;
+  if (n_rays <= 0) { sd::set_error("sd_survivors2d: n_rays must be positive"); return -1; }
+  int* rank = A.take_n<int>(m);
+  int* lab = d_out_labels_paint ? d_out_labels_paint : A.take_n<int>(m);
+  if (!rank || !lab) return -1;
+  hipLaunchKernelGGL(k_survivor_rows, dim3((m + 255) / 256), dim3(256), 0, s, d_positions, m, d_prob, d_points, d_out_prob, d_out_points, rank, lab, d_count);
+  SD_LAUNCH_CHECK();
+  const long long tot = (long long)m * 2 * n_rays;
+  hipLaunchKernelGGL(k_survivor_coord, dim3((unsigned)((tot + 255) / 256)), dim3(256), 0, s, d_positions, m, d_dist, d_points, d_sincos, n_rays, rank,
+                     d_out_coord, d_out_coord_paint, d_count);
+  SD_LAUNCH_CHECK();
+  return 0;
+}
+
+hipEvent_t* order_events(int n) {
+  static std::mutex mu;
+  static std::vector<hipEvent_t> ev[sd::kMaxDevices];
+  int d = 0;
+  if (hipGetDevice(&d) != hipSuccess || d < 0 || d >= sd::kMaxDevices) { sd::set_error("sd_instances2d_finish: no current device"); return nullptr; }
+  std::lock_guard<std::mutex> lock(mu);
+  while ((int)ev[d].size() < n) {
+    hipEvent_t e;
+    if (hipEventCreateWithFlags(&e, hipEventDisableTiming) != hipSuccess) { sd::set_error("sd_instances2d_finish: cannot create an event"); return nullptr; }
+    ev[d].push_back(e);
+  }
+  return ev[d].data();
+}
+
+enum { kMaxBands = 256 };
+
+int default_band_rows(int H, int W) {
+  long long rows = (4ll << 20) / ((long long)W * (long long)sizeof(int));
+  if (rows < 1) rows = 1;
+  if (rows >= H) return H;
+  return sd::div_up(H, sd::div_up(H, rows));
+}
+
+struct Finish {
+  const unsigned char* d_keep; long long n; const float* d_prob; const long long* d_points; const float* d_dist; int R; const double* d_sincos;
+  int H, W, m; int32_t* h_labels; float* h_coord; long long* h_points; float* h_prob; int band_rows, n_bands;
+  hipStream_t s, side; int* h_count;
+
+  int enqueue() {
+    sd::Arena& A = sd::arena();
+    if (A.begin(s)) return -1;
+    long long* pos = A.take_n<long long>((size_t)n);
+    int* count = A.take_n<int>(1);
+    float* oprob = A.take_n<float>(m);
+    long long* opoints = A.take_n<long long>((size_t)m * 2);
+    float* coord = A.take_n<float>((size_t)m * 2 * R);
+    float* cpaint = h_labels ? A.take_n<float>((size_t)m * 2 * R) : nullptr;
+    int* lpaint = h_labels ? A.take_n<int>(m) : nullptr;
+    int* img = h_labels ? A.take_n<int>((size_t)H * W) : nullptr;
+    const bool lists = h_labels && n_bands > 1 && m > 0;
+    int* bandCount = lists ? A.take_n<int>(n_bands) : nullptr;
+    int* bandList = lists ? A.take_n<int>((size_t)n_bands * m) : nullptr;
+    if (!pos || !count || !oprob || !opoints || !coord || (h_labels && (!cpaint || !lpaint || !img)) || (lists && (!bandCount || !bandList))) return -1;
+    hipEvent_t* ev = order_events(1 + n_bands);
+    if (!ev) return -1;
+    if (enqueue_positions(A, s, d_keep, n, pos, count)) return -1;
+    if (enqueue_survivors(A, s, pos, m, count, d_prob, d_points, d_dist, R, d_sincos, oprob, opoints, coord, cpaint, lpaint)) return -1;
+    if (m > 0) SD_CHECK(hipEventRecord(ev[0], s));
+    auto results_home = [&]() -> int {
+      if (m <= 0) return 0;
+      SD_CHECK(hipStreamWaitEvent(side, ev[0], 0));
+      SD_CHECK(hipMemcpyAsync(h_coord, coord, (size_t)m * 2 * R * sizeof(float), hipMemcpyDeviceToHost, side));
+      SD_CHECK(hipMemcpyAsync(h_points, opoints, (size_t)m * 2 * sizeof(long long), hipMemcpyDeviceToHost, side));
+      SD_CHECK(hipMemcpyAsync(h_prob, oprob, (size_t)m * sizeof(float), hipMemcpyDeviceToHost, side));
+      return 0;
+    };
+    if (h_labels) {
+      SD_CHECK(hipMemsetAsync(img, 0, (size_t)H * W * sizeof(int), s));
+      if (lists && sd::raster2d_bin_bands(cpaint, m, count, R, H, band_rows, n_bands, bandCount, bandList, s)) return -1;
+      for (int b = 0; b < n_bands; ++b) {
+        const int y0 = b * band_rows, rows = (y0 + band_rows <= H ? band_rows : H - y0);
+        int* d_rows = img + (size_t)y0 * W;
+        if (sd::raster2d_paint_rows(cpaint, lpaint, m, count, lists ? bandList + (size_t)b * m : nullptr, lists ? bandCount + b : nullptr, R, H, W, y0, rows,
+                                    d_rows, s)) return -1;
+        SD_CHECK(hipEventRecord(ev[1 + b], s));
+        if (b == 0 && results_home()) return -1;
+        SD_CHECK(hipStreamWaitEvent(side, ev[1 + b], 0));
+        SD_CHECK(hipMemcpyAsync(h_labels + (size_t)y0 * W, d_rows, (size_t)rows * W * sizeof(int), hipMemcpyDeviceToHost, side));
+      }
+    } else if (results_home()) return -1;
+    SD_CHECK(hipMemcpyAsync(h_count, count, sizeof(int), hipMemcpyDeviceToHost, s));
+    return 0;
+  }
+};
+}
+
+extern "C" int sd_survivor_positions_device(const unsigned char* d_keep, long long n, long long* d_positions, int32_t* d_count, void* stream) {
+  hipStream_t s = (hipStream_t)stream;
+  if (n <= 0) { SD_CHECK(hipMemsetAsync(d_count, 0, sizeof(int), s)); return 0; }
+  sd::Arena& A = sd::arena();
+  if (A.begin(s)) return -1;
+  return enqueue_positions(A, s, d_keep, n, d_positions, d_count);
+}
+
 extern "C" int sd_survivors2d_device(const long long* d_positions, int m, const float* d_prob, const long long* d_points, const float* d_dist,
                                      int n_rays, const double* d_sincos, float* d_out_prob, long long* d_out_points, float* d_out_coord,
                                      float* d_out_coord_paint, int32_t* d_out_labels_paint, void* stream) {
   hipStream_t s = (hipStream_t)stream;
   if (m <= 0) return 0;
-  if (n_rays <= 0) { sd::set_error("sd_survivors2d: n_rays must be positive"); return -1; }
   sd::Arena& A = sd::arena();
   if (A.begin(s)) return -1;
-  int* rank = A.take_n<int>(m);
-  int* lab = d_out_labels_paint ? d_out_labels_paint : A.take_n<int>(m);
-  if (!rank || !lab) return -1;
-  hipLaunchKernelGGL(k_survivor_rows, dim3((m + 255) / 256), dim3(256), 0, s, d_positions, m, d_prob, d_points, d_out_prob, d_out_points, rank, lab);
-  SD_LAUNCH_CHECK();
-  const long long tot = (long long)m * 2 * n_rays;
-  hipLaunchKernelGGL(k_survivor_coord, dim3((unsigned)((tot + 255) / 256)), dim3(256), 0, s, d_positions, m, d_dist, d_points, d_sincos, n_rays, rank,
-                     d_out_coord, d_out_coord_paint);
-  SD_LAUNCH_CHECK();
+  return enqueue_survivors(A, s, d_positions, m, nullptr, d_prob, d_points, d_dist, n_rays, d_sincos, d_out_prob, d_out_points, d_out_coord, d_out_coord_paint,
+                           d_out_labels_paint);
+}
+
+extern "C" int sd_instances2d_finish_device(const unsigned char* d_keep, long long n, const float* d_prob, const long long* d_points, const float* d_dist,
+                                            int n_rays, const double* d_sincos, int H, int W, int m, int32_t* h_labels, float* h_coord,
+                                            long long* h_points, float* h_prob, int band_rows, void* stream) {
+  if (n < 0 || m < 0 || m > n) { sd::set_error("sd_instances2d_finish: %d survivors of %lld candidates", m, n); return -1; }
+  if (n_rays <= 0) { sd::set_error("sd_instances2d_finish: n_rays must be positive"); return -1; }
+  if (h_labels && (H <= 0 || W <= 0)) { sd::set_error("sd_instances2d_finish: empty label image"); return -1; }
+  if (h_labels && sd::raster2d_check_rays(n_rays)) return -1;
+  if (m > 0 && (!h_coord || !h_points || !h_prob)) { sd::set_error("sd_instances2d_finish: null result pointer"); return -1; }
+  Finish f{d_keep, n, d_prob, d_points, d_dist, n_rays, d_sincos, H, W, m, h_labels, h_coord, h_points, h_prob, 1, 1, (hipStream_t)stream, sd::side_stream(), sd::pinned_words()};
+  if (!f.side || !f.h_count) return -1;
+  if (h_labels) {
+    if (band_rows <= 0) band_rows = sd::option(sd::OPT_FINISH2D_BAND_ROWS);
+    if (band_rows <= 0) band_rows = default_band_rows(H, W);
+    if (band_rows > H) band_rows = H;
+    if (sd::div_up(H, band_rows) > kMaxBands) band_rows = sd::div_up(H, kMaxBands);
+    f.band_rows = band_rows; f.n_bands = sd::div_up(H, band_rows);
+  }
+  f.h_count += 1;
+  *f.h_count = -1;
+  const int rc = f.enqueue();
+  const hipError_t e1 = hipStreamSynchronize(f.side), e2 = hipStreamSynchronize(f.s);
+  if (rc) return -1;
+  SD_CHECK(e1); SD_CHECK(e2);
+  if (*f.h_count != m) {
+    sd::set_error("sd_instances2d_finish: %d keep flags are set, the caller announced %d survivors (the results are not valid)", *f.h_count, m);
+    return -1;
+  }
   return 0;
 }
diff --git a/stardist_amd/lib/_native.py b/stardist_amd/lib/_native.py
--- a/stardist_amd/lib/_native.py
+++ b/stardist_amd/lib/_native.py
@@ -54,6 +54,8 @@
     "sd_select_candidates_device": (_i, [_vp, _vp, _i, _vp, _vp, _i, _f, _i, _vp, _vp, _vp, _vp, _vp]),
     "sd_survivor_positions_device": (_i, [_vp, ctypes.c_longlong, _vp, _vp, _vp]),
     "sd_survivors2d_device": (_i, [_vp, _i, _vp, _vp, _vp, _i, _vp, _vp, _vp, _vp, _vp, _vp, _vp]),
+    "sd_instances2d_finish_device": (_i, [_vp, ctypes.c_longlong, _vp, _vp, _vp, _i, _vp, _i, _i, _i, _vp, _vp, _vp, _vp, _i, _vp]),
+    "sd_raster2d_band_lists_device": (_i, [_vp, _i, _i, _i, _i, _vp, _vp, _vp]),
     "sd_sorted_rows_device": (_i, [_vp, _vp, _i, _i, _vp, _vp, _vp, _vp, _vp, _vp, _vp]),
     "sd_sort_scores_desc_device": (_i, [_vp, _i, _vp, _vp, _vp]),
     "sd_bias_act_device": (_i, [_vp, _vp, ctypes.c_longlong, _i, ctypes.c_longlong, _i, _vp]),
diff --git a/stardist_amd/lib/stardist2d.py b/stardist_amd/lib/stardist2d.py
--- a/stardist_amd/lib/stardist2d.py
+++ b/stardist_amd/lib/stardist2d.py
@@ -133,6 +133,48 @@
     return oprob, opts, coord, cpaint, lpaint
 
 
+def instances2d_finish(keep, m, prob, points, dist, shape, return_labels=True, band_rows=0):
+    import ctypes
+    import torch
+    from ..geometry.geom2d import ray_angles, _SC_CACHE
+    N.require_device()
+    assert keep.is_cuda and prob.dtype == torch.float32 and dist.dtype == torch.float32 and points.dtype == torch.int64 and points.shape[1] == 2
+    n, R = int(dist.shape[0]), int(dist.shape[1])
+    assert keep.numel() == n == prob.numel() == points.shape[0]
+    dev = keep.device
+    keep = keep.contiguous().view(torch.uint8) if keep.dtype == torch.bool else keep.contiguous()
+    prob, points, dist = prob.contiguous(), points.contiguous(), dist.contiguous()
+    key = (R, str(dev))
+    sct = _SC_CACHE.get(key)
+    if sct is None:
+        phis = ray_angles(R)
+        sct = _SC_CACHE[key] = torch.as_tensor(np.ascontiguousarray(np.array([np.sin(phis), np.cos(phis)])), device=dev)
+    m, (H, W) = int(m), (int(shape[0]), int(shape[1]))
+    labels = torch.empty((H, W), dtype=torch.int32, pin_memory=True) if return_labels else None
+    coord = torch.empty((m, 2, R), dtype=torch.float32, pin_memory=True)
+    opts = torch.empty((m, 2), dtype=torch.int64, pin_memory=True)
+    oprob = torch.empty(m, dtype=torch.float32, pin_memory=True)
+    hp = lambda t: ctypes.c_void_p(t.data_ptr()) if (t is not None and t.numel()) else None
+    N.dcall(keep, "sd_instances2d_finish_device", N.tptr(keep), n, N.tptr(prob), N.tptr(points), N.tptr(dist), R, N.tptr(sct), H, W, m,
+            hp(labels), hp(coord), hp(opts), hp(oprob), int(band_rows))
+    return (labels.numpy() if return_labels else None), coord.numpy(), opts.numpy(), oprob.numpy()
+
+
+def raster2d_band_lists(coord, H, band_rows):
+    import torch
+    N.require_device()
+    dev = torch.device("cuda")
+    c = torch.from_numpy(np.ascontiguousarray(coord, np.float32)).to(dev)
+    n, _, R = c.shape
+    nb = -(-int(H) // int(band_rows))
+    cnt = torch.zeros(nb, dtype=torch.int32, device=dev)
+    lst = torch.full((nb, max(n, 1)), -1, dtype=torch.int32, device=dev)
+    N.dcall(c, "sd_raster2d_band_lists_device", N.tptr(c), n, R, int(H), int(band_rows), N.tptr(cnt), N.tptr(lst))
+    torch.cuda.synchronize()
+    cnt, lst = cnt.cpu().numpy(), lst.cpu().numpy()
+    return [np.sort(lst[b, :cnt[b]]) for b in range(nb)]
+
+
 def clip_pairs(xa, ya, xb, yb):
     import torch
     N.require_device()
diff --git a/stardist_amd/models/model2d.py b/stardist_amd/models/model2d.py
--- a/stardist_amd/models/model2d.py
+++ b/stardist_amd/models/model2d.py
@@ -45,13 +45,10 @@
             raise NotImplementedError("overlap_label not supported for 2D yet!")
         import torch
         if scale is None and cand.dist.is_cuda and cand.dist.dtype == torch.float32 and cand.points.dtype == torch.int64 and len(cand.prob):
-            from ..lib.stardist2d import survivors_of_sorted, c_polygons_to_label
+            from ..lib.stardist2d import instances2d_finish
             from ..nms import nms_keep_sorted
-            from ..utils import to_host_many
-            keep = nms_keep_sorted(cand.dist, cand.prob, cand.points_f32, nms_thresh=nms_thresh, **nms_kwargs)
-            probi, points, coord, cpaint, lpaint = survivors_of_sorted(keep, cand.prob, cand.points, cand.dist, want_paint=return_labels)
-            labels = c_polygons_to_label(cpaint, lpaint, img_shape) if return_labels else None
-            labels, coord_h, points_h, prob_h = to_host_many([labels, coord, points, probi])
+            keep, m = nms_keep_sorted(cand.dist, cand.prob, cand.points_f32, nms_thresh=nms_thresh, return_count=True, **nms_kwargs)
+            labels, coord_h, points_h, prob_h = instances2d_finish(keep, m, cand.prob, cand.points, cand.dist, img_shape, return_labels=return_labels)
             return labels, dict(coord=coord_h, points=points_h, prob=prob_h)
         idx = non_maximum_suppression_sparse_sorted(cand.dist, cand.prob, cand.points_f32, nms_thresh=nms_thresh, **nms_kwargs)
         return self._instances_from_survivors(img_shape, cand.points.index_select(0, idx), cand.prob.index_select(0, idx),
diff --git a/stardist_amd/nms.py b/stardist_amd/nms.py
--- a/stardist_amd/nms.py
+++ b/stardist_amd/nms.py
@@ -148,12 +148,13 @@
     return _survivor_positions(nms_keep_sorted(dist, prob, points, b=b, nms_thresh=nms_thresh, use_bbox=use_bbox, use_kdtree=use_kdtree, verbose=verbose))
 
 
-def nms_keep_sorted(dist, prob, points, b=2, nms_thresh=0.5, use_bbox=True, use_kdtree=True, verbose=False):
+def nms_keep_sorted(dist, prob, points, b=2, nms_thresh=0.5, use_bbox=True, use_kdtree=True, verbose=False, return_count=False):
     from .lib.stardist2d import c_non_max_suppression_inds
     import torch
     assert dist.ndim == 2 and prob.ndim == 1 and points.ndim == 2 and points.shape[-1] == 2 and len(prob) == len(dist) == len(points)
-    return c_non_max_suppression_inds(dist.to(torch.float32).contiguous(), points.to(torch.float32).contiguous(), int(use_kdtree), 1, int(verbose),
-                                      np.float32(nms_thresh), _as_uint8=True)
+    keep, stats = c_non_max_suppression_inds(dist.to(torch.float32).contiguous(), points.to(torch.float32).contiguous(), int(use_kdtree), 1, int(verbose),
+                                             np.float32(nms_thresh), return_stats=True, _as_uint8=True)
+    return (keep, int(stats[14])) if return_count else keep
 
 
 def non_maximum_suppression_3d_sparse_sorted(dist, prob, points, rays, b=2, nms_thresh=0.5, use_kdtree=True, verbose=False):
```

Result: slower. 339.5 (-2.9%).
